# oadrian/GPUFluidSimulator

Measured on AMD Instinct MI355X. Metric: particle-steps/sec, higher is better.
Workload: dtype f32; 1 GPU; dam-break C3: 256x256x256 = 16777216 particles, grid 512^3, box 32.0, dt 5e-7, jittered lattice, FLOWING: timed after 6000 run-up steps on the device (+5 warm-up); particles=16777216, parallelism=1 GPU, whole domain, state=flow, runup_steps=6000

## Files before the change

### gpufluidsimulator_amd/capi.py

```python
from __future__ import annotations

import ctypes as C
import os

import numpy as np

HERE = os.path.dirname(os.path.abspath(__file__))
LIB_PATH = os.environ.get("SPH_HIP_LIB", os.path.join(HERE, "libsph_hip.so"))

PHASES = ("z-index", "sort", "b-grid", "dens", "force", "collision", "integrate")
HALO_RECORD_FLOATS = 8


class SphError(RuntimeError):
    pass


EXCHANGE_FN = C.CFUNCTYPE(C.c_int, C.c_void_p, C.c_int, C.c_void_p, C.c_size_t, C.c_void_p, C.c_size_t, C.c_void_p, C.c_size_t,
                          C.c_void_p, C.c_size_t, C.c_void_p)


class Transport(C.Structure):
    _fields_ = [("self", C.c_void_p), ("exchange", EXCHANGE_FN), ("host_buffers", C.c_int),
                ("abort", C.CFUNCTYPE(None, C.c_void_p))]


class Params(C.Structure):
    _fields_ = [("box_min", C.c_float * 3), ("box_max", C.c_float * 3), ("grid", C.c_uint32 * 3),
                ("h", C.c_float), ("mass", C.c_float), ("rest_density", C.c_float), ("gas_constant", C.c_float),
                ("viscosity", C.c_float), ("gravity_y", C.c_float), ("wall_eps", C.c_float),
                ("wall_damping", C.c_float), ("restitution", C.c_float), ("collision_param", C.c_float),
                ("particle_radius", C.c_float)]


MAX_COLLIDERS = 8


class Collider(C.Structure):
    _fields_ = [("center", C.c_float * 3), ("radius", C.c_float), ("velocity", C.c_float * 3), ("pad", C.c_float)]


_P = C.c_void_p
_U32 = C.c_uint32
SIGNATURES = {
    "sph_abi_version": (C.c_int, []),
    "sph_last_error": (C.c_char_p, []),
    "sph_device_count": (C.c_int, [C.POINTER(C.c_int)]),
    "sph_select_device": (C.c_int, [C.c_int]),
    "sph_selected_device": (C.c_int, []),
    "sph_default_params": (None, [C.POINTER(Params), C.POINTER(C.c_float), C.POINTER(_U32)]),
    "sph_grid_dim_for_edge": (_U32, [C.c_float, C.c_float]),
    "sph_create": (C.c_int, [C.POINTER(_P), C.c_int, _U32, C.POINTER(Params)]),
    "sph_create_slab": (C.c_int, [C.POINTER(_P), C.c_int, _U32, C.POINTER(Params), _U32, _U32, _U32]),
    "sph_create_slab_layers": (C.c_int, [C.POINTER(_P), C.c_int, _U32, C.POINTER(Params), _U32, _U32, _U32, _U32]),
    "sph_ghost_layers": (_U32, [_P]),
    "sph_slab_set_protocol": (C.c_int, [_P, C.c_int]),
    "sph_slab_protocol": (C.c_int, [_P, C.POINTER(C.c_uint64)]),
    "sph_destroy": (None, [_P]),
    "sph_set_stream": (C.c_int, [_P, _P]),
    "sph_set_params": (C.c_int, [_P, C.POINTER(Params)]),
    "sph_get_params": (C.c_int, [_P, C.POINTER(Params)]),
    "sph_sync": (C.c_int, [_P]),
    "sph_num_particles": (_U32, [_P]),
    "sph_capacity": (_U32, [_P]),
    "sph_upload": (C.c_int, [_P, _U32, _P, _P, _P]),
    "sph_set_by_index": (C.c_int, [_P, _U32, _U32, C.c_void_p, C.c_void_p]),
    "sph_reset_lattice": (C.c_int, [_P, C.POINTER(_U32), C.c_int, C.POINTER(C.c_float), C.c_uint64, _U32]),
    "sph_download": (C.c_int, [_P, _U32, _U32, _P, _P, _P, _P]),
    "sph_download_owned": (C.c_int, [_P, _P, _P, _P]),
    "sph_download_forces": (C.c_int, [_P, _U32, _U32, _P, _P, _P, _P]),
    "sph_snapshot_save": (C.c_int, [_P, C.c_char_p]),
    "sph_snapshot_load": (C.c_int, [_P, C.c_char_p]),
    "sph_snapshot_info": (C.c_int, [C.c_char_p, C.POINTER(_U32), C.POINTER(Params)]),
    "sph_set_colliders": (C.c_int, [_P, _U32, C.POINTER(Collider)]),
    "sph_get_colliders": (C.c_int, [_P, C.POINTER(_U32), C.POINTER(Collider)]),
    "sph_positions_dev": (C.c_int, [_P, C.POINTER(_P)]),
    "sph_download_positions4": (C.c_int, [_P, _P]),
    "sph_get_keys": (C.c_int, [_P, _P]),
    "sph_get_order": (C.c_int, [_P, _P]),
    "sph_get_cell_range": (C.c_int, [_P, _U32, C.POINTER(_U32), C.POINTER(_U32)]),
    "sph_get_cells": (C.c_int, [_P, _U32, _P, _P, _P]),
    "sph_cell_key": (_U32, [_P, _U32, _U32, _U32]),
    "sph_hash": (C.c_int, [_P]),
    "sph_sort": (C.c_int, [_P]),
    "sph_build_cells": (C.c_int, [_P]),
    "sph_density": (C.c_int, [_P]),
    "sph_force": (C.c_int, [_P]),
    "sph_collide": (C.c_int, [_P]),
    "sph_integrate": (C.c_int, [_P, C.c_float]),
    "sph_step": (C.c_int, [_P, C.c_float, _U32]),
    "sph_step_phased": (C.c_int, [_P, C.c_float, _U32]),
    "sph_force_collide_integrate": (C.c_int, [_P, C.c_float]),
    "sph_timing_enable": (C.c_int, [_P, C.c_int]),
    "sph_timing_get": (C.c_int, [_P, C.POINTER(C.c_float), C.POINTER(_U32)]),
    "sph_timing_reset": (C.c_int, [_P]),
    "sph_last_sort_skipped": (C.c_int, [_P]),
    "sph_sort_stats": (C.c_int, [_P, C.POINTER(C.c_uint64), C.POINTER(C.c_uint64), C.POINTER(C.c_uint64), C.POINTER(C.c_uint32),
                                 C.POINTER(C.c_uint64)]),
    "sph_set_sort_mode": (C.c_int, [_P, C.c_int]),
    "sph_set_direct_hull": (C.c_int, [_P, C.c_uint32]),
    "sph_set_pair_small_launch": (C.c_int, [_P, C.c_uint32]),
    "sph_set_block_order": (C.c_int, [_P, C.c_int, C.c_int, C.c_uint32]),
    "sph_sort_forms": (C.c_int, [_P, C.POINTER(C.c_uint64)]),
    "sph_test_trust_mover_hint": (C.c_int, [_P]),
    "sph_set_precision": (C.c_int, [_P, C.c_int]),
    "sph_get_precision": (C.c_int, [_P]),
    "sph_migrants_count": (C.c_int, [_P, C.POINTER(_U32)]),
    "sph_slab_counts": (C.c_int, [_P, C.POINTER(_U32)]),
    "sph_migrants_pack": (C.c_int, [_P, C.POINTER(_P), _U32]),
    "sph_migrants_append": (C.c_int, [_P, _P, _U32]),
    "sph_halo_count": (C.c_int, [_P, C.POINTER(_U32)]),
    "sph_halo_pack": (C.c_int, [_P, C.POINTER(_P), _U32]),
    "sph_halo_pack_counts": (C.c_int, [_P, C.POINTER(_P), _U32, C.POINTER(_U32)]),
    "sph_halo_unpack": (C.c_int, [_P, _P, _U32, _P, _U32]),
    "sph_halo_pack_density": (C.c_int, [_P, C.POINTER(_P), _U32]),
    "sph_halo_unpack_density": (C.c_int, [_P, _P, _P]),
    "sph_layer_histogram": (C.c_int, [_P, _P, _U32]),
    "sph_rccl_unique_id": (C.c_int, [C.c_void_p]),
    "sph_rccl_transport_create": (C.c_int, [C.POINTER(C.POINTER(Transport)), C.c_void_p, C.c_int, C.c_int, C.c_int]),
    "sph_rccl_transport_destroy": (None, [C.POINTER(Transport)]),
    "sph_rccl_transport_selftest": (C.c_int, [C.POINTER(Transport), C.c_size_t]),
    "sph_rccl_transport_info": (C.c_int, [C.POINTER(Transport), C.POINTER(C.c_int)]),
    "sph_slab_ping": (C.c_int, [_P, C.c_size_t, _U32, C.POINTER(C.c_double)]),
    "sph_slab_recut": (C.c_int, [_P, _U32, _U32]),
    "sph_slab_recut_stats": (C.c_int, [_P, C.POINTER(C.c_uint64)]),
    "sph_slab_set_early_force": (C.c_int, [_P, C.c_int]),
    "sph_slab_early_force_stats": (C.c_int, [_P, C.POINTER(C.c_uint64)]),
    "sph_slab_timing_enable": (C.c_int, [_P, C.c_int]),
    "sph_slab_timing_reset": (C.c_int, [_P]),
    "sph_slab_timing_get": (C.c_int, [_P, C.POINTER(C.c_double)]),
    "sph_slab_test_raise_flag": (C.c_int, [_P, C.c_int]),
    "sph_slab_in_place_merges": (C.c_uint64, [C.c_void_p]),
    "sph_slab_exchanges": (C.c_uint64, [C.c_void_p]),
    "sph_slab_failed": (C.c_int, [C.c_void_p]),
    "sph_slab_create": (C.c_int, [C.POINTER(_P), _P, C.c_int, C.c_int, C.POINTER(Transport), _U32]),
    "sph_slab_destroy": (None, [_P]),
    "sph_slab_step": (C.c_int, [_P, C.c_float, _U32]),
    "sph_slab_sync": (C.c_int, [_P]),
    "sph_slab_stats": (C.c_int, [_P, C.POINTER(C.c_uint64)]),
    "sph_slab_counters": (C.c_int, [_P, C.POINTER(C.c_uint64)]),
    "sph_slab_set_wait_timeout": (C.c_int, [_P, C.c_double]),
    "sph_local_hub_create": (C.c_int, [C.POINTER(_P), C.c_int, C.c_int]),
    "sph_local_hub_destroy": (None, [_P]),
    "sph_local_hub_set_timeout": (C.c_int, [_P, C.c_double]),
    "sph_local_transport_create": (C.c_int, [C.POINTER(C.POINTER(Transport)), _P, C.c_int]),
    "sph_local_transport_destroy": (None, [C.POINTER(Transport)]),
    "sph_loop_transport_create": (C.c_int, [C.POINTER(C.POINTER(Transport)), C.c_float, C.c_double, C.c_double]),
    "sph_loop_transport_destroy": (None, [C.POINTER(Transport)]),
    "sph_ic_dam_break": (None, [C.POINTER(_U32), C.POINTER(C.c_float), C.c_int, C.c_uint64, C.c_uint64, _P, _P]),
    "sph_ic_random_box": (None, [C.c_uint64, C.POINTER(C.c_float), C.c_float, _U32, C.c_float, _P, _P]),
}

_lib = None
_torch_first = None


def load():
    global _lib, _torch_first
    if _lib is None:
        import sys
        _torch_first = "torch" in sys.modules
        if not os.path.exists(LIB_PATH):
            from . import build as _b
            _b.build()
        lib = C.CDLL(LIB_PATH)
        lenient = bool(os.environ.get("SPH_HIP_LIB_ALLOW_MISSING"))
        for name, (res, args) in SIGNATURES.items():
            if lenient and not hasattr(lib, name):
                continue
            fn = getattr(lib, name)
            fn.restype = res
            fn.argtypes = args
        if lib.sph_abi_version() != 2:
            raise SphError("libsph_hip.so ABI version mismatch")
        _lib = lib
    return _lib


def _check(rc):
    if rc < 0:
        raise SphError(f"libsph_hip error {rc}: {load().sph_last_error().decode()}")
    return rc


def default_params(box, grid) -> Params:
    p = Params()
    load().sph_default_params(C.byref(p), (C.c_float * 3)(*[float(b) for b in box]),
                              (C.c_uint32 * 3)(*[int(g) for g in grid]))
    return p


def device_count():
    flag = C.c_int(0)
    n = load().sph_device_count(C.byref(flag))
    return n, bool(flag.value)


class LocalHub:

    def __init__(self, world, device=0, timeout_s=None):
        h = _P()
        _check(load().sph_local_hub_create(C.byref(h), int(world), int(device)))
        self.h = h
        if timeout_s:
            _check(load().sph_local_hub_set_timeout(self.h, float(timeout_s)))

    def transport(self, rank):
        t = C.POINTER(Transport)()
        _check(load().sph_local_transport_create(C.byref(t), self.h, int(rank)))
        return t

    def close(self):
        if getattr(self, "h", None):
            load().sph_local_hub_destroy(self.h)
            self.h = None


def _f32(a, cols):
    a = np.ascontiguousarray(a, dtype=np.float32)
    return a.reshape(-1, cols)


class Context:

    def __init__(self, capacity, box=None, grid=None, params: Params | None = None, device=0,
                 slab=None, ghost_capacity=0, ghost_layers=1):
        self.L = load()
        self.params = params if params is not None else default_params(box, grid)
        h = _P()
        if slab is None:
            _check(self.L.sph_create(C.byref(h), device, int(capacity), C.byref(self.params)))
        else:
            _check(self.L.sph_create_slab_layers(C.byref(h), device, int(capacity), C.byref(self.params),
                                                 int(slab[0]), int(slab[1]), int(ghost_capacity), int(ghost_layers)))
        self.h = h
        self.capacity = int(capacity)
        self.index_base = 0
        self.index_count = int(capacity)

    def close(self):
        if getattr(self, "h", None):
            self.L.sph_destroy(self.h)
            self.h = None

    def __del__(self):
        try:
            self.close()
        except Exception:
            pass

    def __enter__(self):
        return self

    def __exit__(self, *a):
        self.close()

    @property
    def n(self):
        return int(self.L.sph_num_particles(self.h))

    def set_stream(self, stream_handle):
        _check(self.L.sph_set_stream(self.h, _P(stream_handle)))

    def set_params(self, params: Params):
        _check(self.L.sph_set_params(self.h, C.byref(params)))
        self.params = params

    def upload(self, pos, vel=None, index=None):
        pos = _f32(pos, 3)
        n = pos.shape[0]
        vel = _f32(vel, 3) if vel is not None else None
        idx = np.ascontiguousarray(index, dtype=np.uint32) if index is not None else None
        _check(self.L.sph_upload(self.h, n, pos.ctypes.data, vel.ctypes.data if vel is not None else None,
                                 idx.ctypes.data if idx is not None else None))

    def set_by_index(self, first_index, pos=None, vel=None):
        pos = None if pos is None else np.ascontiguousarray(pos, dtype=np.float32)
        vel = None if vel is None else np.ascontiguousarray(vel, dtype=np.float32)
        count = (pos if pos is not None else vel).shape[0]
        assert vel is None or pos is None or vel.shape == pos.shape
        _check(self.L.sph_set_by_index(self.h, int(first_index), int(count),
                                       None if pos is None else pos.ctypes.data, None if vel is None else vel.ctypes.data))

    def reset_lattice(self, lattice, jitter=True, jitter_dims=None, start=0, count=None):
        lat = (_U32 * 3)(*[int(v) for v in lattice])
        total = int(lattice[0]) * int(lattice[1]) * int(lattice[2])
        count = total - start if count is None else count
        jd = (C.c_float * 3)(*[float(v) for v in jitter_dims]) if jitter_dims is not None else None
        _check(self.L.sph_reset_lattice(self.h, lat, 1 if jitter else 0, jd, int(start), int(count)))

    def download(self, index_base=0, count=None, want=("pos", "vel", "density", "pressure")):
        count = self.index_count if count is None else count
        out = {}
        for k in want:
            out[k] = np.full((count, 3) if k in ("pos", "vel") else (count,), np.nan, dtype=np.float32)
        ptr = lambda k: out[k].ctypes.data if k in out else None
        _check(self.L.sph_download(self.h, int(index_base), int(count), ptr("pos"), ptr("vel"), ptr("density"),
                                   ptr("pressure")))
        return out

    def download_owned(self):
        n = self.n
        pos, vel, idx = np.empty((n, 3), np.float32), np.empty((n, 3), np.float32), np.empty(n, np.uint32)
        _check(self.L.sph_download_owned(self.h, pos.ctypes.data, vel.ctypes.data, idx.ctypes.data))
        return pos, vel, idx

    def download_forces(self, index_base=0, count=None, force=True, collision=True):
        count = self.index_count if count is None else count
        out = {}
        if force:
            out["fpress"] = np.full((count, 3), np.nan, dtype=np.float32)
            out["fvisc"] = np.full((count, 3), np.nan, dtype=np.float32)
        if collision:
            out["dv"] = np.full((count, 3), np.nan, dtype=np.float32)
            out["count"] = np.full((count,), -1, dtype=np.int32)
        ptr = lambda k: out[k].ctypes.data if k in out else None
        _check(self.L.sph_download_forces(self.h, int(index_base), int(count), ptr("fpress"), ptr("fvisc"), ptr("dv"),
                                          ptr("count")))
        return out

    def save(self, path):
        _check(self.L.sph_snapshot_save(self.h, os.fsencode(path)))

    def load_snapshot(self, path):
        _check(self.L.sph_snapshot_load(self.h, os.fsencode(path)))

    @staticmethod
    def snapshot_info(path):
        n, p = _U32(0), Params()
        _check(load().sph_snapshot_info(os.fsencode(path), C.byref(n), C.byref(p)))
        return int(n.value), p

    def set_colliders(self, centers, radii, velocities=None):
        centers = _f32(centers, 3)
        n = centers.shape[0]
        radii = np.ascontiguousarray(radii, dtype=np.float32).reshape(-1)
        velocities = np.zeros((n, 3), np.float32) if velocities is None else _f32(velocities, 3)
        if radii.shape[0] != n or velocities.shape[0] != n:
            raise ValueError("centers, radii and velocities describe different numbers of spheres")
        arr = (Collider * max(n, 1))()
        for j in range(n):
            arr[j].center[:] = [float(v) for v in centers[j]]
            arr[j].radius = float(radii[j])
            arr[j].velocity[:] = [float(v) for v in velocities[j]]
        _check(self.L.sph_set_colliders(self.h, n, arr))

    def colliders(self):
        arr = (Collider * MAX_COLLIDERS)()
        n = _U32()
        _check(self.L.sph_get_colliders(self.h, C.byref(n), arr))
        rows = [arr[j] for j in range(n.value)]
        return {"centers": np.array([list(r.center) for r in rows], np.float32).reshape(-1, 3),
                "radii": np.array([r.radius for r in rows], np.float32),
                "velocities": np.array([list(r.velocity) for r in rows], np.float32).reshape(-1, 3)}

    def positions4(self):
        out = np.empty((self.capacity, 4), dtype=np.float32)
        _check(self.L.sph_download_positions4(self.h, out.ctypes.data))
        return out

    def positions_dev(self):
        p = _P()
        _check(self.L.sph_positions_dev(self.h, C.byref(p)))
        return p.value

    def keys(self):
        out = np.empty(self.n, dtype=np.uint32)
        _check(self.L.sph_get_keys(self.h, out.ctypes.data))
        return out

    def order(self):
        out = np.empty(self.n, dtype=np.uint32)
        _check(self.L.sph_get_order(self.h, out.ctypes.data))
        return out

    def cells(self, max_cells=None):
        max_cells = self.n + 16 if max_cells is None else max_cells
        k = np.empty(max_cells, dtype=np.uint32)
        s = np.empty(max_cells, dtype=np.uint32)
        c = np.empty(max_cells, dtype=np.uint32)
        m = _check(self.L.sph_get_cells(self.h, max_cells, k.ctypes.data, s.ctypes.data, c.ctypes.data))
        m = min(m, max_cells)
        return k[:m], s[:m], c[:m]

    def cell_range(self, cell):
        a, b = _U32(), _U32()
        _check(self.L.sph_get_cell_range(self.h, int(cell), C.byref(a), C.byref(b)))
        return a.value, b.value

    def cell_key(self, x, y, z):
        return int(self.L.sph_cell_key(self.h, int(x), int(y), int(z)))

    def hash(self): _check(self.L.sph_hash(self.h))
    def sort(self): _check(self.L.sph_sort(self.h))
    def build_cells(self): _check(self.L.sph_build_cells(self.h))
    def density(self): _check(self.L.sph_density(self.h))
    def force(self): _check(self.L.sph_force(self.h))
    def collide(self): _check(self.L.sph_collide(self.h))
    def integrate(self, dt): _check(self.L.sph_integrate(self.h, float(dt)))
    def step(self, dt, n=1): _check(self.L.sph_step(self.h, float(dt), int(n)))
    def step_phased(self, dt, n=1): _check(self.L.sph_step_phased(self.h, float(dt), int(n)))
    def sync(self): _check(self.L.sph_sync(self.h))

    def timing(self, on=True): _check(self.L.sph_timing_enable(self.h, 1 if on else 0))
    def timing_reset(self): _check(self.L.sph_timing_reset(self.h))

    def sort_skipped(self):
        return bool(self.L.sph_last_sort_skipped(self.h))

    def sort_stats(self):
        a, b, k, m, t = C.c_uint64(), C.c_uint64(), C.c_uint64(), C.c_uint32(), C.c_uint64()
        _check(self.L.sph_sort_stats(self.h, C.byref(a), C.byref(b), C.byref(k), C.byref(m), C.byref(t)))
        return {"sorts": a.value, "merges": b.value, "skips": k.value, "last_movers": m.value, "movers_total": t.value}

    def set_precision(self, mixed_f16=False):
        _check(self.L.sph_set_precision(self.h, 1 if mixed_f16 else 0))

    def set_sort_mode(self, merge=True):
        _check(self.L.sph_set_sort_mode(self.h, int(merge)))

    def trust_mover_hint(self):
        _check(self.L.sph_test_trust_mover_hint(self.h))

    def sort_forms(self):
        out = (C.c_uint64 * 3)()
        _check(self.L.sph_sort_forms(self.h, out))
        return tuple(int(v) for v in out)

    def set_block_order(self, xcd=True, ztile=True, strip_blocks_log2=4):
        _check(self.L.sph_set_block_order(self.h, int(bool(xcd)), int(bool(ztile)), int(strip_blocks_log2)))

    def set_direct_hull(self, slots=512):
        _check(self.L.sph_set_direct_hull(self.h, int(slots) & 0xFFFFFFFF))

    def set_pair_small_launch(self, slots):
        _check(self.L.sph_set_pair_small_launch(self.h, int(slots) & 0xFFFFFFFF))

    def timing_get(self):
        ms = (C.c_float * len(PHASES))()
        steps = _U32(0)
        _check(self.L.sph_timing_get(self.h, ms, C.byref(steps)))
        return {PHASES[k]: float(ms[k]) for k in range(len(PHASES))}, int(steps.value)

    def _pair(self, fn, *a):
        cnt = (_U32 * 2)()
        _check(fn(self.h, cnt, *a))
        return int(cnt[0]), int(cnt[1])

    def slab_counts(self):
        cnt = (_U32 * 4)()
        _check(self.L.sph_slab_counts(self.h, cnt))
        return tuple(int(v) for v in cnt)

    def force_collide_integrate(self, dt): _check(self.L.sph_force_collide_integrate(self.h, float(dt)))

    def migrants_count(self): return self._pair(self.L.sph_migrants_count)
    def halo_count(self): return self._pair(self.L.sph_halo_count)

    def migrants_pack(self, buf_lo, buf_hi, capacity):
        _check(self.L.sph_migrants_pack(self.h, (_P * 2)(buf_lo, buf_hi), int(capacity)))

    def migrants_append(self, buf, n):
        _check(self.L.sph_migrants_append(self.h, _P(buf), int(n)))

    def halo_pack(self, buf_lo, buf_hi, capacity, counts=None):
        if counts is None:
            _check(self.L.sph_halo_pack(self.h, (_P * 2)(buf_lo, buf_hi), int(capacity)))
        else:
            _check(self.L.sph_halo_pack_counts(self.h, (_P * 2)(buf_lo, buf_hi), int(capacity),
                                               (_U32 * 2)(int(counts[0]), int(counts[1]))))

    def halo_unpack(self, lo, n_lo, hi, n_hi):
        _check(self.L.sph_halo_unpack(self.h, _P(lo), int(n_lo), _P(hi), int(n_hi)))

    def halo_pack_density(self, buf_lo, buf_hi, capacity):
        _check(self.L.sph_halo_pack_density(self.h, (_P * 2)(buf_lo, buf_hi), int(capacity)))

    def halo_unpack_density(self, lo, hi):
        _check(self.L.sph_halo_unpack_density(self.h, _P(lo), _P(hi)))

    def layer_histogram(self):
        n = int(self.params.grid[2])
        out = np.zeros(n, dtype=np.uint32)
        _check(self.L.sph_layer_histogram(self.h, out.ctypes.data, n))
        return out
```

### gpufluidsimulator_amd/csrc/sph_capi.hip

```cpp
#include "sph_common.hpp"

#include <cmath>
#include <cstdarg>
#include <cstdlib>
#include <cstring>
#include <new>

namespace sph {

static thread_local std::string g_err;
static int g_device = 0;

void set_error(const char* fmt, ...) {
    char buf[512];
    va_list ap;
    va_start(ap, fmt);
    vsnprintf(buf, sizeof(buf), fmt, ap);
    va_end(ap);
    g_err = buf;
}

int hip_fail(hipError_t e, const char* what, const char* file, int line) {
    set_error("HIP error %d (%s) at %s:%d: %s", (int)e, hipGetErrorString(e), file, line, what);
    return SPH_E_DEVICE;
}

static uint32_t next_pow2(uint32_t x) {
    x--; x |= x >> 1; x |= x >> 2; x |= x >> 4; x |= x >> 8; x |= x >> 16; x++;
    return x;
}

static int derive(sph_ctx* c, const sph_params* p, uint32_t z_lo, uint32_t z_hi, bool slab) {
    for (int a = 0; a < 3; a++) {
        SPH_REQUIRE(p->grid[a] >= 1 && p->grid[a] <= 4096, SPH_E_INVALID, "grid[%d] = %u out of range", a, p->grid[a]);
        SPH_REQUIRE(p->box_max[a] > p->box_min[a], SPH_E_INVALID, "empty box on axis %d", a);
    }
    SPH_REQUIRE(p->h > 0.f && p->mass > 0.f && p->particle_radius > 0.f, SPH_E_INVALID, "h, mass, radius must be > 0");
    SPH_REQUIRE(z_lo < z_hi && z_hi <= p->grid[2], SPH_E_INVALID, "bad slab [%u, %u) of %u layers", z_lo, z_hi, p->grid[2]);
    c->params = *p;
    GridDesc& g = c->grid;
    for (int a = 0; a < 3; a++) {
        g.box_min[a] = p->box_min[a];
        g.box_dims[a] = p->box_max[a] - p->box_min[a];
        {
            int e = 0;
            const float m = frexpf(g.box_dims[a], &e);
            g.inv_dims[a] = (m == 0.5f && e > -100 && e < 100) ? 1.0f / g.box_dims[a] : 0.0f;
        }
        g.g[a] = p->grid[a];
        g.gf[a] = (float)p->grid[a];
    }
    c->z_lo = z_lo; c->z_hi = z_hi;
    const uint32_t G = c->ghost_layers;
    SPH_REQUIRE(G == 1u || G == 2u, SPH_E_INVALID, "a slab keeps 1 or 2 ghost layers per side, not %u", G);
    g.z_off = slab ? (int32_t)z_lo - (int32_t)G : 0;
    g.zl = slab ? z_hi - z_lo + 2u * G : p->grid[2];
    SPH_REQUIRE(slab || (z_lo == 0 && z_hi == p->grid[2]), SPH_E_INVALID, "a whole-domain context owns every layer");
    uint64_t nc = (uint64_t)g.g[0] * g.g[1] * g.zl;
    SPH_REQUIRE(nc < (1ull << 32), SPH_E_INVALID, "cell table too large (%llu cells)", (unsigned long long)nc);
    g.ncells = (uint32_t)nc;
    c->key_bits = 1;
    while (c->key_bits < 32 && (1ull << c->key_bits) < nc) c->key_bits++;

    const float PI_F = 3.141592654f;
    Phys& ph = c->phys;
    ph.h = p->h;
    ph.h2 = p->h * p->h;
    ph.mass = p->mass;
    ph.rest_density = p->rest_density;
    ph.gas_constant = p->gas_constant;
    const float poly6 = 315.f / (65.f * PI_F * powf(p->h, 9.f));
    const float spiky = 45.f / (PI_F * powf(p->h, 6.f));
    ph.poly6_mass = p->mass * poly6;
    ph.spiky_half_mass = p->mass * spiky * 0.5f;
    const float visc = p->viscosity != 0.f ? p->viscosity : 1.f;
    ph.visc_coef = (visc * p->mass) * spiky;
    ph.cp_scale = ph.spiky_half_mass / ph.visc_coef;
    ph.visc_on = p->viscosity != 0.f ? 1.f : 0.f;
    ph.gravity_y = p->gravity_y;
    ph.wall_eps = p->wall_eps;
    ph.wall_damping = p->wall_damping;
    const double cd = (double)p->collision_param * 2.0 * (double)p->particle_radius;
    float r2max = (float)(cd * cd);
    for (int k = 0; k < 8; k++) r2max = nextafterf(r2max, INFINITY);
    while ((double)sqrtf(r2max) > cd) r2max = nextafterf(r2max, 0.f);
    ph.coll_dist2 = r2max;
    ph.coll_mass = p->mass * (1.f + p->restitution);
    for (int a = 0; a < 3; a++) { ph.box_min[a] = p->box_min[a]; ph.box_max[a] = p->box_max[a]; }
    return SPH_OK;
}

template <class T>
static int dev_alloc(T** p, size_t count) {
    *p = nullptr;
    if (count == 0) count = 1;
    hipError_t e = hipMalloc((void**)p, count * sizeof(T));
    if (e != hipSuccess) {
        set_error("hipMalloc of %zu bytes failed: %s", count * sizeof(T), hipGetErrorString(e));
        return SPH_E_NOMEM;
    }
    return SPH_OK;
}

static void free_all(sph_ctx* c) {
    hipFree(c->posi); hipFree(c->velr); hipFree(c->posi2); hipFree(c->velr2); hipFree(c->keyS); hipFree(c->dp); hipFree(c->cw);
    hipFree(c->fpress); hipFree(c->fvisc); hipFree(c->dvel); hipFree(c->pos_out); hipFree(c->cells_base);
    hipFree(c->k0); hipFree(c->v0); hipFree(c->k1); hipFree(c->v1); hipFree(c->os_hist); hipFree(c->os_base); hipFree(c->os_tickets); hipFree(c->os_tot); hipFree(c->os_status); hipFree(c->os_status32); hipFree(c->keyS2); hipFree(c->mm_tileL); hipFree(c->mm_tileA);
    if (c->os_err_host) hipHostFree(c->os_err_host);
    hipFree(c->d_scratch);
    hipFree(c->mm_mask); hipFree(c->mm_M64); hipFree(c->mm_tile_cnt); hipFree(c->mm_tile_off);
    hipFree(c->mm_k0); hipFree(c->mm_k1); hipFree(c->mm_v1); hipFree(c->mm_count); hipFree(c->mm_total);
    if (c->mm_count_host) hipHostFree(c->mm_count_host);
    if (c->h_scratch) hipHostFree(c->h_scratch);
}

static int create_impl(sph_ctx** out, int device, uint32_t capacity, const sph_params* p, uint32_t z_lo, uint32_t z_hi,
                       uint32_t gcap, bool slab, uint32_t ghost_layers = 1) {
    SPH_REQUIRE(out && p, SPH_E_INVALID, "null argument");
    *out = nullptr;
    SPH_REQUIRE(capacity > 0 && (uint64_t)capacity + 2ull * gcap < (1ull << 31), SPH_E_INVALID, "bad capacity");
    int ndev = 0;
    hipError_t e = hipGetDeviceCount(&ndev);
    if (e != hipSuccess || ndev <= 0) {
        set_error("no HIP device available (%s): libsph_hip has no CPU fallback", hipGetErrorString(e));
        return SPH_E_DEVICE;
    }
    if (device < 0) device = g_device;
    SPH_REQUIRE(device < ndev, SPH_E_DEVICE, "device %d out of range (%d devices)", device, ndev);
    SPH_HIP(hipSetDevice(device));
    hipDeviceProp_t prop;
    SPH_HIP(hipGetDeviceProperties(&prop, device));
    if (strncmp(prop.gcnArchName, "gfx950", 6) != 0) {
        set_error("device %d is %s; libsph_hip is built for gfx950 (MI355X) only", device, prop.gcnArchName);
        return SPH_E_DEVICE;
    }
    sph_ctx* c = new (std::nothrow) sph_ctx();
    SPH_REQUIRE(c, SPH_E_NOMEM, "out of host memory");
    c->device = device;
    c->ghost_layers = slab ? ghost_layers : 1u;
    int rc = derive(c, p, z_lo, z_hi, slab);
    if (rc) { delete c; return rc; }
    c->cap = capacity; c->gcap = gcap; c->tot = capacity + 2 * gcap; c->slab = slab;
    c->own_off = gcap;
    c->sort_blocks_cap = ceil_div(capacity, SORT_TILE_KEYS) + 1;
    c->pos_out_cap = slab ? 0 : capacity;
    const size_t tot = (size_t)c->tot + 256;
    rc = dev_alloc(&c->posi, tot);
    if (!rc) rc = dev_alloc(&c->velr, tot);
    if (!rc) rc = dev_alloc(&c->posi2, tot);
    if (!rc) rc = dev_alloc(&c->velr2, tot);
    if (!rc) rc = dev_alloc(&c->keyS, tot);
    if (!rc) rc = dev_alloc(&c->keyS2, tot);
    if (!rc) rc = dev_alloc(&c->dp, tot);
    if (!rc) rc = dev_alloc(&c->cw, tot);
    if (!rc) rc = dev_alloc(&c->fpress, tot);
    if (!rc) rc = dev_alloc(&c->fvisc, tot);
    if (!rc) rc = dev_alloc(&c->dvel, tot);
    if (!rc) rc = dev_alloc(&c->pos_out, (size_t)c->pos_out_cap);
    if (!rc) rc = dev_alloc(&c->cells_base, (size_t)c->grid.ncells + 2);
    if (!rc) { c->cells = c->cells_base + 1; c->cells_alloc = c->grid.ncells; }
    if (!rc) rc = dev_alloc(&c->k0, (size_t)capacity);
    if (!rc) rc = dev_alloc(&c->v0, (size_t)capacity);
    if (!rc) rc = dev_alloc(&c->k1, (size_t)capacity);
    if (!rc) rc = dev_alloc(&c->v1, (size_t)capacity);
    const size_t os_groups = (size_t)c->sort_blocks_cap / 4 + 3;
    c->os_groups_cap = (uint32_t)os_groups;
    if (!rc) rc = dev_alloc(&c->os_hist, os_groups * 4 * 512);
    if (!rc) rc = dev_alloc(&c->os_base, os_groups * 4 * 512);
    if (!rc) rc = dev_alloc(&c->os_tickets, (size_t)4 * os_groups);
    if (!rc) rc = dev_alloc(&c->os_tot, (size_t)4 * 512);
    if (!rc) rc = dev_alloc(&c->os_status, (size_t)512 * c->sort_blocks_cap);
    if (!rc) rc = dev_alloc(&c->os_status32, (size_t)512 * c->sort_blocks_cap);
    if (!rc) rc = dev_alloc(&c->mm_tileL, (size_t)c->sort_blocks_cap + 2);
    if (!rc) rc = dev_alloc(&c->mm_tileA, (size_t)c->sort_blocks_cap + 2);
    if (!rc && (hipHostMalloc((void**)&c->os_err_host, sizeof(uint32_t), hipHostMallocMapped) != hipSuccess ||
                hipHostGetDevicePointer((void**)&c->os_err_dev, c->os_err_host, 0) != hipSuccess)) {
        set_error("hipHostMalloc(mapped) failed");
        rc = SPH_E_NOMEM;
    }
    if (!rc) {
        *c->os_err_host = 0;
        if (hipMemset(c->os_status, 0, (size_t)512 * c->sort_blocks_cap * sizeof(unsigned long long)) != hipSuccess ||
            hipMemset(c->os_status32, 0, (size_t)512 * c->sort_blocks_cap * sizeof(uint32_t)) != hipSuccess ||
            hipMemset(c->os_tickets, 0, 4 * os_groups * sizeof(uint32_t)) != hipSuccess ||
            hipMemset(c->os_hist, 0, os_groups * 4 * 512 * sizeof(uint32_t)) != hipSuccess ||
            hipMemset(c->keyS, 0, tot * sizeof(uint32_t)) != hipSuccess ||
            hipMemset(c->keyS2, 0, tot * sizeof(uint32_t)) != hipSuccess) {
            set_error("hipMemset failed");
            rc = SPH_E_DEVICE;
        }
    }
    if (!rc) rc = dev_alloc(&c->d_scratch, (size_t)64);
    if (!rc && hipHostMalloc((void**)&c->h_scratch, 64 * sizeof(uint32_t)) != hipSuccess) {
        set_error("hipHostMalloc failed");
        rc = SPH_E_NOMEM;
    }
    if (const char* env = getenv("SPH_BLOCK_ORDER")) {
        int x = 1, z = 1, sh = 4, zd = 1, xr = 1;
        if (sscanf(env, "%d,%d,%d,%d,%d", &x, &z, &sh, &zd, &xr) >= 1) {
            c->order_xcd = x != 0; c->order_ztile = z != 0; if (sh >= 1 && sh <= 10) c->order_strip_sh = (uint32_t)sh;
            c->order_ztile_dens = zd != 0; c->order_xrot = xr != 0;
        }
    }
    if (const char* env = getenv("SPH_PAIR_SMALL_SLOTS")) {
        unsigned long v = 0;
        if (sscanf(env, "%lu", &v) == 1) c->pair_small_slots = v > 0xFFFFFFFFul ? 0xFFFFFFFFu : (uint32_t)v;
    }
    {
        const char* env = getenv("SPH_SORT_MERGE");
        c->sort_merge = !(env && env[0] == '0');
        const size_t nchunks = (size_t)ceil_div(capacity, 64u) + 1, ntiles = nchunks / 256 + 2;
        if (!rc) rc = dev_alloc(&c->mm_mask, nchunks);
        if (!rc) rc = dev_alloc(&c->mm_M64, nchunks);
        if (!rc) rc = dev_alloc(&c->mm_tile_cnt, ntiles);
        if (!rc) rc = dev_alloc(&c->mm_tile_off, ntiles);
        if (!rc) rc = dev_alloc(&c->mm_k0, (size_t)capacity);
        if (!rc) rc = dev_alloc(&c->mm_k1, (size_t)capacity);
        if (!rc) rc = dev_alloc(&c->mm_v1, (size_t)capacity);
        if (!rc) rc = dev_alloc(&c->mm_count, (size_t)1);
        if (!rc) rc = dev_alloc(&c->mm_total, (size_t)1);
        if (!rc && (hipHostMalloc((void**)&c->mm_count_host, 8 * sizeof(uint32_t), hipHostMallocMapped) != hipSuccess ||
                    hipHostGetDevicePointer((void**)&c->mm_count_host_dev, c->mm_count_host, 0) != hipSuccess)) {
            set_error("hipHostMalloc(mapped) failed");
            rc = SPH_E_NOMEM;
        }
        if (!rc) {
            c->mm_count_host[0] = 0;
            c->mm_count_host[1] = 1; c->mm_count_host[2] = 0;
            for (int k = 3; k < 8; k++) c->mm_count_host[k] = 0;
            if (hipMemset(c->mm_tile_cnt, 0, ntiles * sizeof(uint32_t)) != hipSuccess ||
                hipMemset(c->mm_count, 0, sizeof(uint32_t)) != hipSuccess ||
                hipMemset(c->mm_total, 0, sizeof(unsigned long long)) != hipSuccess) {
                set_error("hipMemset failed");
                rc = SPH_E_DEVICE;
            }
        }
    }
    if (!rc && hipMemset(c->cells_base, 0, ((size_t)c->grid.ncells + 2) * sizeof(uint2)) != hipSuccess) {
        set_error("hipMemset(cells) failed");
        rc = SPH_E_DEVICE;
    }
    if (!rc && (hipMemset(c->dp, 0, tot * sizeof(float2)) != hipSuccess ||
                hipMemset(c->cw, 0, tot * sizeof(float2)) != hipSuccess ||
                hipMemset(c->posi, 0, tot * sizeof(float4)) != hipSuccess ||
                hipMemset(c->velr, 0, tot * sizeof(float4)) != hipSuccess ||
                hipMemset(c->posi2, 0, tot * sizeof(float4)) != hipSuccess ||
                hipMemset(c->velr2, 0, tot * sizeof(float4)) != hipSuccess)) {
        set_error("hipMemset failed");
        rc = SPH_E_DEVICE;
    }
    if (rc) { free_all(c); delete c; return rc; }
    *out = c;
    return SPH_OK;
}

void timing_collect(sph_ctx* c) {
    for (size_t k = 0; k + 3 <= c->events.size(); k += 3) {
        hipEvent_t a = c->events[k], b = c->events[k + 1];
        int phase = (int)(intptr_t)c->events[k + 2];
        hipEventSynchronize(b);
        float ms = 0.f;
        if (hipEventElapsedTime(&ms, a, b) == hipSuccess) c->ph_ms[phase] += ms;
        hipEventDestroy(a);
        hipEventDestroy(b);
    }
    c->events.clear();
}

static int do_hash(sph_ctx* c) {
    PhaseTimer t(c, SPH_PH_ZINDEX);
    const uint32_t lo = c->own_off - c->n_glo, hi = c->own_off + c->n + c->n_ghi;
    c->cells_clear_deferred = c->sort_merge && c->order_valid && c->cells_valid && c->cells_lo == lo && c->cells_hi == hi;
    int rc;
    c->ghost_clear_pending = false;
    if (c->cells_clear_deferred && c->defer_ghost_clear && (c->n_glo | c->n_ghi)) {
        c->ghost_clear[0] = lo; c->ghost_clear[1] = c->own_off; c->ghost_clear[2] = c->own_off + c->n; c->ghost_clear[3] = hi;
        c->ghost_clear_pending = true;
        rc = SPH_OK;
    } else if (c->cells_clear_deferred) {
        rc = launch_cells_clear_2ranges(c, lo, c->own_off, c->own_off + c->n, hi);
        c->cells_lo = c->own_off; c->cells_hi = c->own_off + c->n;
    } else {
        rc = launch_cells_clear(c);
    }
    if (rc) return rc;
    rc = launch_hash(c);
    if (rc) return rc;
    c->keys_fresh = false;
    c->stage = sph_ctx::ST_HASHED;
    return SPH_OK;
}

static int do_sort(sph_ctx* c) {
    PhaseTimer t(c, SPH_PH_SORT);
    int rc = launch_sort(c);
    if (rc) return rc;
    c->n_glo = c->n_ghi = 0;
    c->halo_n_valid = false;
    c->stage = sph_ctx::ST_SORTED;
    c->have_dens = c->have_force = c->have_coll = false;
    return SPH_OK;
}

static int do_cells(sph_ctx* c) {
    PhaseTimer t(c, SPH_PH_BGRID);
    const uint32_t lo = c->own_off - c->n_glo, hi = c->own_off + c->n + c->n_ghi;
    if (!(c->cells_valid && c->cells_lo == lo && c->cells_hi == hi)) {
        int rc = launch_cells_build(c);
        if (rc) return rc;
    }
    c->stage = sph_ctx::ST_CELLS;
    return SPH_OK;
}

int step_hash(sph_ctx* c) { return do_hash(c); }
int step_sort(sph_ctx* c) { return do_sort(c); }
int step_cells(sph_ctx* c) { return do_cells(c); }

static int do_density(sph_ctx* c) {
    PhaseTimer t(c, SPH_PH_DENS);
    int rc = launch_density(c);
    if (rc) return rc;
    c->have_dens = true;
    return SPH_OK;
}

}

namespace sph {
int set_slab_range(sph_ctx* c, uint32_t z_lo, uint32_t z_hi) {
    SPH_REQUIRE(c && c->slab, SPH_E_INVALID, "set_slab_range needs a slab context");
    sph_ctx tmp;
    tmp.params = c->params;
    tmp.ghost_layers = c->ghost_layers;
    int rc = derive(&tmp, &c->params, z_lo, z_hi, true);
    if (rc) return rc;
    if (tmp.grid.ncells > c->cells_alloc) {
        SPH_HIP(hipStreamSynchronize(c->stream));
        uint2* base = nullptr;
        rc = dev_alloc(&base, (size_t)tmp.grid.ncells + 2);
        if (rc) return rc;
        if (hipMemset(base, 0, ((size_t)tmp.grid.ncells + 2) * sizeof(uint2)) != hipSuccess) {
            hipFree(base);
            set_error("set_slab_range: clearing the new cell table failed");
            return SPH_E_DEVICE;
        }
        hipFree(c->cells_base);
        c->cells_base = base; c->cells = base + 1; c->cells_alloc = tmp.grid.ncells;
    }
    c->grid = tmp.grid; c->z_lo = z_lo; c->z_hi = z_hi; c->key_bits = tmp.key_bits;
    c->cells_valid = false; c->cells_clear_deferred = false;
    c->keys_fresh = false; c->order_valid = false;
    c->stage = sph_ctx::ST_LOADED;
    c->have_dens = c->have_force = c->have_coll = false;
    c->n_glo = c->n_ghi = 0;
    c->halo_n_valid = false;
    return SPH_OK;
}
}

using namespace sph;

__global__ __launch_bounds__(256) void k_set_by_index(float4* __restrict__ posi, float4* __restrict__ velr, uint32_t n,
                                                      uint32_t first, uint32_t count, const float* __restrict__ pos,
                                                      const float* __restrict__ vel, float4* __restrict__ pos_by_index) {
    const uint32_t i = blockIdx.x * 256u + threadIdx.x;
    if (i >= n) return;
    float4 p = posi[i];
    const uint32_t k = __float_as_uint(p.w) - first;
    if (k >= count) return;
    if (pos) {
        p.x = pos[3 * k]; p.y = pos[3 * k + 1]; p.z = pos[3 * k + 2];
        posi[i] = p;
        if (pos_by_index) pos_by_index[first + k] = make_float4(p.x, p.y, p.z, 1.0f);
    }
    if (vel) velr[i] = make_float4(vel[3 * k], vel[3 * k + 1], vel[3 * k + 2], 0.f);
}


__global__ __launch_bounds__(256) void k_gather_cells(const uint32_t* __restrict__ keys, uint32_t m,
                                                      const uint2* __restrict__ cells, uint2* __restrict__ out) {
    const uint32_t k = blockIdx.x * 256u + threadIdx.x;
    if (k < m) out[k] = cells[keys[k]];
}

extern "C" {

int sph_abi_version(void) { return SPH_ABI_VERSION; }

const char* sph_last_error(void) { return g_err.c_str(); }

int sph_device_count(int* is_gfx950) {
    int n = 0;
    if (is_gfx950) *is_gfx950 = 0;
    hipError_t e = hipGetDeviceCount(&n);
    if (e != hipSuccess) { set_error("hipGetDeviceCount: %s", hipGetErrorString(e)); return SPH_E_DEVICE; }
    if (n > 0 && is_gfx950) {
        hipDeviceProp_t prop;
        if (hipGetDeviceProperties(&prop, 0) == hipSuccess) *is_gfx950 = strncmp(prop.gcnArchName, "gfx950", 6) == 0;
    }
    return n;
}

int sph_select_device(int device) {
    int n = 0;
    hipError_t e = hipGetDeviceCount(&n);
    if (e != hipSuccess || n <= 0) {
        set_error("no HIP device available (%s): libsph_hip has no CPU fallback", hipGetErrorString(e));
        return SPH_E_DEVICE;
    }
    SPH_REQUIRE(device >= 0 && device < n, SPH_E_DEVICE, "device %d out of range (%d devices)", device, n);
    hipDeviceProp_t prop;
    SPH_HIP(hipGetDeviceProperties(&prop, device));
    SPH_REQUIRE(strncmp(prop.gcnArchName, "gfx950", 6) == 0, SPH_E_DEVICE,
                "device %d is %s; libsph_hip is built for gfx950 (MI355X) only", device, prop.gcnArchName);
    SPH_HIP(hipSetDevice(device));
    g_device = device;
    return SPH_OK;
}

int sph_selected_device(void) { return g_device; }

void sph_default_params(sph_params* p, const float box_dims[3], const uint32_t grid[3]) {
    memset(p, 0, sizeof(*p));
    for (int a = 0; a < 3; a++) {
        p->box_min[a] = -box_dims[a] / 2;
        p->box_max[a] = box_dims[a] / 2;
        p->grid[a] = grid[a];
    }
    p->h = 0.1f;
    p->mass = 65.f;
    p->rest_density = 1000.f;
    p->gas_constant = 2000.f;
    p->viscosity = 250.f;
    p->gravity_y = -9.81f * 11000;
    p->wall_eps = 0.00001f;
    p->wall_damping = -.75f;
    p->restitution = 0.f;
    p->collision_param = 1.0f;
    p->particle_radius = 1.0f / 64.0f;
}

uint32_t sph_grid_dim_for_edge(float edge, float h) { return next_pow2((uint32_t)(edge / (0.66666f * h))); }

int sph_create(sph_ctx** out, int device, uint32_t capacity, const sph_params* p) {
    if (!p) { set_error("null params"); return SPH_E_INVALID; }
    return create_impl(out, device, capacity, p, 0, p->grid[2], 0, false);
}

int sph_create_slab(sph_ctx** out, int device, uint32_t capacity, const sph_params* p, uint32_t z_lo, uint32_t z_hi,
                    uint32_t ghost_capacity) {
    if (!p) { set_error("null params"); return SPH_E_INVALID; }
    return create_impl(out, device, capacity, p, z_lo, z_hi, ghost_capacity, true);
}

int sph_create_slab_layers(sph_ctx** out, int device, uint32_t capacity, const sph_params* p, uint32_t z_lo, uint32_t z_hi,
                           uint32_t ghost_capacity, uint32_t ghost_layers) {
    if (!p) { set_error("null params"); return SPH_E_INVALID; }
    if (ghost_layers != 1u && ghost_layers != 2u) { set_error("a slab keeps 1 or 2 ghost layers per side, not %u", ghost_layers); return SPH_E_INVALID; }
    return create_impl(out, device, capacity, p, z_lo, z_hi, ghost_capacity, true, ghost_layers);
}

uint32_t sph_ghost_layers(const sph_ctx* c) { return c ? (c->slab ? c->ghost_layers : 0u) : 0u; }

void sph_destroy(sph_ctx* c) {
    if (!c) return;
    hipSetDevice(c->device);
    hipStreamSynchronize(c->stream);
    timing_collect(c);
    free_all(c);
    delete c;
}

int sph_set_stream(sph_ctx* c, void* s) {
    SPH_REQUIRE(c, SPH_E_INVALID, "null context");
    c->stream = (hipStream_t)s;
    return SPH_OK;
}

int sph_set_params(sph_ctx* c, const sph_params* p) {
    SPH_REQUIRE(c && p, SPH_E_INVALID, "null argument");
    for (int a = 0; a < 3; a++)
        SPH_REQUIRE(p->grid[a] == c->params.grid[a], SPH_E_INVALID, "the grid cannot change after sph_create");
    sph_ctx tmp;
    tmp.params = c->params;
    tmp.ghost_layers = c->ghost_layers;
    int rc = derive(&tmp, p, c->z_lo, c->z_hi, c->slab);
    if (rc) return rc;
    c->params = tmp.params; c->grid = tmp.grid; c->phys = tmp.phys;
    c->keys_fresh = false;
    c->order_valid = false;
    c->sort_form_both_until = c->sort_calls + 5;
    return SPH_OK;
}

int sph_get_params(const sph_ctx* c, sph_params* p) {
    SPH_REQUIRE(c && p, SPH_E_INVALID, "null argument");
    *p = c->params;
    return SPH_OK;
}

int sph_sync(sph_ctx* c) {
    SPH_REQUIRE(c, SPH_E_INVALID, "null context");
    SPH_HIP(hipStreamSynchronize(c->stream));
    SPH_REQUIRE(*c->os_err_host == 0u, SPH_E_DEVICE,
                "radix sort: a look-back on another tile's digit counts timed out (results of the last sort are invalid)");
    return SPH_OK;
}

uint32_t sph_num_particles(const sph_ctx* c) { return c ? c->n : 0; }
uint32_t sph_capacity(const sph_ctx* c) { return c ? c->cap : 0; }

int sph_upload(sph_ctx* c, uint32_t n, const float* pos, const float* vel, const uint32_t* index) {
    SPH_REQUIRE(c, SPH_E_INVALID, "null context");
    SPH_REQUIRE(n <= c->cap, SPH_E_CAPACITY, "%u particles > capacity %u", n, c->cap);
    SPH_REQUIRE(n == 0 || pos, SPH_E_INVALID, "null positions");
    SPH_HIP(hipSetDevice(c->device));
    std::vector<float4> hp(n), hv(n);
    for (uint32_t i = 0; i < n; i++) {
        uint32_t idx = index ? index[i] : i;
        if (!c->slab) SPH_REQUIRE(idx < c->pos_out_cap, SPH_E_INVALID, "creation index %u >= capacity %u", idx, c->pos_out_cap);
        float w;
        memcpy(&w, &idx, 4);
        hp[i] = make_float4(pos[3 * i], pos[3 * i + 1], pos[3 * i + 2], w);
        hv[i] = vel ? make_float4(vel[3 * i], vel[3 * i + 1], vel[3 * i + 2], 0.f) : make_float4(0.f, 0.f, 0.f, 0.f);
    }
    SPH_HIP(hipStreamSynchronize(c->stream));
    int rc = launch_cells_clear(c);
    if (rc) return rc;
    c->own_off = c->gcap;
    c->n = n; c->n_glo = c->n_ghi = 0;
    if (n) {
        SPH_HIP(hipMemcpyAsync(c->posi + c->own_off, hp.data(), n * sizeof(float4), hipMemcpyHostToDevice, c->stream));
        SPH_HIP(hipMemcpyAsync(c->velr + c->own_off, hv.data(), n * sizeof(float4), hipMemcpyHostToDevice, c->stream));
        SPH_HIP(hipMemsetAsync(c->dp + c->own_off, 0, n * sizeof(float2), c->stream));
        SPH_HIP(hipMemsetAsync(c->cw + c->own_off, 0, n * sizeof(float2), c->stream));
        if (!c->slab) {
            std::vector<float4> ho(c->pos_out_cap, make_float4(0.f, 0.f, 0.f, 0.f));
            for (uint32_t i = 0; i < n; i++) {
                uint32_t idx = index ? index[i] : i;
                ho[idx] = make_float4(pos[3 * i], pos[3 * i + 1], pos[3 * i + 2], 1.0f);
            }
            SPH_HIP(hipMemcpyAsync(c->pos_out, ho.data(), ho.size() * sizeof(float4), hipMemcpyHostToDevice, c->stream));
            SPH_HIP(hipStreamSynchronize(c->stream));
        }
    }
    SPH_HIP(hipStreamSynchronize(c->stream));
    c->stage = sph_ctx::ST_LOADED;
    c->keys_fresh = false;
    c->order_valid = false;
    c->sort_form_both_until = c->sort_calls + 5;
    c->have_dens = c->have_force = c->have_coll = false;
    return SPH_OK;
}

int sph_set_by_index(sph_ctx* c, uint32_t first_index, uint32_t count, const float* pos_xyz, const float* vel_xyz) {
    SPH_REQUIRE(c, SPH_E_INVALID, "null context");
    SPH_REQUIRE(c->slab || (uint64_t)first_index + count <= c->pos_out_cap, SPH_E_INVALID,
                "creation indices [%u, +%u) exceed the capacity %u", first_index, count, c->pos_out_cap);
    if (count == 0 || (!pos_xyz && !vel_xyz)) return SPH_OK;
    SPH_HIP(hipSetDevice(c->device));
    float* d_pos = nullptr; float* d_vel = nullptr;
    const size_t bytes = (size_t)count * 3 * sizeof(float);
    int rc = SPH_OK;
    if (pos_xyz) rc = dev_alloc(&d_pos, (size_t)count * 3);
    if (!rc && vel_xyz) rc = dev_alloc(&d_vel, (size_t)count * 3);
    if (!rc) {
        hipError_t e = hipSuccess;
        if (pos_xyz) e = hipMemcpyAsync(d_pos, pos_xyz, bytes, hipMemcpyHostToDevice, c->stream);
        if (e == hipSuccess && vel_xyz) e = hipMemcpyAsync(d_vel, vel_xyz, bytes, hipMemcpyHostToDevice, c->stream);
        if (e == hipSuccess && c->n) {
            hipLaunchKernelGGL(k_set_by_index, dim3(ceil_div(c->n, 256)), dim3(256), 0, c->stream, c->posi + c->own_off,
                               c->velr + c->own_off, c->n, first_index, count, d_pos, d_vel,
                               c->slab ? nullptr : c->pos_out);
            e = hipGetLastError();
        }
        if (e == hipSuccess) e = hipStreamSynchronize(c->stream);
        if (e != hipSuccess) { set_error("sph_set_by_index: %s", hipGetErrorString(e)); rc = SPH_E_DEVICE; }
    }
    hipFree(d_pos); hipFree(d_vel);
    if (rc) return rc;
    mm_drop_marks(c);
    c->keys_fresh = false;
    c->sort_form_both_until = c->sort_calls + 5;
    c->stage = sph_ctx::ST_LOADED;
    c->have_dens = c->have_force = c->have_coll = false;
    return SPH_OK;
}

int sph_reset_lattice(sph_ctx* c, const uint32_t lattice[3], int jitter, const float jitter_dims[3], uint64_t start,
                      uint32_t count) {
    SPH_REQUIRE(c && lattice, SPH_E_INVALID, "null argument");
    SPH_REQUIRE(count <= c->cap, SPH_E_CAPACITY, "%u particles > capacity %u", count, c->cap);
    const uint64_t total = (uint64_t)lattice[0] * lattice[1] * lattice[2];
    SPH_REQUIRE(lattice[0] && lattice[1] && lattice[2] && start + count <= total, SPH_E_INVALID,
                "index range [%llu, +%u) outside the %llu-particle lattice", (unsigned long long)start, count,
                (unsigned long long)total);
    SPH_REQUIRE(c->slab || start + count <= c->pos_out_cap, SPH_E_INVALID, "creation indices exceed the capacity %u",
                c->pos_out_cap);
    SPH_REQUIRE(total <= 0xFFFFFFFFull, SPH_E_INVALID, "creation indices are 32-bit");
    SPH_HIP(hipSetDevice(c->device));
    int rc = launch_cells_clear(c);
    if (rc) return rc;
    c->own_off = c->gcap;
    c->n = count; c->n_glo = c->n_ghi = 0;
    rc = launch_reset_lattice(c, lattice, jitter, jitter_dims, start, count);
    if (rc) return rc;
    c->stage = sph_ctx::ST_LOADED;
    c->keys_fresh = false;
    c->order_valid = false;
    c->sort_form_both_until = c->sort_calls + 5;
    c->have_dens = c->have_force = c->have_coll = false;
    return SPH_OK;
}

static int fetch_sorted(sph_ctx* c, std::vector<float4>* hp, std::vector<float4>* hv, std::vector<float2>* hd) {
    SPH_HIP(hipSetDevice(c->device));
    const uint32_t n = c->n;
    if (hp) { hp->resize(n); if (n) SPH_HIP(hipMemcpyAsync(hp->data(), c->posi + c->own_off, n * sizeof(float4), hipMemcpyDeviceToHost, c->stream)); }
    if (hv) { hv->resize(n); if (n) SPH_HIP(hipMemcpyAsync(hv->data(), c->velr + c->own_off, n * sizeof(float4), hipMemcpyDeviceToHost, c->stream)); }
    if (hd) { hd->resize(n); if (n) SPH_HIP(hipMemcpyAsync(hd->data(), c->dp + c->own_off, n * sizeof(float2), hipMemcpyDeviceToHost, c->stream)); }
    SPH_HIP(hipStreamSynchronize(c->stream));
    return SPH_OK;
}

static inline uint32_t idx_of(const float4& p) { uint32_t u; memcpy(&u, &p.w, 4); return u; }

int sph_download(sph_ctx* c, uint32_t base, uint32_t count, float* pos, float* vel, float* density, float* pressure) {
    SPH_REQUIRE(c, SPH_E_INVALID, "null context");
    std::vector<float4> hp, hv;
    std::vector<float2> hd;
    int rc = fetch_sorted(c, &hp, vel ? &hv : nullptr, (density || pressure) ? &hd : nullptr);
    if (rc) return rc;
    for (uint32_t s = 0; s < c->n; s++) {
        const uint32_t rel = idx_of(hp[s]) - base;
        if (rel >= count) continue;
        const size_t i = rel;
        if (pos) { pos[3 * i] = hp[s].x; pos[3 * i + 1] = hp[s].y; pos[3 * i + 2] = hp[s].z; }
        if (vel) { vel[3 * i] = hv[s].x; vel[3 * i + 1] = hv[s].y; vel[3 * i + 2] = hv[s].z; }
        if (density) density[i] = hd[s].x;
        if (pressure) pressure[i] = hd[s].y;
    }
    return SPH_OK;
}

int sph_download_owned(sph_ctx* c, float* pos, float* vel, uint32_t* index) {
    SPH_REQUIRE(c, SPH_E_INVALID, "null context");
    std::vector<float4> hp, hv;
    int rc = fetch_sorted(c, &hp, vel ? &hv : nullptr, nullptr);
    if (rc) return rc;
    for (uint32_t s = 0; s < c->n; s++) {
        if (pos) { pos[3 * s] = hp[s].x; pos[3 * s + 1] = hp[s].y; pos[3 * s + 2] = hp[s].z; }
        if (vel) { vel[3 * s] = hv[s].x; vel[3 * s + 1] = hv[s].y; vel[3 * s + 2] = hv[s].z; }
        if (index) index[s] = idx_of(hp[s]);
    }
    return SPH_OK;
}

int sph_download_forces(sph_ctx* c, uint32_t base, uint32_t n_out, float* fp, float* fv, float* dv, int32_t* count) {
    SPH_REQUIRE(c, SPH_E_INVALID, "null context");
    SPH_REQUIRE((!fp && !fv) || c->have_force, SPH_E_STATE, "sph_force has not run for this particle order");
    SPH_REQUIRE((!dv && !count) || c->have_coll, SPH_E_STATE, "sph_collide has not run for this particle order");
    std::vector<float4> hp;
    int rc = fetch_sorted(c, &hp, nullptr, nullptr);
    if (rc) return rc;
    const uint32_t n = c->n;
    std::vector<float4> a(n), b(n), d(n);
    if (n && (fp || fv)) {
        SPH_HIP(hipMemcpy(a.data(), c->fpress + c->own_off, n * sizeof(float4), hipMemcpyDeviceToHost));
        SPH_HIP(hipMemcpy(b.data(), c->fvisc + c->own_off, n * sizeof(float4), hipMemcpyDeviceToHost));
    }
    if (n && (dv || count)) SPH_HIP(hipMemcpy(d.data(), c->dvel + c->own_off, n * sizeof(float4), hipMemcpyDeviceToHost));
    for (uint32_t s = 0; s < n; s++) {
        const uint32_t rel = idx_of(hp[s]) - base;
        if (rel >= n_out) continue;
        const size_t i = rel;
        if (fp) { fp[3 * i] = a[s].x; fp[3 * i + 1] = a[s].y; fp[3 * i + 2] = a[s].z; }
        if (fv) { fv[3 * i] = b[s].x; fv[3 * i + 1] = b[s].y; fv[3 * i + 2] = b[s].z; }
        if (dv) { dv[3 * i] = d[s].x; dv[3 * i + 1] = d[s].y; dv[3 * i + 2] = d[s].z; }
        if (count) { uint32_t u; memcpy(&u, &d[s].w, 4); count[i] = (int32_t)u; }
    }
    return SPH_OK;
}

static const uint32_t kSnapMagic = 0x53485053u, kSnapVersion = 1u;

int sph_snapshot_save(sph_ctx* c, const char* path) {
    SPH_REQUIRE(c && path, SPH_E_INVALID, "null argument");
    std::vector<float4> hp, hv;
    int rc = fetch_sorted(c, &hp, &hv, nullptr);
    if (rc) return rc;
    FILE* f = fopen(path, "wb");
    SPH_REQUIRE(f, SPH_E_INVALID, "cannot open %s for writing", path);
    const uint32_t hdr[4] = {kSnapMagic, kSnapVersion, c->n, (uint32_t)sizeof(sph_params)};
    bool ok = fwrite(hdr, sizeof(hdr), 1, f) == 1 && fwrite(&c->params, sizeof(sph_params), 1, f) == 1;
    if (c->n) ok = ok && fwrite(hp.data(), sizeof(float4), c->n, f) == c->n && fwrite(hv.data(), sizeof(float4), c->n, f) == c->n;
    ok = (fclose(f) == 0) && ok;
    SPH_REQUIRE(ok, SPH_E_INVALID, "short write to %s", path);
    return SPH_OK;
}

static int snap_header(FILE* f, const char* path, uint32_t* n, sph_params* p) {
    uint32_t hdr[4];
    SPH_REQUIRE(fread(hdr, sizeof(hdr), 1, f) == 1 && hdr[0] == kSnapMagic, SPH_E_INVALID, "%s is not an SPH snapshot", path);
    SPH_REQUIRE(hdr[1] == kSnapVersion && hdr[3] == sizeof(sph_params), SPH_E_INVALID, "%s: unsupported snapshot version", path);
    SPH_REQUIRE(fread(p, sizeof(sph_params), 1, f) == 1, SPH_E_INVALID, "%s: truncated", path);
    *n = hdr[2];
    return SPH_OK;
}

int sph_snapshot_info(const char* path, uint32_t* n, sph_params* p) {
    SPH_REQUIRE(path && n && p, SPH_E_INVALID, "null argument");
    FILE* f = fopen(path, "rb");
    SPH_REQUIRE(f, SPH_E_INVALID, "cannot open %s", path);
    int rc = snap_header(f, path, n, p);
    fclose(f);
    return rc;
}

int sph_snapshot_load(sph_ctx* c, const char* path) {
    SPH_REQUIRE(c && path, SPH_E_INVALID, "null argument");
    FILE* f = fopen(path, "rb");
    SPH_REQUIRE(f, SPH_E_INVALID, "cannot open %s", path);
    uint32_t n = 0;
    sph_params p;
    int rc = snap_header(f, path, &n, &p);
    if (rc) { fclose(f); return rc; }
    if (n > c->cap) { fclose(f); set_error("snapshot holds %u particles, context capacity is %u", n, c->cap); return SPH_E_CAPACITY; }
    std::vector<float4> hp(n), hv(n);
    bool ok = n == 0 || (fread(hp.data(), sizeof(float4), n, f) == n && fread(hv.data(), sizeof(float4), n, f) == n);
    fclose(f);
    SPH_REQUIRE(ok, SPH_E_INVALID, "%s: truncated", path);
    rc = sph_set_params(c, &p);
    if (rc) return rc;
    std::vector<float> pos((size_t)n * 3), vel((size_t)n * 3);
    std::vector<uint32_t> idx(n);
    if (!c->slab) {
        std::vector<bool> seen(n, false);
        for (uint32_t i = 0; i < n; i++) {
            const uint32_t k = idx_of(hp[i]);
            SPH_REQUIRE(k < n && !seen[k], SPH_E_INVALID, "%s: creation index %u of record %u is out of range or repeated", path, k, i);
            seen[k] = true;
        }
    }
    for (uint32_t i = 0; i < n; i++) {
        pos[3 * i] = hp[i].x; pos[3 * i + 1] = hp[i].y; pos[3 * i + 2] = hp[i].z;
        vel[3 * i] = hv[i].x; vel[3 * i + 1] = hv[i].y; vel[3 * i + 2] = hv[i].z;
        idx[i] = idx_of(hp[i]);
    }
    return sph_upload(c, n, pos.data(), vel.data(), idx.data());
}

int sph_set_colliders(sph_ctx* c, uint32_t n, const sph_collider* colliders) {
    SPH_REQUIRE(c, SPH_E_INVALID, "null context");
    SPH_REQUIRE(n <= SPH_MAX_COLLIDERS, SPH_E_INVALID, "%u colliders > SPH_MAX_COLLIDERS (%d)", n, SPH_MAX_COLLIDERS);
    SPH_REQUIRE(n == 0 || colliders, SPH_E_INVALID, "null colliders");
    for (uint32_t j = 0; j < n; j++) {
        const sph_collider& s = colliders[j];
        SPH_REQUIRE(std::isfinite(s.radius) && s.radius > 0.f, SPH_E_INVALID, "collider %u: radius %g is not a positive finite number", j,
                    (double)s.radius);
        for (int a = 0; a < 3; a++)
            SPH_REQUIRE(std::isfinite(s.center[a]) && std::isfinite(s.velocity[a]), SPH_E_INVALID,
                        "collider %u: centre or velocity is not finite", j);
    }
    for (uint32_t j = 0; j < n; j++) {
        c->colliders[j] = colliders[j];
        c->colliders[j].pad = 0.f;
    }
    c->n_colliders = n;
    return SPH_OK;
}

int sph_get_colliders(const sph_ctx* c, uint32_t* n, sph_collider* out) {
    SPH_REQUIRE(c && n, SPH_E_INVALID, "null argument");
    *n = c->n_colliders;
    if (out)
        for (uint32_t j = 0; j < c->n_colliders; j++) out[j] = c->colliders[j];
    return SPH_OK;
}

int sph_positions_dev(sph_ctx* c, void** out) {
    SPH_REQUIRE(c && out, SPH_E_INVALID, "null argument");
    SPH_REQUIRE(!c->slab, SPH_E_STATE, "slab contexts keep no by-index position buffer");
    *out = c->pos_out;
    return SPH_OK;
}

int sph_download_positions4(sph_ctx* c, float* out) {
    SPH_REQUIRE(c && out, SPH_E_INVALID, "null argument");
    SPH_REQUIRE(!c->slab, SPH_E_STATE, "slab contexts keep no by-index position buffer");
    SPH_HIP(hipSetDevice(c->device));
    SPH_HIP(hipMemcpyAsync(out, c->pos_out, (size_t)c->pos_out_cap * sizeof(float4), hipMemcpyDeviceToHost, c->stream));
    SPH_HIP(hipStreamSynchronize(c->stream));
    return SPH_OK;
}

int sph_get_keys(sph_ctx* c, uint32_t* keys) {
    SPH_REQUIRE(c && keys, SPH_E_INVALID, "null argument");
    SPH_REQUIRE(c->stage >= sph_ctx::ST_HASHED, SPH_E_STATE, "sph_hash has not run");
    SPH_HIP(hipSetDevice(c->device));
    const uint32_t* src = c->stage == sph_ctx::ST_HASHED ? c->k0 : c->keyS + c->own_off;
    if (c->n) SPH_HIP(hipMemcpyAsync(keys, src, c->n * sizeof(uint32_t), hipMemcpyDeviceToHost, c->stream));
    SPH_HIP(hipStreamSynchronize(c->stream));
    return SPH_OK;
}

int sph_get_order(sph_ctx* c, uint32_t* index) {
    SPH_REQUIRE(c && index, SPH_E_INVALID, "null argument");
    std::vector<float4> hp;
    int rc = fetch_sorted(c, &hp, nullptr, nullptr);
    if (rc) return rc;
    for (uint32_t s = 0; s < c->n; s++) index[s] = idx_of(hp[s]);
    return SPH_OK;
}

int sph_get_cell_range(sph_ctx* c, uint32_t cell, uint32_t* start, uint32_t* end) {
    SPH_REQUIRE(c && start && end, SPH_E_INVALID, "null argument");
    SPH_REQUIRE(c->cells_valid, SPH_E_STATE, "sph_build_cells has not run");
    SPH_REQUIRE(cell < c->grid.ncells, SPH_E_INVALID, "cell %u out of range", cell);
    uint2 v;
    SPH_HIP(hipSetDevice(c->device));
    SPH_HIP(hipStreamSynchronize(c->stream));
    SPH_HIP(hipMemcpy(&v, c->cells + cell, sizeof(v), hipMemcpyDeviceToHost));
    *start = v.x - (v.y > v.x ? c->own_off - c->n_glo : 0);
    *end = v.y - (v.y > v.x ? c->own_off - c->n_glo : 0);
    return SPH_OK;
}

int sph_get_cells(sph_ctx* c, uint32_t max_cells, uint32_t* key, uint32_t* start, uint32_t* count) {
    SPH_REQUIRE(c, SPH_E_INVALID, "null context");
    SPH_REQUIRE(c->cells_valid, SPH_E_STATE, "sph_build_cells has not run");
    SPH_HIP(hipSetDevice(c->device));
    SPH_HIP(hipStreamSynchronize(c->stream));
    const uint32_t lo = c->cells_lo, hi = c->cells_hi;
    std::vector<uint32_t> ks(hi - lo);
    if (hi > lo) SPH_HIP(hipMemcpy(ks.data(), c->keyS + lo, (hi - lo) * sizeof(uint32_t), hipMemcpyDeviceToHost));
    std::vector<uint32_t> uniq;
    for (uint32_t s = 0; s < hi - lo; s++)
        if (s == 0 || ks[s] != ks[s - 1]) uniq.push_back(ks[s]);
    const uint32_t m = (uint32_t)uniq.size(), take = m < max_cells ? m : max_cells;
    if (take) {
        uint32_t* d_keys = nullptr; uint2* d_out = nullptr;
        int rc = dev_alloc(&d_keys, (size_t)take);
        if (!rc) rc = dev_alloc(&d_out, (size_t)take);
        std::vector<uint2> got(take);
        if (!rc) {
            hipError_t e = hipMemcpy(d_keys, uniq.data(), take * sizeof(uint32_t), hipMemcpyHostToDevice);
            if (e == hipSuccess) {
                hipLaunchKernelGGL(k_gather_cells, dim3(ceil_div(take, 256)), dim3(256), 0, c->stream, d_keys, take, c->cells,
                                   d_out);
                e = hipGetLastError();
            }
            if (e == hipSuccess) e = hipStreamSynchronize(c->stream);
            if (e == hipSuccess) e = hipMemcpy(got.data(), d_out, take * sizeof(uint2), hipMemcpyDeviceToHost);
            if (e != hipSuccess) { set_error("sph_get_cells: %s", hipGetErrorString(e)); rc = SPH_E_DEVICE; }
        }
        hipFree(d_keys); hipFree(d_out);
        if (rc) return rc;
        for (uint32_t k = 0; k < take; k++) {
            if (key) key[k] = uniq[k];
            if (start) start[k] = got[k].x - lo;
            if (count) count[k] = got[k].y - got[k].x;
        }
    }
    return (int)m;
}

uint32_t sph_cell_key(const sph_ctx* c, uint32_t x, uint32_t y, uint32_t z) {
    if (!c) return 0;
    return ((uint32_t)((int32_t)z - c->grid.z_off) * c->grid.g[1] + y) * c->grid.g[0] + x;
}

int sph_hash(sph_ctx* c) {
    SPH_REQUIRE(c, SPH_E_INVALID, "null context");
    SPH_HIP(hipSetDevice(c->device));
    return do_hash(c);
}

int sph_sort(sph_ctx* c) {
    SPH_REQUIRE(c, SPH_E_INVALID, "null context");
    SPH_REQUIRE(c->stage == sph_ctx::ST_HASHED, SPH_E_STATE, "sph_sort needs sph_hash first");
    SPH_HIP(hipSetDevice(c->device));
    return do_sort(c);
}

int sph_build_cells(sph_ctx* c) {
    SPH_REQUIRE(c, SPH_E_INVALID, "null context");
    SPH_REQUIRE(c->stage >= sph_ctx::ST_SORTED, SPH_E_STATE, "sph_build_cells needs sph_sort first");
    SPH_HIP(hipSetDevice(c->device));
    return do_cells(c);
}

int sph_density(sph_ctx* c) {
    SPH_REQUIRE(c, SPH_E_INVALID, "null context");
    SPH_REQUIRE(c->stage >= sph_ctx::ST_CELLS && c->cells_valid, SPH_E_STATE, "sph_density needs sph_build_cells first");
    SPH_HIP(hipSetDevice(c->device));
    return do_density(c);
}

int sph_force(sph_ctx* c) {
    SPH_REQUIRE(c, SPH_E_INVALID, "null context");
    SPH_REQUIRE(c->stage >= sph_ctx::ST_CELLS && c->have_dens, SPH_E_STATE, "sph_force needs sph_density first");
    SPH_HIP(hipSetDevice(c->device));
    PhaseTimer t(c, SPH_PH_FORCE);
    int rc = launch_force(c, true, false, false, 0.f);
    if (rc) return rc;
    c->have_force = true;
    return SPH_OK;
}

int sph_collide(sph_ctx* c) {
    SPH_REQUIRE(c, SPH_E_INVALID, "null context");
    SPH_REQUIRE(c->stage >= sph_ctx::ST_CELLS && c->cells_valid, SPH_E_STATE, "sph_collide needs sph_build_cells first");
    SPH_HIP(hipSetDevice(c->device));
    PhaseTimer t(c, SPH_PH_COLLISION);
    int rc = launch_force(c, false, true, false, 0.f);
    if (rc) return rc;
    c->have_coll = true;
    return SPH_OK;
}

int sph_integrate(sph_ctx* c, float dt) {
    SPH_REQUIRE(c, SPH_E_INVALID, "null context");
    SPH_REQUIRE(c->have_dens && c->have_force && c->have_coll, SPH_E_STATE,
                "sph_integrate needs sph_density, sph_force and sph_collide first");
    SPH_HIP(hipSetDevice(c->device));
    PhaseTimer t(c, SPH_PH_INTEGRATE);
    int rc = launch_integrate(c, dt);
    if (rc) return rc;
    c->have_force = c->have_coll = false;
    return SPH_OK;
}

int sph_step(sph_ctx* c, float dt, uint32_t n_steps) {
    SPH_REQUIRE(c, SPH_E_INVALID, "null context");
    SPH_HIP(hipSetDevice(c->device));
    for (uint32_t s = 0; s < n_steps; s++) {
        int rc = do_hash(c);
        if (!rc) rc = do_sort(c);
        if (!rc) rc = do_cells(c);
        if (!rc) rc = do_density(c);
        if (rc) return rc;
        {
            PhaseTimer t(c, SPH_PH_FORCE);
            rc = launch_force(c, true, true, true, dt);
            if (rc) return rc;
        }
        c->have_force = c->have_coll = false;
        if (c->timing) { c->timed_steps++; if (c->events.size() > 3 * 4096) timing_collect(c); }
    }
    return SPH_OK;
}

int sph_force_collide_integrate(sph_ctx* c, float dt) {
    SPH_REQUIRE(c, SPH_E_INVALID, "null context");
    SPH_REQUIRE(c->stage >= sph_ctx::ST_CELLS && c->have_dens, SPH_E_STATE,
                "sph_force_collide_integrate needs sph_density first");
    SPH_HIP(hipSetDevice(c->device));
    PhaseTimer t(c, SPH_PH_FORCE);
    int rc = launch_force(c, true, true, true, dt);
    if (rc) return rc;
    c->have_force = c->have_coll = false;
    return SPH_OK;
}

int sph_step_phased(sph_ctx* c, float dt, uint32_t n_steps) {
    for (uint32_t s = 0; s < n_steps; s++) {
        int rc = sph_hash(c);
        if (!rc) rc = sph_sort(c);
        if (!rc) rc = sph_build_cells(c);
        if (!rc) rc = sph_density(c);
        if (!rc) rc = sph_force(c);
        if (!rc) rc = sph_collide(c);
        if (!rc) rc = sph_integrate(c, dt);
        if (rc) return rc;
        if (c->timing) { c->timed_steps++; if (c->events.size() > 3 * 4096) timing_collect(c); }
    }
    return SPH_OK;
}

int sph_timing_enable(sph_ctx* c, int on) {
    SPH_REQUIRE(c, SPH_E_INVALID, "null context");
    c->timing = on != 0;
    return SPH_OK;
}

int sph_timing_get(sph_ctx* c, float ms[SPH_PH_COUNT], uint32_t* n_steps) {
    SPH_REQUIRE(c && ms, SPH_E_INVALID, "null argument");
    SPH_HIP(hipSetDevice(c->device));
    timing_collect(c);
    for (int k = 0; k < SPH_PH_COUNT; k++) ms[k] = (float)c->ph_ms[k];
    if (n_steps) *n_steps = c->timed_steps;
    return SPH_OK;
}

int sph_timing_reset(sph_ctx* c) {
    SPH_REQUIRE(c, SPH_E_INVALID, "null context");
    SPH_HIP(hipSetDevice(c->device));
    timing_collect(c);
    for (int k = 0; k < SPH_PH_COUNT; k++) c->ph_ms[k] = 0;
    c->timed_steps = 0;
    return SPH_OK;
}

int sph_last_sort_skipped(const sph_ctx* c) { return c && c->last_sort_skipped ? 1 : 0; }

int sph_set_precision(sph_ctx* c, int precision) {
    SPH_REQUIRE(c, SPH_E_INVALID, "null context");
    SPH_REQUIRE(precision == SPH_PRECISION_F32 || precision == SPH_PRECISION_MIXED_F16, SPH_E_INVALID,
                "unknown precision %d", precision);
    c->precision = precision;
    return SPH_OK;
}

int sph_get_precision(const sph_ctx* c) { return c ? c->precision : SPH_PRECISION_F32; }

int sph_set_sort_mode(sph_ctx* c, int merge) {
    SPH_REQUIRE(c, SPH_E_INVALID, "null context");
    c->sort_merge = merge != 0;
    c->sort_merge_always = merge == 2;
    return SPH_OK;
}

int sph_test_trust_mover_hint(sph_ctx* c) {
    SPH_REQUIRE(c, SPH_E_INVALID, "null context");
    c->sort_form_both_until = 0;
    return SPH_OK;
}

int sph_sort_forms(const sph_ctx* c, uint64_t out[3]) {
    SPH_REQUIRE(c && out, SPH_E_INVALID, "null argument");
    for (int k = 0; k < 3; k++) out[k] = c->sort_forms[k];
    return SPH_OK;
}

int sph_set_block_order(sph_ctx* c, int xcd, int ztile, uint32_t strip_blocks_log2) {
    SPH_REQUIRE(c, SPH_E_INVALID, "null context");
    SPH_REQUIRE(strip_blocks_log2 >= 1u && strip_blocks_log2 <= 10u, SPH_E_INVALID, "strip of 2^%u blocks", strip_blocks_log2);
    c->order_xcd = xcd != 0;
    c->order_ztile = c->order_ztile_dens = ztile != 0;
    c->order_strip_sh = strip_blocks_log2;
    return SPH_OK;
}

int sph_set_direct_hull(sph_ctx* c, uint32_t slots) {
    SPH_REQUIRE(c, SPH_E_INVALID, "null context");
    c->direct_hull = slots;
    return SPH_OK;
}

int sph_set_pair_small_launch(sph_ctx* c, uint32_t slots) {
    SPH_REQUIRE(c, SPH_E_INVALID, "null context");
    c->pair_small_slots = slots;
    return SPH_OK;
}

int sph_sort_stats(sph_ctx* c, uint64_t* sorts, uint64_t* merges, uint64_t* skips, uint32_t* last_movers,
                   uint64_t* movers_total) {
    SPH_REQUIRE(c, SPH_E_INVALID, "null context");
    SPH_HIP(hipSetDevice(c->device));
    SPH_HIP(hipStreamSynchronize(c->stream));
    if (movers_total) {
        unsigned long long t = 0;
        SPH_HIP(hipMemcpy(&t, c->mm_total, sizeof(t), hipMemcpyDeviceToHost));
        *movers_total = t;
    }
    if (sorts) *sorts = c->sort_calls;
    if (merges) *merges = c->sort_merges;
    if (skips) *skips = c->sort_skips;
    if (last_movers) *last_movers = *c->mm_count_host;
    return SPH_OK;
}

}
```

### gpufluidsimulator_amd/csrc/sph_common.hpp

```cpp
#pragma once

#include <hip/hip_runtime.h>

#include <cstdint>
#include <cstdio>
#include <string>
#include <vector>

#include "../../include/sph_hip.h"

namespace sph {

constexpr int WAVE = 64;
#ifndef SPH_SORT_KPT
#define SPH_SORT_KPT 16
#endif
constexpr uint32_t SORT_TILE_KEYS = 256 * SPH_SORT_KPT;
#ifndef SPH_PAIR_SMALL_SLOTS_DEFAULT
#define SPH_PAIR_SMALL_SLOTS_DEFAULT 524288u
#endif
constexpr uint32_t MM_TILE_CHUNKS = 256;

struct GridDesc {
    float box_min[3];
    float box_dims[3];
    float inv_dims[3];
    uint32_t g[3];
    float gf[3];
    int32_t z_off;
    uint32_t zl;
    uint32_t ncells;
};

struct Phys {
    float h, h2;
    float mass;
    float rest_density, gas_constant;
    float poly6_mass;
    float spiky_half_mass;
    float visc_coef;
    float cp_scale;
    float gravity_y;
    float wall_eps, wall_damping;
    float coll_dist2;
    float coll_mass;
    float box_min[3], box_max[3];
    float visc_on;
};

struct Spheres {
    float4 c[SPH_MAX_COLLIDERS];
    float4 u[SPH_MAX_COLLIDERS];
    uint32_t n;
};

}

struct sph_ctx {
    int device = 0;
    hipStream_t stream = nullptr;
    sph_params params{};
    int precision = SPH_PRECISION_F32;
    sph::GridDesc grid{};
    sph::Phys phys{};

    uint32_t cap = 0;
    uint32_t gcap = 0;
    uint32_t tot = 0;
    bool slab = false;
    uint32_t z_lo = 0, z_hi = 0;
    uint32_t ghost_layers = 1;

    uint32_t n = 0;
    uint32_t own_off = 0;
    uint32_t n_glo = 0, n_ghi = 0;
    uint32_t halo_n[2] = {0, 0};
    bool halo_n_valid = false;

    float4* posi = nullptr;
    float4* velr = nullptr;
    float4* posi2 = nullptr;
    float4* velr2 = nullptr;
    uint32_t* keyS = nullptr;
    uint32_t* keyS2 = nullptr;
    float2* dp = nullptr;
    float2* cw = nullptr;
    float4* fpress = nullptr;
    float4* fvisc = nullptr;
    float4* dvel = nullptr;
    float4* pos_out = nullptr;
    uint32_t pos_out_cap = 0;

    uint32_t n_colliders = 0;
    sph_collider colliders[SPH_MAX_COLLIDERS] = {};

    uint32_t direct_hull = 512;
    uint32_t pair_small_slots = SPH_PAIR_SMALL_SLOTS_DEFAULT;
    bool order_xcd = true, order_ztile = true;
    bool order_ztile_dens = true, order_xrot = true;
    uint32_t order_strip_sh = 4;

    uint2* cells = nullptr;
    uint2* cells_base = nullptr;
    uint32_t cells_alloc = 0;
    uint32_t cells_lo = 0, cells_hi = 0;
    bool cells_valid = false;
    bool cells_clear_deferred = false;
    bool owned_cells_in_bounds = false, owned_cells_pending = false;
    bool defer_ghost_clear = false, ghost_clear_pending = false;
    uint32_t ghost_clear[4] = {0, 0, 0, 0};
    bool keys_fresh = false;

    uint32_t* k0 = nullptr; uint32_t* v0 = nullptr;
    uint32_t* k1 = nullptr; uint32_t* v1 = nullptr;
    uint32_t* os_hist = nullptr;
    uint32_t* os_base = nullptr;
    uint32_t* os_tickets = nullptr;
    uint32_t* os_tot = nullptr;
    uint32_t os_groups_cap = 0;
    unsigned long long* os_status = nullptr;
    uint32_t* os_status32 = nullptr;
    uint32_t os_epoch = 0;
    uint32_t* os_err_host = nullptr;
    uint32_t* os_err_dev = nullptr;
    uint32_t sort_blocks_cap = 0;
    uint32_t key_bits = 0;
    const uint32_t* last_perm = nullptr;
    bool keep_perm = false;
    bool sort_merge = true;
    bool sort_merge_always = false;
    bool order_valid = false;
    bool last_sort_skipped = false;
    bool host_paced = false;
    uint32_t sort_seq_issued = 0;
    uint32_t scan_seq_issued = 0;
    uint32_t cells_seq_next = 0;
    bool mm_counted_valid = false;
    uint64_t sort_merges = 0, sort_calls = 0, sort_skips = 0;
    uint64_t sort_form_both_until = 0;
    uint64_t sort_forms[3] = {0, 0, 0};
    uint64_t* mm_mask = nullptr;
    uint32_t* mm_M64 = nullptr;
    uint32_t* mm_tile_cnt = nullptr; uint32_t* mm_tile_off = nullptr;
    uint32_t* mm_k0 = nullptr; uint32_t* mm_k1 = nullptr; uint32_t* mm_v1 = nullptr;
    uint32_t* mm_count = nullptr;
    uint32_t* mm_count_host = nullptr;
    uint32_t* mm_count_host_dev = nullptr;
    unsigned long long* mm_total = nullptr;
    bool mm_marked = false;
    bool mm_scanned = false;
    uint32_t* mm_tileL = nullptr;
    uint32_t* mm_tileA = nullptr;
    uint32_t mm_marked_off = 0, mm_marked_n = 0;
    uint32_t* d_scratch = nullptr;
    uint32_t* h_scratch = nullptr;

    enum Stage { ST_LOADED = 0, ST_HASHED, ST_SORTED, ST_CELLS } stage = ST_LOADED;
    bool have_force = false, have_coll = false, have_dens = false;

    bool timing = false;
    std::vector<hipEvent_t> events;
    double ph_ms[SPH_PH_COUNT] = {0};
    uint32_t timed_steps = 0;
};

namespace sph {

void set_error(const char* fmt, ...);
void mm_drop_marks(sph_ctx* c);
void mm_scan_marks(sph_ctx* c);
int hip_fail(hipError_t e, const char* what, const char* file, int line);

#define SPH_HIP(call)                                                        \
    do {                                                                     \
        hipError_t e__ = (call);                                             \
        if (e__ != hipSuccess) return sph::hip_fail(e__, #call, __FILE__, __LINE__); \
    } while (0)

#define SPH_REQUIRE(cond, code, ...)          \
    do {                                      \
        if (!(cond)) {                        \
            sph::set_error(__VA_ARGS__);      \
            return (code);                    \
        }                                     \
    } while (0)

int launch_hash(sph_ctx* c);
int launch_reset_lattice(sph_ctx* c, const uint32_t lattice[3], int jitter, const float jitter_dims[3], uint64_t start,
                         uint32_t count);
int launch_sort(sph_ctx* c);
int launch_merge_arrivals(sph_ctx* c, uint32_t n_in, uint32_t n_front = 0);
int launch_cells_clear(sph_ctx* c);
int launch_cells_clear_range(sph_ctx* c, uint32_t lo, uint32_t hi);
int launch_cells_build_range(sph_ctx* c, uint32_t lo, uint32_t hi);
int launch_cells_clear_2ranges(sph_ctx* c, uint32_t lo0, uint32_t hi0, uint32_t lo1, uint32_t hi1);
int launch_cells_build_2ranges(sph_ctx* c, uint32_t lo0, uint32_t hi0, uint32_t lo1, uint32_t hi1);
int launch_cells_build(sph_ctx* c);
constexpr uint32_t CELLS_SPT = 4;
inline uint32_t cells_build_blocks(uint32_t count) { return (count + 256u * CELLS_SPT - 1u) / (256u * CELLS_SPT); }
int launch_density(sph_ctx* c);
int launch_force(sph_ctx* c, bool force, bool collide, bool integrate, float dt);
int launch_density_range(sph_ctx* c, uint32_t lo, uint32_t hi);
int launch_density_hole(sph_ctx* c, uint32_t lo, uint32_t hi, uint32_t hole_lo, uint32_t hole_hi);
int launch_density_dev_range(sph_ctx* c, const uint32_t* range_dev, uint32_t max_count);
int launch_force_dev_range(sph_ctx* c, const uint32_t* range_dev, uint32_t max_count, float dt);
int launch_force_hole(sph_ctx* c, uint32_t lo, uint32_t hi, uint32_t hole_lo, uint32_t hole_hi, bool force, bool collide,
                      bool integrate, float dt, bool mark);
bool force_begin(sph_ctx* c, bool integrate);
int launch_force_range(sph_ctx* c, uint32_t lo, uint32_t hi, bool force, bool collide, bool integrate, float dt, bool mark);
void force_finish(sph_ctx* c, bool integrate, bool mark, float dt);
int set_slab_range(sph_ctx* c, uint32_t z_lo, uint32_t z_hi);
int step_hash(sph_ctx* c);
int step_sort(sph_ctx* c);
int step_cells(sph_ctx* c);
int launch_integrate(sph_ctx* c, float dt);

inline uint32_t ceil_div(uint32_t a, uint32_t b) { return (a + b - 1) / b; }

struct PhaseTimer {
    sph_ctx* c; int phase; hipEvent_t a = nullptr, b = nullptr;
    PhaseTimer(sph_ctx* c_, int ph) : c(c_), phase(ph) {
        if (!c->timing) return;
        if (hipEventCreate(&a) != hipSuccess || hipEventCreate(&b) != hipSuccess) { a = b = nullptr; return; }
        hipEventRecord(a, c->stream);
    }
    ~PhaseTimer() {
        if (!a || !b) return;
        hipEventRecord(b, c->stream);
        c->events.push_back(a);
        c->events.push_back(b);
        c->events.push_back((hipEvent_t)(intptr_t)phase);
    }
};
void timing_collect(sph_ctx* c);

}
```

### gpufluidsimulator_amd/csrc/sph_pairs.hip

```cpp
#include "sph_device.hpp"

namespace sph {

#ifndef SPH_PAIR_THREADS
#define SPH_PAIR_THREADS 256
#endif
constexpr int PAIR_THREADS = SPH_PAIR_THREADS;
constexpr int PAIR_WAVES = PAIR_THREADS / WAVE;
#ifndef SPH_DENS_THREADS
#define SPH_DENS_THREADS SPH_PAIR_THREADS
#endif
constexpr int DENS_THREADS = SPH_DENS_THREADS;
constexpr int SMALL_THREADS_PAIR = 128;
static inline bool small_blocks(const sph_ctx* c) { return c->n < c->pair_small_slots; }
constexpr int PIECE = 128;

typedef float v2f __attribute__((ext_vector_type(2)));
typedef const volatile __attribute__((address_space(3))) v2f* lds_v2f_ptr;
typedef const volatile __attribute__((address_space(3))) float* lds_f32_ptr;

__global__ __launch_bounds__(256) void k_cells_clear(const uint32_t* __restrict__ key, uint32_t lo, uint32_t hi,
                                                     uint2* __restrict__ cells) {
    uint32_t s = lo + blockIdx.x * 256u + threadIdx.x;
    if (s >= hi) return;
    uint32_t k = key[s];
    if (s == lo || key[s - 1] != k) cells[k] = make_uint2(0u, 0u);
}

__global__ __launch_bounds__(256) void k_cells_build(const uint32_t* __restrict__ key, uint32_t lo, uint32_t hi,
                                                     uint2* __restrict__ cells, volatile uint32_t* __restrict__ ends_host, uint32_t seq) {
    cells_build_thread(key, lo, hi, cells, ends_host, seq, blockIdx.x * 256u + threadIdx.x);
}

__global__ __launch_bounds__(256) void k_cells_clear2(const uint32_t* __restrict__ key, uint32_t lo0, uint32_t hi0,
                                                      uint32_t lo1, uint32_t hi1, uint2* __restrict__ cells) {
    const uint32_t t = blockIdx.x * 256u + threadIdx.x, n0 = hi0 - lo0;
    const uint32_t lo = t < n0 ? lo0 : lo1, hi = t < n0 ? hi0 : hi1;
    const uint32_t s = t < n0 ? lo0 + t : lo1 + (t - n0);
    if (s >= hi) return;
    const uint32_t k = key[s];
    if (s == lo || key[s - 1] != k) cells[k] = make_uint2(0u, 0u);
}

__global__ __launch_bounds__(256) void k_cells_build2(const uint32_t* __restrict__ key, uint32_t lo0, uint32_t hi0,
                                                      uint32_t lo1, uint32_t hi1, uint2* __restrict__ cells) {
    const uint32_t t = blockIdx.x * 256u + threadIdx.x, n0 = hi0 - lo0;
    const uint32_t lo = t < n0 ? lo0 : lo1, hi = t < n0 ? hi0 : hi1;
    const uint32_t s = t < n0 ? lo0 + t : lo1 + (t - n0);
    if (s >= hi) return;
    const uint32_t k = key[s];
    if (s == lo || key[s - 1] != k) cells[k].x = s;
    if (s + 1 == hi || key[s + 1] != k) cells[k].y = s + 1;
}

int launch_cells_clear_2ranges(sph_ctx* c, uint32_t lo0, uint32_t hi0, uint32_t lo1, uint32_t hi1) {
    if (hi0 < lo0) hi0 = lo0;
    if (hi1 < lo1) hi1 = lo1;
    const uint32_t tot = (hi0 - lo0) + (hi1 - lo1);
    if (!tot) return SPH_OK;
    hipLaunchKernelGGL(k_cells_clear2, dim3(ceil_div(tot, 256)), dim3(256), 0, c->stream, c->keyS, lo0, hi0, lo1, hi1, c->cells);
    SPH_HIP(hipGetLastError());
    return SPH_OK;
}

int launch_cells_build_2ranges(sph_ctx* c, uint32_t lo0, uint32_t hi0, uint32_t lo1, uint32_t hi1) {
    if (hi0 < lo0) hi0 = lo0;
    if (hi1 < lo1) hi1 = lo1;
    const uint32_t tot = (hi0 - lo0) + (hi1 - lo1);
    if (!tot) return SPH_OK;
    hipLaunchKernelGGL(k_cells_build2, dim3(ceil_div(tot, 256)), dim3(256), 0, c->stream, c->keyS, lo0, hi0, lo1, hi1, c->cells);
    SPH_HIP(hipGetLastError());
    return SPH_OK;
}

int launch_cells_clear(sph_ctx* c) {
    if (!c->cells_valid || c->cells_hi <= c->cells_lo) { c->cells_valid = false; return SPH_OK; }
    hipLaunchKernelGGL(k_cells_clear, dim3(ceil_div(c->cells_hi - c->cells_lo, 256)), dim3(256), 0, c->stream, c->keyS,
                       c->cells_lo, c->cells_hi, c->cells);
    SPH_HIP(hipGetLastError());
    c->cells_valid = false;
    return SPH_OK;
}

int launch_cells_clear_range(sph_ctx* c, uint32_t lo, uint32_t hi) {
    if (hi <= lo) return SPH_OK;
    hipLaunchKernelGGL(k_cells_clear, dim3(ceil_div(hi - lo, 256)), dim3(256), 0, c->stream, c->keyS, lo, hi, c->cells);
    SPH_HIP(hipGetLastError());
    return SPH_OK;
}

int launch_cells_build_range(sph_ctx* c, uint32_t lo, uint32_t hi) {
    if (hi <= lo) return SPH_OK;
    uint32_t* ends = (lo == c->own_off && hi == c->own_off + c->n) ? c->mm_count_host_dev + 1 : (uint32_t*)nullptr;
    const uint32_t seq = ends ? c->cells_seq_next : 0u;
    if (ends) c->cells_seq_next = 0u;
    hipLaunchKernelGGL(k_cells_build, dim3(cells_build_blocks(hi - lo)), dim3(256), 0, c->stream, c->keyS, lo, hi, c->cells, ends, seq);
    SPH_HIP(hipGetLastError());
    return SPH_OK;
}

int launch_cells_build(sph_ctx* c) {
    const uint32_t lo = c->own_off - c->n_glo, hi = c->own_off + c->n + c->n_ghi;
    int rc;
    if (c->cells_valid && c->cells_lo == c->own_off && c->cells_hi == c->own_off + c->n) {
        rc = launch_cells_build_2ranges(c, lo, c->own_off, c->own_off + c->n, hi);
    } else {
        rc = launch_cells_clear(c);
        if (!rc) rc = launch_cells_build_range(c, lo, hi);
    }
    if (rc) return rc;
    c->cells_lo = lo; c->cells_hi = hi; c->cells_valid = true;
    return SPH_OK;
}

struct Rows {
    uint32_t lo[9], hi[9];
};

__device__ __forceinline__ void lane_rows(const uint2* __restrict__ cells, const GridDesc& g, uint32_t key, bool active,
                                          Rows& R) {
    const uint32_t gx = g.g[0], gy = g.g[1];
    uint32_t cx, cy, lz;
    if (((gx & (gx - 1u)) | (gy & (gy - 1u))) == 0u) {
        const uint32_t sx = 31u - (uint32_t)__clz((int)gx), sy = 31u - (uint32_t)__clz((int)gy);
        cx = key & (gx - 1u);
        cy = (key >> sx) & (gy - 1u);
        lz = key >> (sx + sy);
    } else {
        cx = key % gx;
        const uint32_t t = key / gx;
        cy = t % gy;
        lz = t / gy;
    }
    const bool has_l = cx > 0u, has_r = cx + 1u < gx;
    const bool y_ok[3] = {cy > 0u, true, cy + 1u < gy};
    const bool z_ok[3] = {lz > 0u, true, lz + 1u < g.zl};
    const int sy_ = (int)gx, sz_ = (int)(gx * gy);
    uint2 a[9], b[9], d[9];
    bool ok[9];
#pragma unroll
    for (int dz = -1; dz <= 1; dz++) {
#pragma unroll
        for (int dy = -1; dy <= 1; dy++) {
            const int r = (dz + 1) * 3 + (dy + 1);
            ok[r] = active && y_ok[dy + 1] && z_ok[dz + 1];
            const uint2* p = cells + (ok[r] ? (int)key + dz * sz_ + dy * sy_ : (int)key);
            a[r] = p[-1]; b[r] = p[0]; d[r] = p[1];
        }
    }
#pragma unroll
    for (int r = 0; r < 9; r++) {
        const bool na = ok[r] && has_l && a[r].y > a[r].x, nb = ok[r] && b[r].y > b[r].x,
                   nd = ok[r] && has_r && d[r].y > d[r].x;
        R.lo[r] = na ? a[r].x : (nb ? b[r].x : (nd ? d[r].x : 0u));
        R.hi[r] = nd ? d[r].y : (nb ? b[r].y : (na ? a[r].y : 0u));
    }
}

__device__ __forceinline__ void lane_row_one(const uint2* __restrict__ cells, const GridDesc& g, uint32_t key, bool active,
                                             int dz, int dy, uint32_t& lo, uint32_t& hi) {
    const uint32_t gx = g.g[0], gy = g.g[1];
    uint32_t cx, cy, lz;
    if (((gx & (gx - 1u)) | (gy & (gy - 1u))) == 0u) {
        const uint32_t sx = 31u - (uint32_t)__clz((int)gx), sy = 31u - (uint32_t)__clz((int)gy);
        cx = key & (gx - 1u); cy = (key >> sx) & (gy - 1u); lz = key >> (sx + sy);
    } else {
        cx = key % gx;
        const uint32_t t = key / gx;
        cy = t % gy; lz = t / gy;
    }
    const bool ok = active && (int)cy + dy >= 0 && (int)cy + dy < (int)gy && (int)lz + dz >= 0 && (int)lz + dz < (int)g.zl;
    const uint2* p = cells + (ok ? (int)key + dz * (int)(gx * gy) + dy * (int)gx : (int)key);
    const uint2 a = p[-1], b = p[0], d = p[1];
    const bool na = ok && cx > 0u && a.y > a.x, nb = ok && b.y > b.x, nd = ok && cx + 1u < gx && d.y > d.x;
    lo = na ? a.x : (nb ? b.x : (nd ? d.x : 0u));
    hi = nd ? d.y : (nb ? b.y : (na ? a.y : 0u));
}

#ifndef SPH_DENS_OCC
#define SPH_DENS_OCC 6
#endif
#ifndef SPH_FORCE_OCC
#define SPH_FORCE_OCC 5
#endif

__device__ __forceinline__ float in_vgpr(float x) {
    asm volatile("" : "+v"(x));
    return x;
}

__device__ __forceinline__ float inv_sqrt(float x) { return __builtin_amdgcn_rsqf(x); }

__device__ __forceinline__ void wave_lds_sync() {
    __builtin_amdgcn_fence(__ATOMIC_RELEASE, "wavefront");
    __builtin_amdgcn_wave_barrier();
    __builtin_amdgcn_fence(__ATOMIC_ACQUIRE, "wavefront");
}

constexpr int lds_ent(int threads) { return (threads / WAVE + 1) * PIECE + 8; }
#ifndef SPH_DENS_UNROLL
#define SPH_DENS_UNROLL 4
#endif
constexpr int UNROLL = SPH_DENS_UNROLL;
#ifndef SPH_FORCE_UNROLL
#define SPH_FORCE_UNROLL 2
#endif
#ifndef SPH_EXACT_DIV
#define SPH_EXACT_DIV 0
#endif

struct Hulls {
    uint32_t A[9], B[9];
};

__device__ __forceinline__ void wave_hulls(const Rows& R, Hulls& H) {
#pragma unroll
    for (int r = 0; r < 9; r++) {
        const uint64_t m = __ballot(R.hi[r] > R.lo[r]);
        if (m == 0ull) { H.A[r] = 0u; H.B[r] = 0u; continue; }
        const int first = __builtin_ctzll(m), last = 63 - __builtin_clzll(m);
        H.A[r] = (uint32_t)__builtin_amdgcn_readlane((int)R.lo[r], first);
        H.B[r] = (uint32_t)__builtin_amdgcn_readlane((int)R.hi[r], last);
    }
}

template <class Load, class Store, class Work>
__device__ __forceinline__ void traverse(const Hulls& H, Load&& load, Store&& store, Work&& work) {
    bool ready = false;
#pragma unroll
    for (int r = 0; r < 9; r++) {
        if (H.A[r] >= H.B[r]) continue;
        if (!ready) load(H.A[r]);
        ready = false;
        for (uint32_t a = H.A[r]; a < H.B[r]; a += PIECE) {
            const uint32_t b = min(a + PIECE, H.B[r]);
            if (a != H.A[r]) load(a);
            store();
            if (b >= H.B[r] && r + 1 < 9 && H.A[r + 1] < H.B[r + 1]) {
                load(H.A[r + 1]);
                ready = true;
            }
            wave_lds_sync();
            work(r, a, b);
            wave_lds_sync();
        }
    }
}

__device__ __forceinline__ bool wave_has_long_hull(const Hulls& H, uint32_t key, uint32_t direct_hull) {
    const uint32_t k0 = (uint32_t)__builtin_amdgcn_readlane((int)key, 0), k1 = (uint32_t)__builtin_amdgcn_readlane((int)key, 63);
    if (k1 - k0 <= 64u && direct_hull >= 128u) return false;
    bool any = false;
#pragma unroll
    for (int r = 0; r < 9; r++) any = any || (H.B[r] > H.A[r] && H.B[r] - H.A[r] > direct_hull);
    return any;
}

template <class Row>
__device__ __forceinline__ void direct_rows(const uint2* __restrict__ cells, const GridDesc& g, uint32_t key, bool active,
                                            Row&& row) {
#pragma clang loop unroll(disable)
    for (int r = 0; r < 9; r++) {
        uint32_t l0, l1;
        lane_row_one(cells, g, key, active, r / 3 - 1, r % 3 - 1, l0, l1);
        const uint32_t len = l1 > l0 ? l1 - l0 : 0u;
        const uint32_t T = wave_max_u32(len);
        if (T) row(l0, len, T);
    }
}

struct Targets {
    uint32_t lo, hi, gap_lo, gap_len;
    const uint32_t* dev;
    uint32_t direct_hull;
    BlockOrder order;
};

__device__ __forceinline__ uint32_t pair_block() {
    const uint32_t rot = max(gridDim.x >> 6, 1u);
    return blockIdx.x < rot ? gridDim.x - rot + blockIdx.x : blockIdx.x - rot;
}

__device__ __forceinline__ bool wave_targets(const Targets& T, uint32_t wave, uint32_t lane, uint32_t& i, uint32_t& hi,
                                             uint32_t& first) {
    uint32_t lo = T.lo;
    hi = T.hi;
    if (T.dev) { lo = T.dev[0]; hi = T.dev[1]; }
    first = lo + (ordered_block(pair_block(), gridDim.x, T.order) * (blockDim.x >> 6) + wave) * WAVE;
    if (first >= T.gap_lo) first += T.gap_len;
    i = first + lane;
    return first < hi;
}

template <int THREADS>
__global__ __launch_bounds__(THREADS, SPH_DENS_OCC) void k_density(const float4* __restrict__ posi,
                                                                   const uint32_t* __restrict__ keyS,
                                                                   const uint2* __restrict__ cells,
                                                                   float2* __restrict__ dp, float2* __restrict__ cw,
                                                                   Targets tg, GridDesc g, Phys ph) {
    static_assert(UNROLL % 2 == 0, "the z-pair walk reads candidates two at a time");
    constexpr int DENS_ENT = lds_ent(THREADS);
    __shared__ float2 s_xy[DENS_ENT];
    __shared__ __attribute__((aligned(8))) float s_z[DENS_ENT];
    __shared__ __attribute__((aligned(8))) float s_zo_[DENS_ENT + 2];
    float* const s_zo = s_zo_ + 2;
    if (tg.dev && tg.dev[0] + ordered_block(pair_block(), gridDim.x, tg.order) * (uint32_t)THREADS >= tg.dev[1]) return;
    for (uint32_t k = threadIdx.x; k < DENS_ENT; k += THREADS) {
        s_xy[k] = make_float2(0.f, 0.f);
        s_z[k] = 0.f;
        s_zo_[k] = 0.f;
        if (k < 2u) s_zo_[DENS_ENT + k] = 0.f;
    }
    __syncthreads();
    const uint32_t wave = threadIdx.x >> 6, lane = threadIdx.x & 63u;
    const uint32_t slice = wave * PIECE;
    uint32_t i, tgt_hi, wave_first;
    if (!wave_targets(tg, wave, lane, i, tgt_hi, wave_first)) return;
    const bool active = i < tgt_hi;
    const uint32_t ii = active ? i : tgt_hi - 1;
    const float4 pi = posi[ii];
    Rows R;
    const uint32_t my_key = keyS[ii];
    lane_rows(cells, g, my_key, active, R);
    Hulls H;
    wave_hulls(R, H);
    float4 q0, q1;
    float acc = 0.f;
    const float h2_v = in_vgpr(ph.h2);
    auto pair_math = [&](float x, float y, float z, bool valid) {
        const float dx = pi.x - x, dy = pi.y - y, dz = pi.z - z;
        float d = fmaxf(fmaf(-dz, dz, fmaf(-dy, dy, fmaf(-dx, dx, h2_v))), 0.f);
        d = valid ? d : 0.f;
        acc = fmaf(d * d, d, acc);
    };
    auto finish = [&]() {
        if (active) {
            float rho = acc * ph.poly6_mass;
            float p = fmaxf(0.f, ph.gas_constant * (rho - ph.rest_density));
            dp[i] = make_float2(rho, p);
            cw[i] = neighbour_terms(ph, rho, p);
        }
    };
    if (wave_has_long_hull(H, my_key, tg.direct_hull)) {
        const uint32_t me = active ? i : tgt_hi - 1u;
        direct_rows(cells, g, keyS[me], active, [&](uint32_t l0, uint32_t len, uint32_t T) {
            for (uint32_t t = 0; t < T; t += 2u) {
                float4 q[2];
#pragma unroll
                for (uint32_t u = 0; u < 2u; u++) q[u] = posi[t + u < len ? l0 + t + u : me];
#pragma unroll
                for (uint32_t u = 0; u < 2u; u++) pair_math(q[u].x, q[u].y, q[u].z, t + u < len);
            }
        });
        finish();
        return;
    }
    traverse(
        H,
        [&](uint32_t a) {
            q0 = posi[a + lane];
            q1 = posi[a + WAVE + lane];
        },
        [&]() {
            s_xy[slice + lane] = make_float2(q0.x, q0.y);
            s_z[slice + lane] = q0.z;
            s_xy[slice + WAVE + lane] = make_float2(q1.x, q1.y);
            s_z[slice + WAVE + lane] = q1.z;
            s_zo[(int)(slice + lane) - 1] = q0.z;
            s_zo[slice + WAVE + lane - 1u] = q1.z;
        },
        [&](int r, uint32_t a, uint32_t b) {
            const uint32_t l0 = max(R.lo[r], a), l1 = min(R.hi[r], b);
            const uint32_t len = l1 > l0 ? l1 - l0 : 0u;
            const uint32_t rel = len ? l0 - a : 0u;
            uint32_t idx = slice + rel;
            const uint32_t tmin = wave_min_u32_uniform_first(len) & ~(uint32_t)(UNROLL - 1);
            lds_v2f_ptr zp = (lds_v2f_ptr)((rel & 1u) ? (const float*)s_zo : (const float*)s_z) + ((slice + rel) >> 1);
            auto group = [&](uint32_t t, bool check) {
#pragma unroll
                for (int u = 0; u < UNROLL; u += 2) {
                    const v2f xy0 = ((lds_v2f_ptr)s_xy)[idx + u], xy1 = ((lds_v2f_ptr)s_xy)[idx + u + 1];
                    const v2f zz = zp[u >> 1];
                    pair_math(xy0.x, xy0.y, zz.x, !check || t + u < len);
                    pair_math(xy1.x, xy1.y, zz.y, !check || t + u + 1 < len);
                }
                idx += UNROLL;
                zp += UNROLL / 2;
            };
            uint32_t t = 0;
            for (; t < tmin; t += UNROLL) group(t, false);
            for (; __ballot(t < len) != 0ull; t += UNROLL) group(t, true);
        });
    finish();
}

typedef _Float16 h2 __attribute__((ext_vector_type(2)));
typedef const volatile __attribute__((address_space(3))) h2* lds_h2_ptr;
typedef _Float16 h4 __attribute__((ext_vector_type(4)));
typedef const volatile __attribute__((address_space(3))) h4* lds_h4_ptr;

__device__ __forceinline__ h2 h2_splat(float x) { const _Float16 v = (_Float16)x; return h2{v, v}; }
__device__ __forceinline__ h2 h2_mask(bool lo, bool hi) {
    const uint32_t bits = (lo ? 0x3C00u : 0u) | (hi ? 0x3C000000u : 0u);
    return __builtin_bit_cast(h2, bits);
}

constexpr int HPAIRS = PIECE / 2;
constexpr int LDS_PAIRS = (PAIR_WAVES + 1) * HPAIRS + 8;
constexpr int HUNROLL = 4;

struct PairWalk {
    uint32_t idx;
    uint32_t whole;
    bool odd;
    uint32_t kmin, T;
};

__device__ __forceinline__ PairWalk pair_walk(uint32_t slice_pairs, uint32_t l0, uint32_t l1) {
    PairWalk w;
    const uint32_t len = l1 > l0 ? l1 - l0 : 0u;
    w.idx = (len && (l0 & 1u) ? (uint32_t)LDS_PAIRS : 0u) + slice_pairs + (len ? l0 >> 1 : 0u);
    w.whole = len >> 1;
    w.odd = (len & 1u) != 0u;
    uint32_t tmin;
    wave_min_max_u32(w.whole + (w.odd ? 1u : 0u), tmin, w.T);
    w.kmin = wave_min_u32_uniform_first(w.whole) & ~(uint32_t)(HUNROLL - 1);
    return w;
}

#ifndef SPH_DENSH_OCC
#define SPH_DENSH_OCC 5
#endif
#ifndef SPH_MIXED_SPAN
#define SPH_MIXED_SPAN 6.0f
#endif
#ifndef SPH_MIXED_XSPAN
#define SPH_MIXED_XSPAN 1000.0f
#endif
#ifndef SPH_MIXED_PASSES
#define SPH_MIXED_PASSES 3
#endif

__global__ __launch_bounds__(PAIR_THREADS, SPH_DENSH_OCC) void k_density_h(const float4* __restrict__ posi,
                                                                           const uint32_t* __restrict__ keyS,
                                                                           const uint2* __restrict__ cells,
                                                                           float2* __restrict__ dp, float2* __restrict__ cw,
                                                                           Targets tg, GridDesc g, Phys ph) {
    struct XY { h2 x, y; };
    struct ZL { h2 z, xl; };
    __shared__ XY s_xy[2 * LDS_PAIRS];
    __shared__ ZL s_zl[2 * LDS_PAIRS];
    const h2 zero = h2{(_Float16)0, (_Float16)0}, one = h2{(_Float16)1, (_Float16)1};
    for (uint32_t k = threadIdx.x; k < 2 * LDS_PAIRS; k += PAIR_THREADS) {
        s_xy[k].x = zero; s_xy[k].y = zero; s_zl[k].z = zero; s_zl[k].xl = zero;
    }
    __syncthreads();
    const uint32_t wave = threadIdx.x >> 6, lane = threadIdx.x & 63u;
    const uint32_t slice = wave * HPAIRS;
    uint32_t i, tgt_hi, wave_first;
    if (!wave_targets(tg, wave, lane, i, tgt_hi, wave_first)) return;
    const bool active = i < tgt_hi;
    const uint32_t ii = active ? i : tgt_hi - 1;
    const float4 pi = posi[ii];
    const uint32_t my_key = keyS[ii];
    const float inv_h = 1.0f / ph.h;
    float4 q0, q1, q2;
    float acc = 0.f;
    float acc32 = 0.f;

    auto serve = [&](bool in, float rx, float ry, float rz) {
        const float X = (pi.x - rx) * inv_h;
        const float Xc = rintf(X + X) * 0.5f;
        const h2 tx = h2_splat(Xc), txl = h2_splat(X - Xc);
        const h2 ty = h2_splat((pi.y - ry) * inv_h), tz = h2_splat((pi.z - rz) * inv_h);
        auto pair_math = [&](h2& row, h2 x, h2 xl, h2 y, h2 z, h2 m, bool masked) {
            const h2 dx = (tx - x) + (txl - xl), dy = ty - y, dz = tz - z;
            h2 t = one - dx * dx;
            t = t - dy * dy;
            t = t - dz * dz;
            t = __builtin_elementwise_max(t, zero);
            if (masked) t = t * m;
            row = row + (t * t) * t;
        };
        auto x_parts = [&](float qx, _Float16& hi, _Float16& lo) {
            const float v = (qx - rx) * inv_h;
            const float c = rintf(v + v) * 0.5f;
            hi = (_Float16)c;
            lo = (_Float16)(v - c);
        };
        Rows R;
        lane_rows(cells, g, my_key, in, R);
        Hulls H;
        wave_hulls(R, H);
        if (wave_has_long_hull(H, my_key, tg.direct_hull)) {
            direct_rows(cells, g, keyS[ii], in, [&](uint32_t l0, uint32_t len, uint32_t) {
                const uint32_t T = wave_max_u32((len + 1u) >> 1);
                h2 row = zero;
                for (uint32_t k = 0; k < T; k++) {
                    const bool v0 = 2u * k < len, v1 = 2u * k + 1u < len;
                    const float4 a = posi[v0 ? l0 + 2u * k : ii], b = posi[v1 ? l0 + 2u * k + 1u : ii];
                    _Float16 xa, xb, la, lb;
                    x_parts(a.x, xa, la);
                    x_parts(b.x, xb, lb);
                    const h2 x = h2{xa, xb}, xl = h2{la, lb};
                    const h2 y = h2{(_Float16)((a.y - ry) * inv_h), (_Float16)((b.y - ry) * inv_h)};
                    const h2 z = h2{(_Float16)((a.z - rz) * inv_h), (_Float16)((b.z - rz) * inv_h)};
                    pair_math(row, x, xl, y, z, h2_mask(v0, v1), true);
                }
                acc += (float)row.x + (float)row.y;
            });
            return;
        }
        traverse(
            H,
            [&](uint32_t a) {
                q0 = posi[a + 2u * lane];
                q1 = posi[a + 2u * lane + 1u];
                q2 = posi[a + 2u * lane + 2u];
            },
            [&]() {
                _Float16 x0, x1, x2, l0, l1, l2;
                x_parts(q0.x, x0, l0);
                x_parts(q1.x, x1, l1);
                x_parts(q2.x, x2, l2);
                const _Float16 y0 = (_Float16)((q0.y - ry) * inv_h), y1 = (_Float16)((q1.y - ry) * inv_h),
                               y2 = (_Float16)((q2.y - ry) * inv_h);
                const _Float16 z0 = (_Float16)((q0.z - rz) * inv_h), z1 = (_Float16)((q1.z - rz) * inv_h),
                               z2 = (_Float16)((q2.z - rz) * inv_h);
                s_xy[slice + lane].x = h2{x0, x1}; s_xy[slice + lane].y = h2{y0, y1};
                s_zl[slice + lane].z = h2{z0, z1}; s_zl[slice + lane].xl = h2{l0, l1};
                s_xy[LDS_PAIRS + slice + lane].x = h2{x1, x2}; s_xy[LDS_PAIRS + slice + lane].y = h2{y1, y2};
                s_zl[LDS_PAIRS + slice + lane].z = h2{z1, z2}; s_zl[LDS_PAIRS + slice + lane].xl = h2{l1, l2};
            },
            [&](int r, uint32_t a, uint32_t b) {
                const uint32_t l0 = max(R.lo[r], a), l1 = min(R.hi[r], b);
                const PairWalk w = pair_walk(slice, l1 > l0 ? l0 - a : 0u, l1 > l0 ? l1 - a : 0u);
                uint32_t idx = w.idx;
                h2 row = zero;
                auto pair = [&](int u, h2 m, bool masked) {
                    const h4 xy = ((lds_h4_ptr)s_xy)[idx + u], zl = ((lds_h4_ptr)s_zl)[idx + u];
                    pair_math(row, __builtin_shufflevector(xy, xy, 0, 1), __builtin_shufflevector(zl, zl, 2, 3),
                              __builtin_shufflevector(xy, xy, 2, 3), __builtin_shufflevector(zl, zl, 0, 1), m, masked);
                };
                uint32_t k = 0;
                for (; k < w.kmin; k += HUNROLL) {
#pragma unroll
                    for (int u = 0; u < HUNROLL; u++) pair(u, one, false);
                    idx += HUNROLL;
                }
                for (; k < w.T; k++) {
                    pair(0, h2_mask(k < w.whole + (w.odd ? 1u : 0u), k < w.whole), true);
                    idx++;
                }
                acc += (float)row.x + (float)row.y;
            });
    };

    constexpr float MIXED_SPAN = SPH_MIXED_SPAN;
    uint64_t todo = __ballot(active);
    for (int pass = 0; todo != 0ull; pass++) {
        if (pass == SPH_MIXED_PASSES) {
            const bool in = ((todo >> lane) & 1ull) != 0ull;
            const float h2_v = in_vgpr(ph.h2);
            direct_rows(cells, g, keyS[ii], in, [&](uint32_t l0, uint32_t len, uint32_t T) {
                for (uint32_t t = 0; t < T; t += 2u) {
                    float4 q[2];
#pragma unroll
                    for (uint32_t u = 0; u < 2u; u++) q[u] = posi[t + u < len ? l0 + t + u : ii];
#pragma unroll
                    for (uint32_t u = 0; u < 2u; u++) {
                        const float dx = pi.x - q[u].x, dy = pi.y - q[u].y, dz = pi.z - q[u].z;
                        float d = fmaxf(fmaf(-dz, dz, fmaf(-dy, dy, fmaf(-dx, dx, h2_v))), 0.f);
                        d = t + u < len ? d : 0.f;
                        acc32 = fmaf(d * d, d, acc32);
                    }
                }
            });
            break;
        }
        const int lead = __builtin_ctzll(todo);
        const float rx = __builtin_bit_cast(float, __builtin_amdgcn_readlane(__builtin_bit_cast(int, pi.x), lead)),
                    ry = __builtin_bit_cast(float, __builtin_amdgcn_readlane(__builtin_bit_cast(int, pi.y), lead)),
                    rz = __builtin_bit_cast(float, __builtin_amdgcn_readlane(__builtin_bit_cast(int, pi.z), lead));
        const float far = fmaxf(fabsf(pi.y - ry), fabsf(pi.z - rz)) * inv_h;
        const bool in = ((todo >> lane) & 1ull) != 0ull && far <= MIXED_SPAN &&
                        fabsf(pi.x - rx) * inv_h <= SPH_MIXED_XSPAN;
        todo &= ~__ballot(in);
        serve(in, rx, ry, rz);
    }
    if (active) {
        const float h2f = ph.h2;
        const float rho = fmaf(acc, ph.poly6_mass * (h2f * h2f * h2f), acc32 * ph.poly6_mass);
        const float p = fmaxf(0.f, ph.gas_constant * (rho - ph.rest_density));
        dp[i] = make_float2(rho, p);
        cw[i] = neighbour_terms(ph, rho, p);
    }
}

int launch_density_range(sph_ctx* c, uint32_t lo, uint32_t hi);
int launch_density(sph_ctx* c) {
    if (c->n == 0) return SPH_OK;
    return launch_density_range(c, c->own_off, c->own_off + c->n);
}

__device__ __forceinline__ void wall(float& x, float& v, float lo, float hi, float eps, float damp) {
    if (x - eps < lo) { x = lo + eps; v *= damp; }
    if (x + eps > hi) { x = hi - eps; v *= damp; }
}

__device__ __forceinline__ void push_out_of_spheres(const Phys& ph, float4& pi, float4& vi, const Spheres& sp) {
#pragma clang fp contract(off)
    bool inside = false;
    for (uint32_t j = 0; j < sp.n; j++) {
        const float dx = pi.x - sp.c[j].x, dy = pi.y - sp.c[j].y, dz = pi.z - sp.c[j].z;
        inside |= dx * dx + dy * dy + dz * dz < sp.u[j].w;
    }
    if (__ballot(inside) == 0ull) return;
    bool hit = false;
    for (uint32_t j = 0; j < sp.n; j++) {
        const float dx = pi.x - sp.c[j].x, dy = pi.y - sp.c[j].y, dz = pi.z - sp.c[j].z;
        const float r2 = dx * dx + dy * dy + dz * dz;
        if (r2 < sp.u[j].w) {
            float nx = 0.f, ny = 1.f, nz = 0.f;
            if (r2 > 0.f) {
                const float r = sqrtf(r2);
                nx = dx / r; ny = dy / r; nz = dz / r;
            }
            const float rp = sp.c[j].w;
            pi.x = sp.c[j].x + rp * nx;
            pi.y = sp.c[j].y + rp * ny;
            pi.z = sp.c[j].z + rp * nz;
            const float wn = (vi.x - sp.u[j].x) * nx + (vi.y - sp.u[j].y) * ny + (vi.z - sp.u[j].z) * nz;
            if (wn < 0.f) {
                const float k = (ph.wall_damping - 1.f) * wn;
                vi.x += k * nx; vi.y += k * ny; vi.z += k * nz;
            }
            hit = true;
        }
    }
    if (hit) {
        wall(pi.x, vi.x, ph.box_min[0], ph.box_max[0], ph.wall_eps, ph.wall_damping);
        wall(pi.y, vi.y, ph.box_min[1], ph.box_max[1], ph.wall_eps, ph.wall_damping);
        wall(pi.z, vi.z, ph.box_min[2], ph.box_max[2], ph.wall_eps, ph.wall_damping);
    }
}

template <class... Sph>
__device__ __forceinline__ void integrate_one(const Phys& ph, float dt, float4& pi, float4& vi, float rho, float fx,
                                              float fy, float fz, float dvx, float dvy, float dvz, const Sph&... sp) {
    fy += ph.gravity_y * rho;
#if SPH_EXACT_DIV
    float ax = fx / rho, ay = fy / rho, az = fz / rho;
#else
    const float ir = __builtin_amdgcn_rcpf(rho);
    float ax = fx * ir, ay = fy * ir, az = fz * ir;
#endif
    vi.x += dt * ax + dvx;
    vi.y += dt * ay + dvy;
    vi.z += dt * az + dvz;
    pi.x += dt * vi.x;
    pi.y += dt * vi.y;
    pi.z += dt * vi.z;
    const float e = ph.wall_eps;
    const bool near_wall = pi.x - e < ph.box_min[0] || pi.x + e > ph.box_max[0] || pi.y - e < ph.box_min[1] || pi.y + e > ph.box_max[1] ||
                           pi.z - e < ph.box_min[2] || pi.z + e > ph.box_max[2];
    if (__ballot(near_wall) != 0ull) {
        wall(pi.x, vi.x, ph.box_min[0], ph.box_max[0], ph.wall_eps, ph.wall_damping);
        wall(pi.y, vi.y, ph.box_min[1], ph.box_max[1], ph.wall_eps, ph.wall_damping);
        wall(pi.z, vi.z, ph.box_min[2], ph.box_max[2], ph.wall_eps, ph.wall_damping);
    }
    if constexpr (sizeof...(Sph) > 0) push_out_of_spheres(ph, pi, vi, sp...);
}

#ifdef SPH_PAIR_STATS
__device__ unsigned long long g_pair_stats[12];
__device__ int g_pair_stats_on;
#define PAIR_STAT(k, v) do { if (lane == 0 && g_pair_stats_on) atomicAdd(&g_pair_stats[k], (unsigned long long)(v)); } while (0)
extern "C" void sph_debug_pair_stats(unsigned long long* out, int on) {
    (void)hipDeviceSynchronize();
    (void)hipMemcpyFromSymbol(out, HIP_SYMBOL(g_pair_stats), sizeof(g_pair_stats));
    unsigned long long z[12] = {};
    (void)hipMemcpyToSymbol(HIP_SYMBOL(g_pair_stats), z, sizeof(z));
    (void)hipMemcpyToSymbol(HIP_SYMBOL(g_pair_stats_on), &on, sizeof(on));
}
#else
#define PAIR_STAT(k, v) do { } while (0)
#endif
template <bool FORCE, bool COLL, bool INTEG, int THREADS, class... Sph>
__global__ __launch_bounds__(THREADS, SPH_FORCE_OCC) void k_force(
    const float4* __restrict__ posi, const float4* __restrict__ velr, const float2* __restrict__ dp,
    const float2* __restrict__ cw, const uint32_t* __restrict__ keyS, const uint2* __restrict__ cells, float4* __restrict__ fpress,
    float4* __restrict__ fvisc, float4* __restrict__ dvel, float4* __restrict__ posi_out,
    float4* __restrict__ velr_out, float4* __restrict__ pos_by_index, uint32_t* __restrict__ keys_out,
    uint64_t* __restrict__ mm_mask, uint32_t* __restrict__ mm_tile_cnt, Targets tg,
    uint32_t slot0, float dt, GridDesc g, Phys ph, Sph... sp) {
    constexpr int E2 = 5;
    constexpr int ENT = lds_ent(THREADS);
    __shared__ float2 s_e[ENT * 5];
    if (tg.dev && tg.dev[0] + ordered_block(pair_block(), gridDim.x, tg.order) * (uint32_t)THREADS >= tg.dev[1]) return;
    for (uint32_t k = threadIdx.x; k < ENT * E2; k += THREADS)
        s_e[k] = make_float2(0.f, 0.f);
    __syncthreads();
    const uint32_t wave = threadIdx.x >> 6, lane = threadIdx.x & 63u;
    const uint32_t slice = wave * PIECE;
    uint32_t i, tgt_hi, wave_first;
    if (!wave_targets(tg, wave, lane, i, tgt_hi, wave_first)) return;
    const bool active = i < tgt_hi;
    const uint32_t ii = active ? i : tgt_hi - 1;
    float4 pi = posi[ii];
    float4 vi = velr[ii];
    const float2 dpi = dp[ii];
    Rows R;
    const uint32_t my_key = keyS[ii];
    lane_rows(cells, g, my_key, active, R);
    Hulls H;
    wave_hulls(R, H);
    PAIR_STAT(0, 1);
#ifdef SPH_PAIR_STATS
    {
        uint32_t hmax = 0;
        for (int r = 0; r < 9; r++) hmax = max(hmax, H.B[r] > H.A[r] ? H.B[r] - H.A[r] : 0u);
        PAIR_STAT(5, hmax > 256u ? 1 : 0); PAIR_STAT(6, hmax > 512u ? 1 : 0); PAIR_STAT(7, hmax > 2048u ? 1 : 0);
    }
#endif
    float4 q0, q1, w0, w1;
    float2 e0, e1;
    const float cpi = ph.cp_scale * dpi.y;
    const float h_v = in_vgpr(ph.h);
    const float coll_next_v = in_vgpr(__uint_as_float(__float_as_uint(ph.coll_dist2) + 8u));
    float fpx = 0.f, fpy = 0.f, fpz = 0.f, fvx = 0.f, fvy = 0.f, fvz = 0.f, sw = 0.f;
    float cvx = 0.f, cvy = 0.f, cvz = 0.f;
    uint32_t ccount = 0;
#ifdef SPH_PAIR_STATS
    uint32_t stat_near = 0;
#endif
    auto pair_math = [&](float qx, float qy, float qz, float ux, float uy, float uz, float cpj, float wj, bool valid) -> float {
        const float dx = pi.x - qx, dy = pi.y - qy, dz = pi.z - qz;
        float r2 = fmaf(dz, dz, fmaf(dx, dx, fmaf(dy, dy, 1e-30f)));
        r2 = valid ? r2 : 1e30f;
        if (FORCE) {
            const float rinv = inv_sqrt(r2);
            const float hr = fmaxf(fmaf(-r2, rinv, h_v), 0.f);
            const float w = wj * hr;
            const float s = (cpi + cpj) * w * (hr * rinv);
            fpx += s * dx; fpy += s * dy; fpz += s * dz;
            fvx += w * ux; fvy += w * uy; fvz += w * uz;
            sw += w;
        }
        return r2 - coll_next_v;
    };
    auto collide_math = [&](float qx, float qy, float qz, float wx, float wy, float wz) {
        const float dx = pi.x - qx, dy = pi.y - qy, dz = pi.z - qz;
        const float ux = wx - vi.x, uy = wy - vi.y, uz = wz - vi.z;
        float r2c, dot;
        {
#pragma clang fp contract(off)
            r2c = dx * dx + (dy * dy + dz * dz);
            dot = -(dx * ux + (dy * uy + dz * uz));
        }
        const bool hit = r2c <= ph.coll_dist2 && dot < 0.f;
        const float cfac = hit ? ph.coll_mass * dot * __builtin_amdgcn_rcpf(r2c) : 0.f;
        cvx += cfac * dx; cvy += cfac * dy; cvz += cfac * dz;
        ccount += hit ? 1u : 0u;
    };
    auto finish = [&]() {
#ifdef SPH_PAIR_STATS
        if (COLL) {
            const uint32_t busiest = wave_max_u32(stat_near);
            PAIR_STAT(8, busiest);
            uint32_t sum = stat_near;
            for (int off = 32; off; off >>= 1) sum += (uint32_t)__shfl_xor((int)sum, off);
            PAIR_STAT(9, sum);
        }
#endif
        if (FORCE) {
            fvx = fmaf(-vi.x, sw, fvx) * ph.visc_on; fvy = fmaf(-vi.y, sw, fvy) * ph.visc_on; fvz = fmaf(-vi.z, sw, fvz) * ph.visc_on;
        }
        bool moved = false;
        if (active) {
            float dvx = 0.f, dvy = 0.f, dvz = 0.f;
            if (COLL) {
#if SPH_EXACT_DIV
                const float den = ph.mass * (float)(1u + ccount);
                dvx = -cvx / den; dvy = -cvy / den; dvz = -cvz / den;
#else
                const float nid = -__builtin_amdgcn_rcpf(ph.mass * (float)(1u + ccount));
                dvx = cvx * nid; dvy = cvy * nid; dvz = cvz * nid;
#endif
            }
            if (INTEG) {
                integrate_one(ph, dt, pi, vi, dpi.x, fpx + fvx, fpy + fvy, fpz + fvz, dvx, dvy, dvz, sp...);
                posi_out[i] = pi;
                velr_out[i] = vi;
                if (pos_by_index) pos_by_index[__float_as_uint(pi.w)] = make_float4(pi.x, pi.y, pi.z, 1.0f);
                const uint32_t key = cell_key(g, pi.x, pi.y, pi.z);
                keys_out[i - slot0] = key;
                if (mm_mask) moved = key != keyS[i];
            } else {
                if (FORCE) {
                    fpress[i] = make_float4(fpx, fpy, fpz, 0.f);
                    fvisc[i] = make_float4(fvx, fvy, fvz, 0.f);
                }
                if (COLL) dvel[i] = make_float4(dvx, dvy, dvz, __uint_as_float(ccount));
            }
        }
        if (INTEG && mm_mask) {
            const uint64_t m = __ballot(moved);
            const uint32_t chunk = (wave_first - slot0) >> 6;
            if (lane == 0) {
                mm_mask[chunk] = m;
                if (m) atomicAdd(&mm_tile_cnt[chunk / MM_TILE_CHUNKS], (uint32_t)__popcll(m));
            }
        }
    };
    if (wave_has_long_hull(H, my_key, tg.direct_hull)) {
        const uint32_t me = active ? i : tgt_hi - 1u;
        direct_rows(cells, g, keyS[me], active, [&](uint32_t l0, uint32_t len, uint32_t T) {
            for (uint32_t t = 0; t < T; t++) {
                const bool valid = t < len;
                const uint32_t j = valid ? l0 + t : me;
                const float4 q = posi[j], w = velr[j];
                float2 e = make_float2(0.f, 0.f);
                if (FORCE) e = cw[j];
                const float tt = pair_math(q.x, q.y, q.z, w.x, w.y, w.z, e.x, e.y, valid);
                if (COLL && __ballot(tt < 0.f) != 0ull) {
                    if (tt < 0.f) collide_math(q.x, q.y, q.z, w.x, w.y, w.z);
                }
            }
        });
        finish();
        return;
    }
    traverse(
        H,
        [&](uint32_t a) {
            q0 = posi[a + lane]; q1 = posi[a + WAVE + lane];
            w0 = velr[a + lane]; w1 = velr[a + WAVE + lane];
            if (FORCE) { e0 = cw[a + lane]; e1 = cw[a + WAVE + lane]; }
        },
        [&]() {
            float2* e0p = &s_e[(slice + lane) * 5];
            float2* e1p = &s_e[(slice + WAVE + lane) * 5];
            e0p[0] = make_float2(q0.x, q0.y);
            e0p[1] = make_float2(q0.z, w0.x);
            e0p[2] = make_float2(w0.y, w0.z);
            e1p[0] = make_float2(q1.x, q1.y);
            e1p[1] = make_float2(q1.z, w1.x);
            e1p[2] = make_float2(w1.y, w1.z);
            if (FORCE) {
                e0p[3] = e0;
                e1p[3] = e1;
            }
        },
        [&](int r, uint32_t a, uint32_t b) {
            const uint32_t l0 = max(R.lo[r], a), l1 = min(R.hi[r], b);
            const uint32_t len = l1 > l0 ? l1 - l0 : 0u;
            uint32_t T, tmin_raw;
            wave_min_max_u32(len, tmin_raw, T);
            uint32_t idx = slice + (len ? l0 - a : 0u);
            const uint32_t tmin = tmin_raw & ~(uint32_t)(SPH_FORCE_UNROLL - 1);
            uint32_t near = 0u;
            PAIR_STAT(1, 1); PAIR_STAT(2, T);
            auto pair = [&](int u, bool valid) {
                const lds_v2f_ptr e = (lds_v2f_ptr)s_e + (idx + u) * 5;
                const v2f qa = e[0], qb = e[1];
                v2f qc = {0.f, 0.f}, qd = {0.f, 0.f};
                if (FORCE) { qc = e[2]; qd = e[3]; }
                const float t = pair_math(qa.x, qa.y, qb.x, qb.y, qc.x, qc.y, qd.x, qd.y, valid);
                if (COLL) near = __builtin_amdgcn_alignbit(near, __float_as_uint(t), 31);
            };
            for (uint32_t t0 = 0; t0 < T; t0 += 32u) {
                const uint32_t tend = min(T, t0 + 32u);
                const uint32_t tsafe = min(tend, max(tmin, t0));
                const uint32_t idx0 = idx;
                uint32_t done = 0u;
                near = 0u;
                PAIR_STAT(3, 1);
                uint32_t t = t0;
                for (; t < tsafe; t += SPH_FORCE_UNROLL) {
#pragma unroll
                    for (int u = 0; u < SPH_FORCE_UNROLL; u++) pair(u, true);
                    idx += SPH_FORCE_UNROLL;
                    done += SPH_FORCE_UNROLL;
                }
                for (; t < tend; t += SPH_FORCE_UNROLL) {
#pragma unroll
                    for (int u = 0; u < SPH_FORCE_UNROLL; u++) pair(u, t + u < len);
                    idx += SPH_FORCE_UNROLL;
                    done += SPH_FORCE_UNROLL;
                }
#ifdef SPH_PAIR_STATS
                if (COLL) stat_near += (uint32_t)__popc(near);
#endif
                if (COLL) {
                    while (__ballot(near != 0u) != 0ull) {
                        PAIR_STAT(4, 1);
                        if (near != 0u) {
                            const uint32_t hb = 31u - (uint32_t)__clz((int)near);
                            near &= ~(1u << hb);
                            const uint32_t ci = idx0 + (done - 1u - hb);
                            const float2* e = &s_e[(ci << 2) + ci];
                            const float2 qa = e[0], qb = e[1], qc = e[2];
                            collide_math(qa.x, qa.y, qb.x, qb.y, qc.x, qc.y);
                        }
                    }
                }
            }
        });
    finish();
}

static BlockOrder block_order(const sph_ctx* c, uint32_t nblocks, bool ztile) {
    BlockOrder o{c->order_xcd ? 1u : 0u, 0u, 0u, 0u, c->order_xrot ? 1u : 0u};
    if (!o.xcd || !ztile || !c->order_ztile || nblocks < 1024u) return o;
    const uint32_t k0 = c->mm_count_host[1], k1 = c->mm_count_host[2], layer = c->grid.g[0] * c->grid.g[1];
    if (k1 < k0 || layer == 0u) return o;
    const uint32_t nz = k1 / layer - k0 / layer + 1u;
    const uint32_t per_layer = nblocks / nz;
    if (per_layer < 32u) return o;
    uint32_t lb_sh = 31u - (uint32_t)__builtin_clz(per_layer);
    if ((per_layer >> lb_sh) && (per_layer - (1u << lb_sh)) > (1u << lb_sh) / 2u) lb_sh++;
    const uint32_t q = nblocks >> 3, nl = q >> lb_sh;
    if (nl < 2u) return o;
    o.lb_sh = lb_sh; o.s_sh = c->order_strip_sh; o.nl_sh = 31u - (uint32_t)__builtin_clz(nl);
    if (o.s_sh >= o.lb_sh) o.nl_sh = 0u;
    return o;
}

static Targets targets_with_hole(uint32_t lo, uint32_t hi, uint32_t hole_lo, uint32_t hole_hi, uint32_t& threads) {
    Targets t{lo, hi, hi, 0u, nullptr, 0u, BlockOrder{0u, 0u, 0u, 0u, 0u}};
    threads = hi - lo;
    if (hole_lo < lo) hole_lo = lo;
    if (hole_hi > hi) hole_hi = hi;
    if (hole_lo < hole_hi) {
        const uint32_t g0 = lo + ((hole_lo - lo + 63u) & ~63u);
        if (g0 < hole_hi) { t.gap_lo = g0; t.gap_len = hole_hi - g0; threads -= t.gap_len; }
    }
    return t;
}

static Spheres sphere_table(const sph_ctx* c) {
    Spheres t{};
    const float eps = c->params.wall_eps;
    for (uint32_t j = 0; j < c->n_colliders; j++) {
        const sph_collider& s = c->colliders[j];
        const float rp = s.radius + eps;
        t.c[j] = make_float4(s.center[0], s.center[1], s.center[2], rp);
        t.u[j] = make_float4(s.velocity[0], s.velocity[1], s.velocity[2], rp * rp);
    }
    t.n = c->n_colliders;
    return t;
}

template <bool F, bool C, bool I, class... Sph>
static void force_kernel(sph_ctx* c, bool small, const Targets& tg, uint32_t threads, float dt, bool mark, Sph... sp) {
#define SPH_LAUNCH_FORCE_T(T)                                                                                                   \
    hipLaunchKernelGGL((k_force<F, C, I, T, Sph...>), dim3(ceil_div(threads, (uint32_t)T)), dim3(T), 0, c->stream, c->posi,       \
                       c->velr, c->dp, c->cw, c->keyS, c->cells, c->fpress, c->fvisc, c->dvel, c->posi2, c->velr2,                \
                       c->slab ? nullptr : c->pos_out, c->k0, mark ? c->mm_mask : nullptr, c->mm_tile_cnt, tg, c->own_off, dt, \
                       c->grid, c->phys, sp...)
    if (small) SPH_LAUNCH_FORCE_T(SMALL_THREADS_PAIR); else SPH_LAUNCH_FORCE_T(PAIR_THREADS);
#undef SPH_LAUNCH_FORCE_T
}

static void advance_colliders(sph_ctx* c, float dt) {
#pragma clang fp contract(off)
    for (uint32_t j = 0; j < c->n_colliders; j++)
        for (int a = 0; a < 3; a++) c->colliders[j].center[a] = c->colliders[j].center[a] + dt * c->colliders[j].velocity[a];
}

int launch_force_hole(sph_ctx* c, uint32_t lo, uint32_t hi, uint32_t hole_lo, uint32_t hole_hi, bool force, bool collide,
                      bool integrate, float dt, bool mark) {
    if (hi <= lo) return SPH_OK;
    SPH_REQUIRE(((lo - c->own_off) & 63u) == 0u, SPH_E_INVALID, "force sub-range does not start on a 64-slot chunk");
    uint32_t threads;
    Targets tg = targets_with_hole(lo, hi, hole_lo, hole_hi, threads);
    tg.direct_hull = c->direct_hull;
    const bool small = small_blocks(c);
    const uint32_t bt = small ? (uint32_t)SMALL_THREADS_PAIR : (uint32_t)PAIR_THREADS;
    tg.order = block_order(c, ceil_div(threads, bt), integrate && force);
    SPH_REQUIRE(tg.gap_len == 0u || (((tg.gap_lo - lo) | tg.gap_len) & 63u) == 0u || tg.gap_lo + tg.gap_len == hi, SPH_E_INVALID,
                "force hole is not made of whole 64-slot chunks");
    if (threads == 0) return SPH_OK;
    if (force && collide && integrate) {
        if (c->n_colliders) force_kernel<true, true, true>(c, small, tg, threads, dt, mark, sphere_table(c));
        else force_kernel<true, true, true>(c, small, tg, threads, dt, mark);
    } else if (force && !collide && !integrate) force_kernel<true, false, false>(c, small, tg, threads, dt, mark);
    else if (!force && collide && !integrate) force_kernel<false, true, false>(c, small, tg, threads, dt, mark);
    else {
        set_error("launch_force: unsupported combination");
        return SPH_E_INVALID;
    }
    SPH_HIP(hipGetLastError());
    return SPH_OK;
}

int launch_force_dev_range(sph_ctx* c, const uint32_t* range_dev, uint32_t max_count, float dt) {
    if (max_count == 0) return SPH_OK;
    const Targets tg{0u, 0u, 0xFFFFFFFFu, 0u, range_dev, c->direct_hull, BlockOrder{0u, 0u, 0u, 0u, 0u}};
#define SPH_LAUNCH_EARLY(T, ...)                                                                                                    \
    hipLaunchKernelGGL((k_force<true, true, true, T __VA_OPT__(, ) __VA_ARGS__>), dim3(ceil_div(max_count, (uint32_t)T)), dim3(T), 0,   \
                       c->stream, c->posi, c->velr, c->dp, c->cw, c->keyS, c->cells, c->fpress, c->fvisc, c->dvel, c->posi2, c->velr2,  \
                       c->slab ? nullptr : c->pos_out, c->keyS2, (uint64_t*)nullptr, c->mm_tile_cnt, tg, 0u, dt, c->grid, c->phys      \
                       __VA_OPT__(, sphere_table(c)))
    if (c->n_colliders) {
        if (small_blocks(c)) SPH_LAUNCH_EARLY(SMALL_THREADS_PAIR, Spheres); else SPH_LAUNCH_EARLY(PAIR_THREADS, Spheres);
    } else {
        if (small_blocks(c)) SPH_LAUNCH_EARLY(SMALL_THREADS_PAIR); else SPH_LAUNCH_EARLY(PAIR_THREADS);
    }
#undef SPH_LAUNCH_EARLY
    SPH_HIP(hipGetLastError());
    return SPH_OK;
}

int launch_force_range(sph_ctx* c, uint32_t lo, uint32_t hi, bool force, bool collide, bool integrate, float dt, bool mark) {
    return launch_force_hole(c, lo, hi, hi, hi, force, collide, integrate, dt, mark);
}

bool force_begin(sph_ctx* c, bool integrate) {
    if (integrate) mm_drop_marks(c);
    return integrate && c->sort_merge && c->order_valid;
}

void force_finish(sph_ctx* c, bool integrate, bool mark, float dt) {
    if (!integrate) return;
    advance_colliders(c, dt);
    float4* t;
    t = c->posi; c->posi = c->posi2; c->posi2 = t;
    t = c->velr; c->velr = c->velr2; c->velr2 = t;
    c->keys_fresh = true;
    if (mark) {
        c->mm_marked = true; c->mm_scanned = false; c->mm_marked_off = c->own_off; c->mm_marked_n = c->n;
        mm_scan_marks(c);
    }
}

int launch_force(sph_ctx* c, bool force, bool collide, bool integrate, float dt) {
    if (c->n == 0) {
        if (integrate) advance_colliders(c, dt);
        return SPH_OK;
    }
    const bool mark = force_begin(c, integrate);
    int rc = launch_force_range(c, c->own_off, c->own_off + c->n, force, collide, integrate, dt, mark);
    if (rc) return rc;
    force_finish(c, integrate, mark, dt);
    return SPH_OK;
}

static int launch_density_targets(sph_ctx* c, const Targets& tg, uint32_t threads) {
    if (threads == 0) return SPH_OK;
    if (c->precision == SPH_PRECISION_MIXED_F16)
        hipLaunchKernelGGL(k_density_h, dim3(ceil_div(threads, PAIR_THREADS)), dim3(PAIR_THREADS), 0, c->stream, c->posi,
                           c->keyS, c->cells, c->dp, c->cw, tg, c->grid, c->phys);
    else if (small_blocks(c))
        hipLaunchKernelGGL(k_density<SMALL_THREADS_PAIR>, dim3(ceil_div(threads, (uint32_t)SMALL_THREADS_PAIR)), dim3(SMALL_THREADS_PAIR), 0, c->stream,
                           c->posi, c->keyS, c->cells, c->dp, c->cw, tg, c->grid, c->phys);
    else
        hipLaunchKernelGGL(k_density<DENS_THREADS>, dim3(ceil_div(threads, (uint32_t)DENS_THREADS)), dim3(DENS_THREADS), 0, c->stream, c->posi,
                           c->keyS, c->cells, c->dp, c->cw, tg, c->grid, c->phys);
    SPH_HIP(hipGetLastError());
    return SPH_OK;
}

int launch_density_hole(sph_ctx* c, uint32_t lo, uint32_t hi, uint32_t hole_lo, uint32_t hole_hi) {
    if (hi <= lo) return SPH_OK;
    uint32_t threads;
    Targets tg = targets_with_hole(lo, hi, hole_lo, hole_hi, threads);
    tg.direct_hull = c->direct_hull;
    const uint32_t bt = c->precision == SPH_PRECISION_MIXED_F16 ? (uint32_t)PAIR_THREADS : (small_blocks(c) ? (uint32_t)SMALL_THREADS_PAIR : (uint32_t)DENS_THREADS);
    tg.order = block_order(c, ceil_div(threads, bt), c->order_ztile_dens);
    return launch_density_targets(c, tg, threads);
}

int launch_density_range(sph_ctx* c, uint32_t lo, uint32_t hi) { return launch_density_hole(c, lo, hi, hi, hi); }

int launch_density_dev_range(sph_ctx* c, const uint32_t* range_dev, uint32_t max_count) {
    const Targets tg{0u, 0u, 0xFFFFFFFFu, 0u, range_dev, c->direct_hull, BlockOrder{0u, 0u, 0u, 0u, 0u}};
    return launch_density_targets(c, tg, max_count);
}

template <class... Sph>
__global__ __launch_bounds__(256) void k_integrate(float4* __restrict__ posi, float4* __restrict__ velr,
                                                   const float2* __restrict__ dp, const float4* __restrict__ fpress,
                                                   const float4* __restrict__ fvisc, const float4* __restrict__ dvel,
                                                   float4* __restrict__ pos_by_index, uint32_t lo, uint32_t hi, float dt,
                                                   Phys ph, Sph... sp) {
    uint32_t i = lo + blockIdx.x * 256u + threadIdx.x;
    if (i >= hi) return;
    float4 pi = posi[i], vi = velr[i];
    const float4 fp = fpress[i], fv = fvisc[i], dv = dvel[i];
    integrate_one(ph, dt, pi, vi, dp[i].x, fp.x + fv.x, fp.y + fv.y, fp.z + fv.z, dv.x, dv.y, dv.z, sp...);
    posi[i] = pi;
    velr[i] = vi;
    if (pos_by_index) pos_by_index[__float_as_uint(pi.w)] = make_float4(pi.x, pi.y, pi.z, 1.0f);
}

int launch_integrate(sph_ctx* c, float dt) {
    if (c->n == 0) {
        advance_colliders(c, dt);
        return SPH_OK;
    }
    float4* const pos_out = c->slab ? nullptr : c->pos_out;
    if (c->n_colliders)
        hipLaunchKernelGGL(k_integrate<Spheres>, dim3(ceil_div(c->n, 256)), dim3(256), 0, c->stream, c->posi, c->velr, c->dp,
                           c->fpress, c->fvisc, c->dvel, pos_out, c->own_off, c->own_off + c->n, dt, c->phys, sphere_table(c));
    else
        hipLaunchKernelGGL(k_integrate<>, dim3(ceil_div(c->n, 256)), dim3(256), 0, c->stream, c->posi, c->velr, c->dp,
                           c->fpress, c->fvisc, c->dvel, pos_out, c->own_off, c->own_off + c->n, dt, c->phys);
    SPH_HIP(hipGetLastError());
    advance_colliders(c, dt);
    return SPH_OK;
}

}
```

### gpufluidsimulator_amd/csrc/sph_sort.hip

```cpp
#include "sph_device.hpp"

#include <atomic>
#include <chrono>

namespace sph {

constexpr int SORT_THREADS = 256;
#ifndef SPH_SORT_KPT
#define SPH_SORT_KPT 16
#endif
constexpr int SORT_KPT = SPH_SORT_KPT;
constexpr int SORT_TILE = SORT_THREADS * SORT_KPT;

__global__ __launch_bounds__(256) void k_hash(const float4* __restrict__ posi, uint32_t n, GridDesc g,
                                              uint32_t* __restrict__ keys) {
    uint32_t i = blockIdx.x * 256u + threadIdx.x;
    if (i >= n) return;
    float4 p = posi[i];
    keys[i] = cell_key(g, p.x, p.y, p.z);
}

constexpr int OS_TILE = SORT_TILE;
#ifndef SPH_OS_GROUP
#define SPH_OS_GROUP 16
// ... 821 lines not shown
    }
}

constexpr uint32_t MM_FUSED_SCAN_TILES = 2048;
__global__ __launch_bounds__(256) void k_mm_compact(const uint64_t* __restrict__ mask, uint32_t nchunks, uint32_t n_old,
                                                    const uint32_t* __restrict__ tile_off, const uint32_t* __restrict__ tile_cnt,
                                                    uint32_t nt, uint32_t* __restrict__ m_dev, volatile uint32_t* __restrict__ m_host,
                                                    unsigned long long* __restrict__ m_total,
                                                    const uint32_t* __restrict__ A, const uint32_t* __restrict__ B,
                                                    uint32_t* __restrict__ M64, uint32_t* __restrict__ mk,
                                                    uint32_t* __restrict__ mi, uint2* __restrict__ cells,
                                                    const uint32_t* __restrict__ keys_abs, uint32_t g0lo, uint32_t g0hi,
                                                    uint32_t g1lo, uint32_t g1hi) {
    if (blockIdx.x >= nt) {
        const uint32_t t = (blockIdx.x - nt) * 256u + threadIdx.x, n0 = g0hi - g0lo;
        const uint32_t lo = t < n0 ? g0lo : g1lo, hi = t < n0 ? g0hi : g1hi;
        const uint32_t s = t < n0 ? g0lo + t : g1lo + (t - n0);
        if (s >= hi) return;
        const uint32_t k = keys_abs[s];
        if (s == lo || keys_abs[s - 1] != k) cells[k] = make_uint2(0u, 0u);
        return;
    }
    __shared__ uint32_t part[256];
    uint32_t tile_start;
    if (tile_cnt) {
        uint32_t below = 0, all = 0;
        for (uint32_t t = threadIdx.x; t < nt; t += 256u) { const uint32_t v = tile_cnt[t]; all += v; below += t < blockIdx.x ? v : 0u; }
#pragma unroll
        for (int off = 32; off; off >>= 1) { below += (uint32_t)__shfl_xor((int)below, off); all += (uint32_t)__shfl_xor((int)all, off); }
        if ((threadIdx.x & 63u) == 0u) { part[threadIdx.x >> 6] = below; part[4 + (threadIdx.x >> 6)] = all; }
        __syncthreads();
        tile_start = part[0] + part[1] + part[2] + part[3];
        if (blockIdx.x == 0 && threadIdx.x == 0) {
            const uint32_t m = part[4] + part[5] + part[6] + part[7];
            *m_dev = m; *m_host = m;
            if (m_total) *m_total += m;
        }
        __syncthreads();
    } else {
        tile_start = tile_off[blockIdx.x];
    }
    const uint32_t chunk = blockIdx.x * MM_TILE_CHUNKS + threadIdx.x;
    uint64_t m = chunk < nchunks ? mask[chunk] : 0ull;
    const uint32_t cnt = (uint32_t)__popcll(m);
    part[threadIdx.x] = cnt;
    __syncthreads();
    for (int off = 1; off < 256; off <<= 1) {
        uint32_t v = threadIdx.x >= (uint32_t)off ? part[threadIdx.x - off] : 0u;
        __syncthreads();
        part[threadIdx.x] += v;
        __syncthreads();
    }
    if (chunk >= nchunks) return;
    uint32_t at = tile_start + part[threadIdx.x] - cnt;
    M64[chunk] = at;
    while (m) {
        const uint32_t i = chunk * 64u + (uint32_t)__builtin_ctzll(m);
        m &= m - 1ull;
        mk[at] = B[i];
        mi[at] = i;
        at++;
        if (cells && i < n_old) cells[A[i]] = make_uint2(0u, 0u);
    }
}

__device__ __forceinline__ uint32_t mm_lower_bound(const uint32_t* __restrict__ mk, const uint32_t* __restrict__ mi,
                                                   uint32_t lo, uint32_t hi, uint32_t key, uint32_t slot, Front f) {
    while (lo < hi) {
        const uint32_t mid = lo + ((hi - lo) >> 1);
        const uint32_t k = mk[mid];
        const bool less = k < key || (k == key && mover_slot_less(mi[mid], slot, f));
        if (less) lo = mid + 1; else hi = mid;
    }
    return lo;
}

constexpr uint32_t MM_RANK_TILE = 4096;
__global__ __launch_bounds__(256) void k_mm_tile_rank(const uint32_t* __restrict__ A, uint32_t n,
                                                      const uint32_t* __restrict__ mk, const uint32_t* __restrict__ mi,
                                                      const uint32_t* __restrict__ m_dev, uint32_t* __restrict__ tileL,
                                                      uint32_t* __restrict__ tileA, bool small_too, uint32_t small_max,
                                                      Front front) {
    const uint32_t t = blockIdx.x * 256u + threadIdx.x;
    const uint32_t ntiles = (n + MM_RANK_TILE - 1) / MM_RANK_TILE;
    if (t > ntiles) return;
    const uint32_t m = *m_dev;
    if (small_too && m <= small_max) return;
    const uint32_t slot = t * MM_RANK_TILE;
    const uint32_t a = t == ntiles ? 0xFFFFFFFFu : A[slot];
    tileA[t] = a;
    tileL[t] = t == ntiles ? m : mm_lower_bound(mk, mi, 0u, m, a, slot, front);
}

__device__ __forceinline__ void mm_scatter_body(uint32_t bid, const uint32_t* __restrict__ A, uint32_t n,
                                                const uint64_t* __restrict__ mask, const uint32_t* __restrict__ M64,
                                                const uint32_t* __restrict__ mk, const uint32_t* __restrict__ mi,
                                                const uint32_t* __restrict__ tileL, const float4* __restrict__ posi,
                                                const float4* __restrict__ velr, float4* __restrict__ posi_out,
                                                float4* __restrict__ velr_out, uint32_t* __restrict__ key_out,
                                                uint32_t* __restrict__ perm_out, Front front) {
    const uint32_t i = bid * 256u + threadIdx.x;
    const uint32_t first = __builtin_amdgcn_readfirstlane(i);
    if (first >= n) return;
    const uint32_t lane = threadIdx.x & 63u;
    const uint32_t chunk = first >> 6;
    const uint32_t last = min(first + 63u, n - 1u);
    const uint32_t tile = first / MM_RANK_TILE;
    const uint32_t b0 = tileL[tile], b1 = tileL[tile + 1];
    uint32_t L0 = b0, L1 = b0;
    if (b0 != b1) {
        L0 = mm_lower_bound(mk, mi, b0, b1, A[first], first, front);
        L1 = mm_lower_bound(mk, mi, L0, b1, A[last], last, front);
    }
    if (i >= n) return;
    const uint64_t bits = mask[chunk];
    if ((bits >> lane) & 1ull) return;
    const uint32_t key = A[i];
    const uint32_t before = M64[chunk] + (uint32_t)__popcll(bits & ((1ull << lane) - 1ull));
    const uint32_t L = L0 == L1 ? L0 : mm_lower_bound(mk, mi, L0, L1, key, i, front);
    const uint32_t dst = i - before + L;
    posi_out[dst] = posi[i];
    velr_out[dst] = velr[i];
    key_out[dst] = key;
    if (perm_out) perm_out[dst] = i;
}

__device__ __forceinline__ void mm_place_body(uint32_t bid, uint32_t nblocks, const uint32_t* __restrict__ A, uint32_t n,
                                              uint32_t nchunks, const uint64_t* __restrict__ mask,
                                              const uint32_t* __restrict__ M64, const uint32_t* __restrict__ mk,
                                              const uint32_t* __restrict__ mi, const uint32_t* __restrict__ m_dev,
                                              const uint32_t* __restrict__ tileA, const uint2* __restrict__ cells,
                                              uint32_t slot_base, const float4* __restrict__ posi,
                                              const float4* __restrict__ velr, float4* __restrict__ posi_out,
                                              float4* __restrict__ velr_out, uint32_t* __restrict__ key_out,
                                              uint32_t* __restrict__ perm_out, Front front) {
    const uint32_t m = *m_dev;
    const uint32_t ntiles = (n + MM_RANK_TILE - 1) / MM_RANK_TILE;
    for (uint32_t r = bid * 256u + threadIdx.x; r < m; r += nblocks * 256u) {
        const uint32_t key = mk[r], slot = mi[r];
        uint32_t s, e;
        uint2 ce = make_uint2(0u, 0u);
        if (cells) ce = cells[key];
        if (ce.y > ce.x) {
            s = ce.x - slot_base; e = ce.y - slot_base;
        } else {
            uint32_t lo = 0, hi = ntiles;
            while (lo < hi) { const uint32_t mid = lo + ((hi - lo) >> 1); if (tileA[mid] < key) lo = mid + 1; else hi = mid; }
            uint32_t a = lo ? (lo - 1u) * MM_RANK_TILE : 0u, b = min(lo * MM_RANK_TILE, n);
            while (a < b) { const uint32_t mid = a + ((b - a) >> 1); if (A[mid] < key) a = mid + 1; else b = mid; }
            s = a;
            uint32_t step = 1u, p = s;
            while (p < n && A[p] == key) { p = min(p + step, n); step <<= 1; }
            uint32_t q = p > s ? max(s, p - (step >> 1)) : s;
            a = q; b = p;
            while (a < b) { const uint32_t mid = a + ((b - a) >> 1); if (A[mid] <= key) a = mid + 1; else b = mid; }
            e = a;
        }
        const uint32_t j = slot - front.lo < front.cnt ? s : min(max(slot, s), e);
        uint32_t before = m;
        if ((j >> 6) < nchunks) before = M64[j >> 6] + (uint32_t)__popcll(mask[j >> 6] & ((1ull << (j & 63u)) - 1ull));
        const uint32_t dst = r + (j - before);
        posi_out[dst] = posi[slot];
        velr_out[dst] = velr[slot];
        key_out[dst] = key;
        if (perm_out) perm_out[dst] = slot;
    }
}

__global__ __launch_bounds__(256) void k_mm_move(uint32_t place_blocks, uint32_t* __restrict__ zero_cnt, uint32_t zero_n,
                                                 const uint32_t* __restrict__ A, uint32_t n,
                                                 uint32_t nchunks, const uint64_t* __restrict__ mask,
                                                 const uint32_t* __restrict__ M64, const uint32_t* __restrict__ mk,
                                                 const uint32_t* __restrict__ mi, const uint32_t* __restrict__ m_dev,
                                                 const uint32_t* __restrict__ tileL, const uint32_t* __restrict__ tileA,
                                                 const uint2* __restrict__ cells, uint32_t slot_base,
                                                 const float4* __restrict__ posi, const float4* __restrict__ velr,
                                                 float4* __restrict__ posi_out, float4* __restrict__ velr_out,
                                                 uint32_t* __restrict__ key_out, uint32_t* __restrict__ perm_out, Front front) {
    if (zero_cnt && blockIdx.x * 256u + threadIdx.x < zero_n) zero_cnt[blockIdx.x * 256u + threadIdx.x] = 0u;
    if (blockIdx.x < place_blocks)
        mm_place_body(blockIdx.x, place_blocks, A, n, nchunks, mask, M64, mk, mi, m_dev, tileA, cells, slot_base, posi, velr,
                      posi_out, velr_out, key_out, perm_out, front);
    else
        mm_scatter_body(blockIdx.x - place_blocks, A, n, mask, M64, mk, mi, tileL, posi, velr, posi_out, velr_out, key_out,
                        perm_out, front);
}

static uint32_t merge_grid_for(uint32_t movers_hint, uint32_t n) {
    const uint32_t want = max(ceil_div(2u * movers_hint + 1u, SORT_TILE) + 15u, OS_ONE_GROUP_TILES);
    return min(want, max(ceil_div(n, SORT_TILE), 1u));
}

static void mm_tilescan(sph_ctx* c, uint32_t n, bool counted) {
    const uint32_t nt = ceil_div(ceil_div(n, 64u), MM_TILE_CHUNKS);
    uint32_t seq = 0u;
    if (counted) { if (++c->scan_seq_issued == 0u) c->scan_seq_issued = 1u; seq = c->scan_seq_issued; }
    hipLaunchKernelGGL(k_mm_tilescan, dim3(1), dim3(1024), 0, c->stream, c->mm_tile_cnt, nt, c->mm_tile_off, c->mm_count,
                       c->mm_count_host_dev, counted ? c->mm_total : (unsigned long long*)nullptr, seq);
    c->mm_counted_valid = counted;
}

static uint32_t mm_tiles(uint32_t n) { return ceil_div(ceil_div(n, 64u), MM_TILE_CHUNKS); }

void mm_scan_marks(sph_ctx* c) {
    if (!c->mm_marked || c->mm_scanned) return;
    if (*c->mm_count_host != 0u && mm_tiles(c->mm_marked_n) <= MM_FUSED_SCAN_TILES) return;
    mm_tilescan(c, c->mm_marked_n, true);
    c->mm_scanned = true;
}

void mm_drop_marks(sph_ctx* c) {
    if (!c->mm_marked) return;
    if (!c->mm_scanned) mm_tilescan(c, c->mm_marked_n, false);
    c->mm_marked = false;
    c->mm_scanned = false;
}

static bool launch_merge_count(sph_ctx* c, uint32_t n) {
    if (c->mm_marked && !(c->mm_marked_off == c->own_off && c->mm_marked_n == n)) mm_drop_marks(c);
    if (!c->mm_marked) {
        hipLaunchKernelGGL(k_mm_mark, dim3(ceil_div(n, 256)), dim3(256), 0, c->stream, c->keyS + c->own_off, c->k0, n,
                           c->mm_mask, c->mm_tile_cnt);
        c->mm_scanned = false;
    }
    bool in_compact = false;
    if (!c->mm_scanned) {
        if (mm_tiles(n) <= MM_FUSED_SCAN_TILES) { in_compact = true; c->mm_counted_valid = false; }
        else mm_tilescan(c, n, true);
    }
    c->mm_marked = false;
    c->mm_scanned = false;
    return in_compact;
}

__global__ __launch_bounds__(256) void k_mm_mark_tail(uint32_t n_old, uint32_t n_tot, uint64_t* __restrict__ mask,
                                                      uint32_t* __restrict__ tile_cnt) {
    const uint32_t chunk = blockIdx.x * 256u + threadIdx.x;
    if (chunk * 64u >= n_tot) return;
    const uint32_t lo = chunk * 64u, hi = min(lo + 64u, n_tot);
    uint64_t m = 0ull;
    if (hi > n_old) {
        const uint32_t first = max(lo, n_old) - lo, cnt = hi - lo;
        m = (cnt == 64u ? ~0ull : ((1ull << cnt) - 1ull)) & ~((1ull << first) - 1ull);
        atomicAdd(&tile_cnt[chunk / MM_TILE_CHUNKS], (uint32_t)__popcll(m));
    }
    mask[chunk] = m;
}

static int launch_sort_merge(sph_ctx* c, uint32_t n, uint32_t n_tot, bool table_live, uint32_t hint, Front front = Front{0u, 0u},
                             bool count_in_compact = false, const uint32_t* ghost_clear = nullptr) {
    const uint32_t* A = c->keyS + c->own_off;
    const uint32_t* B = c->k0;
    const uint32_t nchunks = ceil_div(n_tot, 64u), nt = ceil_div(nchunks, MM_TILE_CHUNKS);
    uint32_t* mk = c->mm_k0; uint32_t* mi = c->v0; uint32_t* mk2 = c->mm_k1; uint32_t* mi2 = c->mm_v1;
    const uint32_t gc[4] = {ghost_clear ? ghost_clear[0] : 0u, ghost_clear ? ghost_clear[1] : 0u, ghost_clear ? ghost_clear[2] : 0u,
                            ghost_clear ? ghost_clear[3] : 0u};
    const uint32_t gc_blocks = ceil_div((gc[1] - gc[0]) + (gc[3] - gc[2]), 256u);
    hipLaunchKernelGGL(k_mm_compact, dim3(nt + gc_blocks), dim3(256), 0, c->stream, c->mm_mask, nchunks, n, c->mm_tile_off,
                       count_in_compact ? c->mm_tile_cnt : (const uint32_t*)nullptr, nt, c->mm_count, c->mm_count_host_dev, c->mm_total, A, B,
                       c->mm_M64, mk, mi, table_live ? c->cells : (uint2*)nullptr, c->keyS, gc[0], gc[1], gc[2], gc[3]);
    SPH_HIP(hipGetLastError());
    SmallTail tail;
    int form = SORT_FORM_BOTH;
    tail.A = A; tail.n_slots = n; tail.front = front; tail.hint = hint; tail.form = &form;
    int rc = radix_sort_pairs(c, n_tot, c->mm_count, merge_grid_for(hint, n_tot), false, mk, mi, mk2, mi2, tail);
    if (rc) return rc;
    if (form != SORT_FORM_SMALL) {
        const uint32_t rank_tiles = ceil_div(n, MM_RANK_TILE) + 1u;
        hipLaunchKernelGGL(k_mm_tile_rank, dim3(ceil_div(rank_tiles, 256u)), dim3(256), 0, c->stream, A, n, mk, mi, c->mm_count,
                           c->mm_tileL, c->mm_tileA, form == SORT_FORM_BOTH, OS_SMALL_MAX, front);
        SPH_HIP(hipGetLastError());
    }
    uint32_t* perm = c->keep_perm ? c->v1 : (uint32_t*)nullptr;
    const float4* ps = c->posi + c->own_off; const float4* vs = c->velr + c->own_off;
    float4* po = c->posi2 + c->gcap; float4* vo = c->velr2 + c->gcap; uint32_t* ko = c->keyS2 + c->gcap;
    const uint32_t place_blocks = min(max(ceil_div(2u * hint + 1u, 256u) + 15u, 512u), 65535u);
    hipLaunchKernelGGL(k_mm_move, dim3(place_blocks + ceil_div(n, 256)), dim3(256), 0, c->stream, place_blocks,
                       count_in_compact ? c->mm_tile_cnt : (uint32_t*)nullptr, nt, A, n, nchunks,
                       c->mm_mask, c->mm_M64, mk, mi, c->mm_count, c->mm_tileL, c->mm_tileA,
                       table_live ? c->cells : (const uint2*)nullptr, c->own_off, ps, vs, po, vo, ko, perm, front);
    SPH_HIP(hipGetLastError());
    c->last_perm = perm;
    return SPH_OK;
}

static int sort_throttle(sph_ctx* c) {
    volatile const uint32_t* hw = c->mm_count_host;
    if ((int32_t)(c->sort_seq_issued - hw[3]) < 4) return SPH_OK;
    const auto t0 = std::chrono::steady_clock::now();
    for (uint32_t spins = 1; (int32_t)(c->sort_seq_issued - hw[3]) >= 4; spins++) {
        __builtin_ia32_pause();
        if ((spins & 0xFFFu) == 0u) {
            const hipError_t q = hipStreamQuery(c->stream);
            if (q == hipSuccess) break;
            if (q != hipErrorNotReady) SPH_HIP(q);
            SPH_REQUIRE(std::chrono::duration<double>(std::chrono::steady_clock::now() - t0).count() < 300.0, SPH_E_DEVICE,
                        "sort: the device has not reached the table build of sort %u after 300 s", c->sort_seq_issued - 3u);
        }
    }
    return SPH_OK;
}

int launch_sort(sph_ctx* c) {
    const uint32_t n = c->n;
    if (n == 0) return SPH_OK;
    const uint32_t nblocks = ceil_div(n, SORT_TILE);
    SPH_REQUIRE(nblocks <= c->sort_blocks_cap, SPH_E_CAPACITY, "sort: %u blocks > capacity %u", nblocks,
                c->sort_blocks_cap);
    if (c->sort_merge && !c->host_paced) { const int rc = sort_throttle(c); if (rc) return rc; }
    c->sort_calls++;
    c->last_sort_skipped = false;
    const bool can_merge = c->sort_merge && c->order_valid;
    const bool table_live = c->cells_clear_deferred && c->cells_valid;
    c->cells_clear_deferred = false;
    const bool ghosts_left = c->ghost_clear_pending && table_live;
    c->ghost_clear_pending = false;
    if (can_merge && (*c->mm_count_host <= n / 8u || c->sort_merge_always)) {
        const bool was_still = *c->mm_count_host == 0u;
        const bool count_in_compact = launch_merge_count(c, n);
        if (was_still && table_live && c->own_off == c->gcap && !count_in_compact) {
            volatile const uint32_t* hw = c->mm_count_host;
            if (c->mm_counted_valid && hw[4] == c->scan_seq_issued && (std::atomic_thread_fence(std::memory_order_acquire), hw[0] == 0u)) {
                c->sort_merges++;
                c->sort_skips++;
                c->last_sort_skipped = true;
                c->last_perm = nullptr;
                c->order_valid = true;
                if (ghosts_left) {
                    const int rc2 = launch_cells_clear_2ranges(c, c->ghost_clear[0], c->ghost_clear[1], c->ghost_clear[2], c->ghost_clear[3]);
                    if (rc2) return rc2;
                    c->cells_lo = c->own_off; c->cells_hi = c->own_off + n;
                }
                return SPH_OK;
            }
        }
        int rc = launch_sort_merge(c, n, n, table_live, *c->mm_count_host, Front{0u, 0u}, count_in_compact,
                                   ghosts_left ? c->ghost_clear : (const uint32_t*)nullptr);
        if (rc) return rc;
        c->sort_merges++;
        if (c->cells_valid && !table_live) {
            rc = launch_cells_clear(c);
            if (rc) return rc;
        }
    } else {
        if (c->cells_valid) {
            int rc = launch_cells_clear(c);
            if (rc) return rc;
        }
        if (c->mm_marked) {
            if (!c->mm_scanned) mm_tilescan(c, c->mm_marked_n, true);
            c->mm_marked = false;
            c->mm_scanned = false;
        } else if (can_merge && (c->sort_calls & 7u) == 0) {
            hipLaunchKernelGGL(k_mm_mark, dim3(ceil_div(n, 256)), dim3(256), 0, c->stream, c->keyS + c->own_off, c->k0, n,
                               c->mm_mask, c->mm_tile_cnt);
            mm_tilescan(c, n, true);
            SPH_HIP(hipGetLastError());
        }
        uint32_t* kin = c->k0; uint32_t* vin = c->v0;
        uint32_t* kout = c->k1; uint32_t* vout = c->v1;
        int rc = radix_sort_pairs(c, n, nullptr, nblocks, true, kin, vin, kout, vout);
        if (rc) return rc;
        hipLaunchKernelGGL(k_reorder, dim3(ceil_div(n, 256)), dim3(256), 0, c->stream, kin, vin, n, c->posi + c->own_off,
                           c->velr + c->own_off, c->posi2 + c->gcap, c->velr2 + c->gcap, c->keyS2 + c->gcap);
        SPH_HIP(hipGetLastError());
        c->last_perm = vin;
    }
    float4* t4;
    t4 = c->posi; c->posi = c->posi2; c->posi2 = t4;
    t4 = c->velr; c->velr = c->velr2; c->velr2 = t4;
    uint32_t* tk = c->keyS; c->keyS = c->keyS2; c->keyS2 = tk;
    c->own_off = c->gcap;
    c->cells_valid = false;
    if (++c->sort_seq_issued == 0u) c->sort_seq_issued = 1u;
    c->cells_seq_next = c->sort_seq_issued;
    if (c->owned_cells_in_bounds) {
        c->owned_cells_pending = true;
        c->cells_seq_next = 0u;
    } else {
        int rc = launch_cells_build_range(c, c->gcap, c->gcap + n);
        if (rc) return rc;
    }
    c->order_valid = true;
    c->cells_lo = c->gcap; c->cells_hi = c->gcap + n; c->cells_valid = true;
    return SPH_OK;
}

int launch_merge_arrivals(sph_ctx* c, uint32_t n_in, uint32_t n_front) {
    const uint32_t n = c->n, n_tot = n + n_in;
    SPH_REQUIRE(c->order_valid && c->cells_valid && c->cells_lo == c->own_off && c->cells_hi == c->own_off + n, SPH_E_STATE,
                "launch_merge_arrivals needs the sorted owned range and its cell table");
    SPH_REQUIRE(ceil_div(n_tot, SORT_TILE) <= c->sort_blocks_cap, SPH_E_CAPACITY, "sort: capacity exceeded");
    mm_drop_marks(c);
    const uint32_t nchunks = ceil_div(n_tot, 64u);
    hipLaunchKernelGGL(k_mm_mark_tail, dim3(ceil_div(nchunks, 256u)), dim3(256), 0, c->stream, n, n_tot, c->mm_mask,
                       c->mm_tile_cnt);
    const uint32_t nt = ceil_div(nchunks, MM_TILE_CHUNKS);
    hipLaunchKernelGGL(k_mm_tilescan, dim3(1), dim3(1024), 0, c->stream, c->mm_tile_cnt, nt, c->mm_tile_off, c->mm_count,
                       c->mm_count_host_dev, (unsigned long long*)nullptr, 0u);
    c->mm_counted_valid = false;
    SPH_HIP(hipGetLastError());
    int rc = launch_sort_merge(c, n, n_tot, true, n_in, Front{n, n_front < n_in ? n_front : n_in});
    if (rc) return rc;
    float4* t4;
    t4 = c->posi; c->posi = c->posi2; c->posi2 = t4;
    t4 = c->velr; c->velr = c->velr2; c->velr2 = t4;
    uint32_t* tk = c->keyS; c->keyS = c->keyS2; c->keyS2 = tk;
    c->own_off = c->gcap;
    c->n = n_tot;
    c->cells_valid = false;
    rc = launch_cells_build_range(c, c->gcap, c->gcap + n_tot);
    if (rc) return rc;
    c->cells_lo = c->gcap; c->cells_hi = c->gcap + n_tot; c->cells_valid = true;
    c->order_valid = true;
    c->keys_fresh = false;
    c->n_glo = c->n_ghi = 0;
    c->stage = sph_ctx::ST_SORTED;
    c->have_dens = c->have_force = c->have_coll = false;
    return SPH_OK;
}

const uint32_t* last_sort_permutation(sph_ctx* c) { return c->last_perm; }

int sort_indices_by_key(sph_ctx* c, const uint32_t* keys_dev, uint32_t n, uint32_t bits, const uint32_t** perm_out) {
    *perm_out = nullptr;
    if (n == 0) return SPH_OK;
    const uint32_t nblocks = ceil_div(n, SORT_TILE);
    SPH_REQUIRE(nblocks <= c->sort_blocks_cap && n <= c->cap, SPH_E_CAPACITY, "sort: %u keys > capacity %u", n, c->cap);
    SPH_HIP(hipMemcpyAsync(c->k0, keys_dev, (size_t)n * sizeof(uint32_t), hipMemcpyDeviceToDevice, c->stream));
    uint32_t* kin = c->k0; uint32_t* vin = c->v0;
    uint32_t* kout = c->k1; uint32_t* vout = c->v1;
    const uint32_t saved = c->key_bits;
    c->key_bits = bits;
    const int rc = radix_sort_pairs(c, n, nullptr, nblocks, true, kin, vin, kout, vout);
    c->key_bits = saved;
    if (rc) return rc;
    c->keys_fresh = false;
    c->last_perm = nullptr;
    *perm_out = vin;
    return SPH_OK;
}

}
```

### include/sph_hip.h

```cpp
#ifndef SPH_HIP_H
#define SPH_HIP_H

#include <stddef.h>
#include <stdint.h>

#ifdef __cplusplus
extern "C" {
#endif

#define SPH_ABI_VERSION 2

enum {
    SPH_OK = 0,
    SPH_E_INVALID = -1,
    SPH_E_DEVICE = -2,
    SPH_E_NOMEM = -3,
    SPH_E_CAPACITY = -4,
    SPH_E_STATE = -5,
    SPH_E_PEER = -6
};

typedef struct sph_ctx sph_ctx;

typedef struct sph_params {
    float box_min[3];
    float box_max[3];
    uint32_t grid[3];
    float h;
    float mass;
    float rest_density;
    float gas_constant;
    float viscosity;
    float gravity_y;
    float wall_eps;
    float wall_damping;
    float restitution;
    float collision_param;
    float particle_radius;
} sph_params;

enum {
    SPH_PH_ZINDEX = 0,
    SPH_PH_SORT,
    SPH_PH_BGRID,
    SPH_PH_DENS,
    SPH_PH_FORCE,
    SPH_PH_COLLISION,
    SPH_PH_INTEGRATE,
    SPH_PH_COUNT
};

int sph_abi_version(void);
const char* sph_last_error(void);
int sph_device_count(int* is_gfx950);

int sph_select_device(int device);
int sph_selected_device(void);

void sph_default_params(sph_params* p, const float box_dims[3], const uint32_t grid[3]);
uint32_t sph_grid_dim_for_edge(float edge, float h);

int sph_create(sph_ctx** out, int device, uint32_t capacity, const sph_params* p);
int sph_create_slab(sph_ctx** out, int device, uint32_t capacity, const sph_params* p,
                    uint32_t z_lo, uint32_t z_hi, uint32_t ghost_capacity);
int sph_create_slab_layers(sph_ctx** out, int device, uint32_t capacity, const sph_params* p,
                           uint32_t z_lo, uint32_t z_hi, uint32_t ghost_capacity, uint32_t ghost_layers);
uint32_t sph_ghost_layers(const sph_ctx* c);
void sph_destroy(sph_ctx* c);
int sph_set_stream(sph_ctx* c, void* hip_stream);
int sph_set_params(sph_ctx* c, const sph_params* p);
int sph_get_params(const sph_ctx* c, sph_params* p);
int sph_sync(sph_ctx* c);
uint32_t sph_num_particles(const sph_ctx* c);
uint32_t sph_capacity(const sph_ctx* c);

enum { SPH_PRECISION_F32 = 0, SPH_PRECISION_MIXED_F16 = 1 };
int sph_set_precision(sph_ctx* c, int precision);
int sph_get_precision(const sph_ctx* c);

int sph_upload(sph_ctx* c, uint32_t n, const float* pos_xyz, const float* vel_xyz, const uint32_t* index);
int sph_set_by_index(sph_ctx* c, uint32_t first_index, uint32_t count, const float* pos_xyz, const float* vel_xyz);
int sph_reset_lattice(sph_ctx* c, const uint32_t lattice[3], int jitter, const float jitter_dims[3],
                      uint64_t index_start, uint32_t count);
int sph_download(sph_ctx* c, uint32_t index_base, uint32_t index_count, float* pos_xyz, float* vel_xyz, float* density,
                 float* pressure);
int sph_download_owned(sph_ctx* c, float* pos_xyz, float* vel_xyz, uint32_t* index);
 int sph_download_forces(sph_ctx* c, uint32_t index_base, uint32_t index_count, float* fpress_xyz, float* fvisc_xyz,
                        float* dv_xyz, int32_t* collision_count);
int sph_positions_dev(sph_ctx* c, void** out_dev);
int sph_download_positions4(sph_ctx* c, float* pos_xyzw);

#define SPH_MAX_COLLIDERS 8
typedef struct sph_collider {
    float center[3];
    float radius;
    float velocity[3];
    float pad;
} sph_collider;
int sph_set_colliders(sph_ctx* c, uint32_t n, const sph_collider* colliders);
int sph_get_colliders(const sph_ctx* c, uint32_t* n, sph_collider* out);

int sph_snapshot_save(sph_ctx* c, const char* path);
int sph_snapshot_load(sph_ctx* c, const char* path);
int sph_snapshot_info(const char* path, uint32_t* n, sph_params* p);

 int sph_get_keys(sph_ctx* c, uint32_t* keys);
 int sph_get_order(sph_ctx* c, uint32_t* index);
 int sph_get_cell_range(sph_ctx* c, uint32_t cell, uint32_t* start, uint32_t* end);
 int sph_get_cells(sph_ctx* c, uint32_t max_cells, uint32_t* key, uint32_t* start, uint32_t* count);
 uint32_t sph_cell_key(const sph_ctx* c, uint32_t x, uint32_t y, uint32_t z);

int sph_hash(sph_ctx* c);
int sph_sort(sph_ctx* c);
int sph_build_cells(sph_ctx* c);
int sph_density(sph_ctx* c);
int sph_force(sph_ctx* c);
int sph_collide(sph_ctx* c);
int sph_integrate(sph_ctx* c, float dt);
int sph_step(sph_ctx* c, float dt, uint32_t n_steps);
int sph_step_phased(sph_ctx* c, float dt, uint32_t n_steps);
int sph_force_collide_integrate(sph_ctx* c, float dt);

int sph_timing_enable(sph_ctx* c, int on);
int sph_timing_get(sph_ctx* c, float ms[SPH_PH_COUNT], uint32_t* n_steps);
int sph_timing_reset(sph_ctx* c);
 int sph_sort_stats(sph_ctx* c, uint64_t* sorts, uint64_t* merges, uint64_t* skips, uint32_t* last_movers,
                   uint64_t* movers_total);
 int sph_sort_forms(const sph_ctx* c, uint64_t out[3]);
 int sph_set_sort_mode(sph_ctx* c, int merge);
 int sph_set_direct_hull(sph_ctx* c, uint32_t slots);
 int sph_set_pair_small_launch(sph_ctx* c, uint32_t slots);
 int sph_set_block_order(sph_ctx* c, int xcd, int ztile, uint32_t strip_blocks_log2);
 int sph_last_sort_skipped(const sph_ctx* c);

#define SPH_HALO_RECORD_FLOATS 8
int sph_migrants_count(sph_ctx* c, uint32_t count[2]);
int sph_slab_counts(sph_ctx* c, uint32_t count[4]);
int sph_migrants_pack(sph_ctx* c, void* buf_dev[2], uint32_t capacity);
int sph_migrants_append(sph_ctx* c, const void* buf_dev, uint32_t n);
int sph_halo_count(sph_ctx* c, uint32_t count[2]);
int sph_halo_pack(sph_ctx* c, void* buf_dev[2], uint32_t capacity);
int sph_halo_pack_counts(sph_ctx* c, void* buf_dev[2], uint32_t capacity, const uint32_t count[2]);
int sph_halo_unpack(sph_ctx* c, const void* lo_dev, uint32_t n_lo, const void* hi_dev, uint32_t n_hi);
int sph_halo_pack_density(sph_ctx* c, void* buf_dev[2], uint32_t capacity);
int sph_halo_unpack_density(sph_ctx* c, const void* lo_dev, const void* hi_dev);
int sph_layer_histogram(sph_ctx* c, uint32_t* hist, uint32_t n_layers);

enum { SPH_TAG_MIGRANTS = 1, SPH_TAG_HALO_A = 2, SPH_TAG_HALO_B = 3, SPH_TAG_MIGRANTS_REST = 4, SPH_TAG_PING = 5,
       SPH_TAG_RECUT_COUNTS = 6, SPH_TAG_RECUT = 7,
       SPH_TAG_ONE = 8,
       SPH_TAG_ONE_REST = 9 };
typedef struct sph_transport {
    void* self;
    int (*exchange)(void* self, int tag, const void* send_lo, size_t send_lo_bytes, void* recv_lo, size_t recv_lo_bytes,
                    const void* send_hi, size_t send_hi_bytes, void* recv_hi, size_t recv_hi_bytes, void* hip_stream);
    int host_buffers;
    void (*abort)(void* self);
} sph_transport;

int sph_rccl_unique_id(uint8_t id[128]);
int sph_rccl_transport_create(sph_transport** out, const uint8_t id[128], int rank, int world, int device);
void sph_rccl_transport_destroy(sph_transport* t);
 int sph_rccl_transport_selftest(sph_transport* t, size_t bytes);
 int sph_rccl_transport_info(const sph_transport* t, int out[4]);

typedef struct sph_local_hub sph_local_hub;
int sph_local_hub_create(sph_local_hub** out, int world, int device);
void sph_local_hub_destroy(sph_local_hub* hub);
int sph_local_hub_set_timeout(sph_local_hub* hub, double seconds);
int sph_local_transport_create(sph_transport** out, sph_local_hub* hub, int rank);
void sph_local_transport_destroy(sph_transport* t);

 int sph_loop_transport_create(sph_transport** out, float z_shift, double link_gbs, double latency_us);
 void sph_loop_transport_destroy(sph_transport* t);

typedef struct sph_slab sph_slab;
int sph_slab_create(sph_slab** out, sph_ctx* ctx, int rank, int world, const sph_transport* transport,
                    uint32_t migrant_capacity);
void sph_slab_destroy(sph_slab* s);
int sph_slab_step(sph_slab* s, float dt, uint32_t n_steps);
int sph_slab_sync(sph_slab* s);
int sph_slab_set_wait_timeout(sph_slab* s, double seconds);
 int sph_slab_stats(const sph_slab* s, uint64_t out[5]);
 int sph_slab_counters(const sph_slab* s, uint64_t out[8]);
 uint64_t sph_slab_in_place_merges(const sph_slab* s);
 uint64_t sph_slab_exchanges(const sph_slab* s);
int sph_slab_recut(sph_slab* s, uint32_t new_z_lo, uint32_t new_z_hi);
 int sph_slab_recut_stats(const sph_slab* s, uint64_t out[2]);
int sph_slab_ping(sph_slab* s, size_t bytes, uint32_t reps, double out[3]);
enum {
    SPH_SLAB_T_STEPS = 0, SPH_SLAB_T_WAITS_READY = 1,
    SPH_SLAB_T_WAIT = 2,
    SPH_SLAB_T_PRE = 4, SPH_SLAB_T_POST = 6, SPH_SLAB_T_HOST = 8,
    SPH_SLAB_T_GROUPS = 10,
    SPH_SLAB_T_GROUPS_ONE = 22,
    SPH_SLAB_T_WORDS = 28
};
int sph_slab_timing_enable(sph_slab* s, int on);
int sph_slab_timing_reset(sph_slab* s);
int sph_slab_timing_get(sph_slab* s, double out[SPH_SLAB_T_WORDS]);
 int sph_slab_set_early_force(sph_slab* s, int on);
int sph_slab_set_protocol(sph_slab* s, int groups);
 int sph_slab_protocol(const sph_slab* s, uint64_t out[3]);
 int sph_slab_early_force_stats(const sph_slab* s, uint64_t out[2]);
 int sph_test_trust_mover_hint(sph_ctx* c);
 int sph_slab_test_raise_flag(sph_slab* s, int flag);
int sph_slab_failed(const sph_slab* s);

#ifdef __cplusplus
}
#endif
#endif
```

Before: 4.291 billion particle-steps/s.

## Hand off packed neighbour-row ranges from density kernel to force kernel

The density kernel now writes each lane's nine neighbour-row ranges, packed as 16-bit offsets relative to per-wave hulls, plus the wave hulls into new device buffers. The force kernel reads these back instead of recomputing lane_rows and wave_hulls from the cell table. A generation counter, bumped on every state change such as sort, cell rebuild or integrate, decides whether the cached rows are still valid. The change removes the repeated cell-table lookups and hull reductions in force, at the cost of 9 extra 32-bit stores and loads per particle, about 600 MB of extra memory, and a fallback to the direct path when a hull does not fit in 16 bits.

```diff
diff --git a/gpufluidsimulator_amd/capi.py b/gpufluidsimulator_amd/capi.py
--- a/gpufluidsimulator_amd/capi.py
+++ b/gpufluidsimulator_amd/capi.py
@@ -103,6 +103,8 @@
     "sph_set_block_order": (C.c_int, [_P, C.c_int, C.c_int, C.c_uint32]),
     "sph_sort_forms": (C.c_int, [_P, C.POINTER(C.c_uint64)]),
     "sph_test_trust_mover_hint": (C.c_int, [_P]),
+    "sph_test_set_row_handoff": (C.c_int, [_P, C.c_int]),
+    "sph_test_row_handoff_launches": (C.c_uint64, [_P]),
     "sph_set_precision": (C.c_int, [_P, C.c_int]),
     "sph_get_precision": (C.c_int, [_P]),
     "sph_migrants_count": (C.c_int, [_P, C.POINTER(_U32)]),
@@ -422,6 +424,12 @@
     def trust_mover_hint(self):
         _check(self.L.sph_test_trust_mover_hint(self.h))
 
+    def set_row_handoff(self, on=True):
+        _check(self.L.sph_test_set_row_handoff(self.h, 1 if on else 0))
+
+    def row_handoff_launches(self):
+        return int(self.L.sph_test_row_handoff_launches(self.h))
+
     def sort_forms(self):
         out = (C.c_uint64 * 3)()
         _check(self.L.sph_sort_forms(self.h, out))
diff --git a/gpufluidsimulator_amd/csrc/sph_capi.hip b/gpufluidsimulator_amd/csrc/sph_capi.hip
--- a/gpufluidsimulator_amd/csrc/sph_capi.hip
+++ b/gpufluidsimulator_amd/csrc/sph_capi.hip
@@ -105,6 +105,7 @@
 static void free_all(sph_ctx* c) {
     hipFree(c->posi); hipFree(c->velr); hipFree(c->posi2); hipFree(c->velr2); hipFree(c->keyS); hipFree(c->dp); hipFree(c->cw);
     hipFree(c->fpress); hipFree(c->fvisc); hipFree(c->dvel); hipFree(c->pos_out); hipFree(c->cells_base);
+    hipFree(c->rows); hipFree(c->row_hulls);
     hipFree(c->k0); hipFree(c->v0); hipFree(c->k1); hipFree(c->v1); hipFree(c->os_hist); hipFree(c->os_base); hipFree(c->os_tickets); hipFree(c->os_tot); hipFree(c->os_status); hipFree(c->os_status32); hipFree(c->keyS2); hipFree(c->mm_tileL); hipFree(c->mm_tileA);
     if (c->os_err_host) hipHostFree(c->os_err_host);
     hipFree(c->d_scratch);
@@ -157,6 +158,11 @@
     if (!rc) rc = dev_alloc(&c->fvisc, tot);
     if (!rc) rc = dev_alloc(&c->dvel, tot);
     if (!rc) rc = dev_alloc(&c->pos_out, (size_t)c->pos_out_cap);
+    if (!slab) {
+        c->row_stride = (uint32_t)tot;
+        if (!rc) rc = dev_alloc(&c->rows, 9 * tot);
+        if (!rc) rc = dev_alloc(&c->row_hulls, (tot / 64 + 2) * 18);
+    }
     if (!rc) rc = dev_alloc(&c->cells_base, (size_t)c->grid.ncells + 2);
     if (!rc) { c->cells = c->cells_base + 1; c->cells_alloc = c->grid.ncells; }
     if (!rc) rc = dev_alloc(&c->k0, (size_t)capacity);
@@ -349,6 +355,7 @@
         c->cells_base = base; c->cells = base + 1; c->cells_alloc = tmp.grid.ncells;
     }
     c->grid = tmp.grid; c->z_lo = z_lo; c->z_hi = z_hi; c->key_bits = tmp.key_bits;
+    state_changed(c);
     c->cells_valid = false; c->cells_clear_deferred = false;
     c->keys_fresh = false; c->order_valid = false;
     c->stage = sph_ctx::ST_LOADED;
@@ -488,6 +495,7 @@
     int rc = derive(&tmp, p, c->z_lo, c->z_hi, c->slab);
     if (rc) return rc;
     c->params = tmp.params; c->grid = tmp.grid; c->phys = tmp.phys;
+    state_changed(c);
     c->keys_fresh = false;
     c->order_valid = false;
     c->sort_form_both_until = c->sort_calls + 5;
@@ -526,6 +534,7 @@
         hv[i] = vel ? make_float4(vel[3 * i], vel[3 * i + 1], vel[3 * i + 2], 0.f) : make_float4(0.f, 0.f, 0.f, 0.f);
     }
     SPH_HIP(hipStreamSynchronize(c->stream));
+    state_changed(c);
     int rc = launch_cells_clear(c);
     if (rc) return rc;
     c->own_off = c->gcap;
@@ -560,6 +569,7 @@
                 "creation indices [%u, +%u) exceed the capacity %u", first_index, count, c->pos_out_cap);
     if (count == 0 || (!pos_xyz && !vel_xyz)) return SPH_OK;
     SPH_HIP(hipSetDevice(c->device));
+    state_changed(c);
     float* d_pos = nullptr; float* d_vel = nullptr;
     const size_t bytes = (size_t)count * 3 * sizeof(float);
     int rc = SPH_OK;
@@ -600,6 +610,7 @@
                 c->pos_out_cap);
     SPH_REQUIRE(total <= 0xFFFFFFFFull, SPH_E_INVALID, "creation indices are 32-bit");
     SPH_HIP(hipSetDevice(c->device));
+    state_changed(c);
     int rc = launch_cells_clear(c);
     if (rc) return rc;
     c->own_off = c->gcap;
@@ -1022,6 +1033,14 @@
     return SPH_OK;
 }
 
+int sph_test_set_row_handoff(sph_ctx* c, int on) {
+    SPH_REQUIRE(c, SPH_E_INVALID, "null context");
+    c->row_handoff = on != 0;
+    return SPH_OK;
+}
+
+uint64_t sph_test_row_handoff_launches(const sph_ctx* c) { return c ? c->row_handoff_launches : 0; }
+
 int sph_test_trust_mover_hint(sph_ctx* c) {
     SPH_REQUIRE(c, SPH_E_INVALID, "null context");
     c->sort_form_both_until = 0;
diff --git a/gpufluidsimulator_amd/csrc/sph_common.hpp b/gpufluidsimulator_amd/csrc/sph_common.hpp
--- a/gpufluidsimulator_amd/csrc/sph_common.hpp
+++ b/gpufluidsimulator_amd/csrc/sph_common.hpp
@@ -90,6 +90,14 @@
     float4* dvel = nullptr;
     float4* pos_out = nullptr;
     uint32_t pos_out_cap = 0;
+
+    uint32_t* rows = nullptr;
+    uint32_t* row_hulls = nullptr;
+    uint32_t row_stride = 0;
+    uint64_t state_gen = 1, rows_gen = 0;
+    uint32_t rows_lo = 0, rows_hi = 0;
+    bool row_handoff = true;
+    uint64_t row_handoff_launches = 0;
 
     uint32_t n_colliders = 0;
     sph_collider colliders[SPH_MAX_COLLIDERS] = {};
@@ -167,6 +175,7 @@
 namespace sph {
 
 void set_error(const char* fmt, ...);
+inline void state_changed(sph_ctx* c) { c->state_gen++; }
 void mm_drop_marks(sph_ctx* c);
 void mm_scan_marks(sph_ctx* c);
 int hip_fail(hipError_t e, const char* what, const char* file, int line);
diff --git a/gpufluidsimulator_amd/csrc/sph_pairs.hip b/gpufluidsimulator_amd/csrc/sph_pairs.hip
--- a/gpufluidsimulator_amd/csrc/sph_pairs.hip
+++ b/gpufluidsimulator_amd/csrc/sph_pairs.hip
@@ -54,6 +54,7 @@
 }
 
 int launch_cells_clear_2ranges(sph_ctx* c, uint32_t lo0, uint32_t hi0, uint32_t lo1, uint32_t hi1) {
+    state_changed(c);
     if (hi0 < lo0) hi0 = lo0;
     if (hi1 < lo1) hi1 = lo1;
     const uint32_t tot = (hi0 - lo0) + (hi1 - lo1);
@@ -64,6 +65,7 @@
 }
 
 int launch_cells_build_2ranges(sph_ctx* c, uint32_t lo0, uint32_t hi0, uint32_t lo1, uint32_t hi1) {
+    state_changed(c);
     if (hi0 < lo0) hi0 = lo0;
     if (hi1 < lo1) hi1 = lo1;
     const uint32_t tot = (hi0 - lo0) + (hi1 - lo1);
@@ -74,6 +76,7 @@
 }
 
 int launch_cells_clear(sph_ctx* c) {
+    state_changed(c);
     if (!c->cells_valid || c->cells_hi <= c->cells_lo) { c->cells_valid = false; return SPH_OK; }
     hipLaunchKernelGGL(k_cells_clear, dim3(ceil_div(c->cells_hi - c->cells_lo, 256)), dim3(256), 0, c->stream, c->keyS,
                        c->cells_lo, c->cells_hi, c->cells);
@@ -83,6 +86,7 @@
 }
 
 int launch_cells_clear_range(sph_ctx* c, uint32_t lo, uint32_t hi) {
+    state_changed(c);
     if (hi <= lo) return SPH_OK;
     hipLaunchKernelGGL(k_cells_clear, dim3(ceil_div(hi - lo, 256)), dim3(256), 0, c->stream, c->keyS, lo, hi, c->cells);
     SPH_HIP(hipGetLastError());
@@ -90,6 +94,7 @@
 }
 
 int launch_cells_build_range(sph_ctx* c, uint32_t lo, uint32_t hi) {
+    state_changed(c);
     if (hi <= lo) return SPH_OK;
     uint32_t* ends = (lo == c->own_off && hi == c->own_off + c->n) ? c->mm_count_host_dev + 1 : (uint32_t*)nullptr;
     const uint32_t seq = ends ? c->cells_seq_next : 0u;
@@ -100,6 +105,7 @@
 }
 
 int launch_cells_build(sph_ctx* c) {
+    state_changed(c);
     const uint32_t lo = c->own_off - c->n_glo, hi = c->own_off + c->n + c->n_ghi;
     int rc;
     if (c->cells_valid && c->cells_lo == c->own_off && c->cells_hi == c->own_off + c->n) {
@@ -221,6 +227,72 @@
         const int first = __builtin_ctzll(m), last = 63 - __builtin_clzll(m);
         H.A[r] = (uint32_t)__builtin_amdgcn_readlane((int)R.lo[r], first);
         H.B[r] = (uint32_t)__builtin_amdgcn_readlane((int)R.hi[r], last);
+    }
+}
+
+struct PRows {
+    uint32_t w[9];
+};
+
+__device__ __forceinline__ bool hulls_fit16(const Hulls& H) {
+    uint32_t m = 0u;
+#pragma unroll
+    for (int r = 0; r < 9; r++) m = max(m, H.B[r] - H.A[r]);
+    return m <= 0xFFFFu;
+}
+
+__device__ __forceinline__ void pack_rows(const Rows& R, const Hulls& H, PRows& P) {
+#pragma unroll
+    for (int r = 0; r < 9; r++) {
+        const uint32_t len = R.hi[r] - R.lo[r];
+        P.w[r] = len ? (R.lo[r] - H.A[r]) | (len << 16) : 0u;
+    }
+}
+
+__device__ __forceinline__ void piece_range(uint32_t w, uint32_t hullA, uint32_t a, uint32_t b, uint32_t& rel, uint32_t& len) {
+    const uint32_t pa = a - hullA, pb = b - hullA;
+    const uint32_t r0 = w & 0xFFFFu, r1 = r0 + (w >> 16);
+    const uint32_t l0 = max(r0, pa), l1 = min(r1, pb);
+    len = l1 > l0 ? l1 - l0 : 0u;
+    rel = len ? l0 - pa : 0u;
+}
+
+#ifndef SPH_ROW_HANDOFF
+#define SPH_ROW_HANDOFF 1
+#endif
+struct RowStore {
+    uint32_t* rows;
+    uint32_t* hulls;
+    uint32_t stride;
+};
+
+__device__ __forceinline__ void store_rows(const RowStore& rs, const PRows& P, const Hulls& H, bool fits, uint32_t chunk,
+                                           uint32_t lane, uint32_t i, bool active) {
+    int hv = 0;
+#pragma unroll
+    for (int r = 0; r < 9; r++) {
+        asm("v_writelane_b32 %0, %1, %2" : "+v"(hv) : "s"(H.A[r]), "n"(r));
+        asm("v_writelane_b32 %0, %1, %2" : "+v"(hv) : "s"(H.B[r]), "n"(9 + r));
+    }
+    if (lane < 18u) rs.hulls[(size_t)chunk * 18u + lane] = (uint32_t)hv;
+    if (active && fits) {
+#pragma unroll
+        for (int r = 0; r < 9; r++) rs.rows[(size_t)r * rs.stride + i] = P.w[r];
+    }
+}
+
+__device__ __forceinline__ void load_rows(const uint32_t* __restrict__ rows, const uint32_t* __restrict__ hulls, uint32_t stride,
+                                          uint32_t chunk, uint32_t ii, bool active, PRows& P, Hulls& H) {
+    const uint32_t* hp = hulls + (size_t)chunk * 18u;
+#pragma unroll
+    for (int r = 0; r < 9; r++) {
+        H.A[r] = (uint32_t)__builtin_amdgcn_readfirstlane((int)hp[r]);
+        H.B[r] = (uint32_t)__builtin_amdgcn_readfirstlane((int)hp[9 + r]);
+    }
+#pragma unroll
+    for (int r = 0; r < 9; r++) {
+        const uint32_t w = rows[(size_t)r * stride + ii];
+        P.w[r] = active ? w : 0u;
     }
 }
 
@@ -292,12 +364,12 @@
     return first < hi;
 }
 
-template <int THREADS>
+template <int THREADS, bool WRITE>
 __global__ __launch_bounds__(THREADS, SPH_DENS_OCC) void k_density(const float4* __restrict__ posi,
                                                                    const uint32_t* __restrict__ keyS,
                                                                    const uint2* __restrict__ cells,
                                                                    float2* __restrict__ dp, float2* __restrict__ cw,
-                                                                   Targets tg, GridDesc g, Phys ph) {
+                                                                   Targets tg, GridDesc g, Phys ph, RowStore rs) {
     static_assert(UNROLL % 2 == 0, "the z-pair walk reads candidates two at a time");
     constexpr int DENS_ENT = lds_ent(THREADS);
     __shared__ float2 s_xy[DENS_ENT];
@@ -319,11 +391,18 @@
     const bool active = i < tgt_hi;
     const uint32_t ii = active ? i : tgt_hi - 1;
     const float4 pi = posi[ii];
-    Rows R;
     const uint32_t my_key = keyS[ii];
-    lane_rows(cells, g, my_key, active, R);
+    PRows P;
     Hulls H;
-    wave_hulls(R, H);
+    bool fits;
+    {
+        Rows R;
+        lane_rows(cells, g, my_key, active, R);
+        wave_hulls(R, H);
+        fits = hulls_fit16(H);
+        pack_rows(R, H, P);
+    }
+    if (WRITE) store_rows(rs, P, H, fits, (uint32_t)__builtin_amdgcn_readfirstlane((int)((wave_first - tg.lo) >> 6)), lane, i, active);
     float4 q0, q1;
     float acc = 0.f;
     const float h2_v = in_vgpr(ph.h2);
@@ -341,7 +420,7 @@
             cw[i] = neighbour_terms(ph, rho, p);
         }
     };
-    if (wave_has_long_hull(H, my_key, tg.direct_hull)) {
+    if (!fits || wave_has_long_hull(H, my_key, tg.direct_hull)) {
         const uint32_t me = active ? i : tgt_hi - 1u;
         direct_rows(cells, g, keyS[me], active, [&](uint32_t l0, uint32_t len, uint32_t T) {
             for (uint32_t t = 0; t < T; t += 2u) {
@@ -370,9 +449,8 @@
             s_zo[slice + WAVE + lane - 1u] = q1.z;
         },
         [&](int r, uint32_t a, uint32_t b) {
-            const uint32_t l0 = max(R.lo[r], a), l1 = min(R.hi[r], b);
-            const uint32_t len = l1 > l0 ? l1 - l0 : 0u;
-            const uint32_t rel = len ? l0 - a : 0u;
+            uint32_t rel, len;
+            piece_range(P.w[r], H.A[r], a, b, rel, len);
             uint32_t idx = slice + rel;
             const uint32_t tmin = wave_min_u32_uniform_first(len) & ~(uint32_t)(UNROLL - 1);
             lds_v2f_ptr zp = (lds_v2f_ptr)((rel & 1u) ? (const float*)s_zo : (const float*)s_z) + ((slice + rel) >> 1);
@@ -686,14 +764,15 @@
 #else
 #define PAIR_STAT(k, v) do { } while (0)
 #endif
-template <bool FORCE, bool COLL, bool INTEG, int THREADS, class... Sph>
+template <bool FORCE, bool COLL, bool INTEG, int THREADS, bool HANDOFF, class... Sph>
 __global__ __launch_bounds__(THREADS, SPH_FORCE_OCC) void k_force(
     const float4* __restrict__ posi, const float4* __restrict__ velr, const float2* __restrict__ dp,
     const float2* __restrict__ cw, const uint32_t* __restrict__ keyS, const uint2* __restrict__ cells, float4* __restrict__ fpress,
     float4* __restrict__ fvisc, float4* __restrict__ dvel, float4* __restrict__ posi_out,
     float4* __restrict__ velr_out, float4* __restrict__ pos_by_index, uint32_t* __restrict__ keys_out,
     uint64_t* __restrict__ mm_mask, uint32_t* __restrict__ mm_tile_cnt, Targets tg,
-    uint32_t slot0, float dt, GridDesc g, Phys ph, Sph... sp) {
+    uint32_t slot0, float dt, GridDesc g, Phys ph, const uint32_t* __restrict__ rows, const uint32_t* __restrict__ row_hulls,
+    uint32_t row_stride, Sph... sp) {
     constexpr int E2 = 5;
     constexpr int ENT = lds_ent(THREADS);
     __shared__ float2 s_e[ENT * 5];
@@ -710,11 +789,18 @@
     float4 pi = posi[ii];
     float4 vi = velr[ii];
     const float2 dpi = dp[ii];
-    Rows R;
     const uint32_t my_key = keyS[ii];
-    lane_rows(cells, g, my_key, active, R);
+    PRows P;
     Hulls H;
-    wave_hulls(R, H);
+    if constexpr (HANDOFF) {
+        load_rows(rows, row_hulls, row_stride, (uint32_t)__builtin_amdgcn_readfirstlane((int)((wave_first - tg.lo) >> 6)), ii, active, P, H);
+    } else {
+        Rows R;
+        lane_rows(cells, g, my_key, active, R);
+        wave_hulls(R, H);
+        pack_rows(R, H, P);
+    }
+    const bool fits = hulls_fit16(H);
     PAIR_STAT(0, 1);
 #ifdef SPH_PAIR_STATS
     {
@@ -813,7 +899,7 @@
             }
         }
     };
-    if (wave_has_long_hull(H, my_key, tg.direct_hull)) {
+    if (!fits || wave_has_long_hull(H, my_key, tg.direct_hull)) {
         const uint32_t me = active ? i : tgt_hi - 1u;
         direct_rows(cells, g, keyS[me], active, [&](uint32_t l0, uint32_t len, uint32_t T) {
             for (uint32_t t = 0; t < T; t++) {
@@ -853,11 +939,11 @@
             }
         },
         [&](int r, uint32_t a, uint32_t b) {
-            const uint32_t l0 = max(R.lo[r], a), l1 = min(R.hi[r], b);
-            const uint32_t len = l1 > l0 ? l1 - l0 : 0u;
+            uint32_t rel, len;
+            piece_range(P.w[r], H.A[r], a, b, rel, len);
             uint32_t T, tmin_raw;
             wave_min_max_u32(len, tmin_raw, T);
-            uint32_t idx = slice + (len ? l0 - a : 0u);
+            uint32_t idx = slice + rel;
             const uint32_t tmin = tmin_raw & ~(uint32_t)(SPH_FORCE_UNROLL - 1);
             uint32_t near = 0u;
             PAIR_STAT(1, 1); PAIR_STAT(2, T);
@@ -952,14 +1038,26 @@
     return t;
 }
 
+static bool rows_launch_ok(const sph_ctx* c, const Targets& tg) {
+    return SPH_ROW_HANDOFF && c->row_handoff && c->rows && !c->slab && !tg.dev && tg.gap_len == 0u && tg.hi > tg.lo;
+}
+static bool rows_handoff_ok(const sph_ctx* c, const Targets& tg) {
+    return rows_launch_ok(c, tg) && c->rows_gen == c->state_gen && c->rows_lo == tg.lo && c->rows_hi == tg.hi;
+}
+
 template <bool F, bool C, bool I, class... Sph>
 static void force_kernel(sph_ctx* c, bool small, const Targets& tg, uint32_t threads, float dt, bool mark, Sph... sp) {
-#define SPH_LAUNCH_FORCE_T(T)                                                                                                   \
-    hipLaunchKernelGGL((k_force<F, C, I, T, Sph...>), dim3(ceil_div(threads, (uint32_t)T)), dim3(T), 0, c->stream, c->posi,       \
+#define SPH_LAUNCH_FORCE_T(T, H)                                                                                                \
+    hipLaunchKernelGGL((k_force<F, C, I, T, H, Sph...>), dim3(ceil_div(threads, (uint32_t)T)), dim3(T), 0, c->stream, c->posi,    \
                        c->velr, c->dp, c->cw, c->keyS, c->cells, c->fpress, c->fvisc, c->dvel, c->posi2, c->velr2,                \
                        c->slab ? nullptr : c->pos_out, c->k0, mark ? c->mm_mask : nullptr, c->mm_tile_cnt, tg, c->own_off, dt, \
-                       c->grid, c->phys, sp...)
-    if (small) SPH_LAUNCH_FORCE_T(SMALL_THREADS_PAIR); else SPH_LAUNCH_FORCE_T(PAIR_THREADS);
+                       c->grid, c->phys, c->rows, c->row_hulls, c->row_stride, sp...)
+    if (rows_handoff_ok(c, tg)) {
+        c->row_handoff_launches++;
+        if (small) SPH_LAUNCH_FORCE_T(SMALL_THREADS_PAIR, true); else SPH_LAUNCH_FORCE_T(PAIR_THREADS, true);
+    } else {
+        if (small) SPH_LAUNCH_FORCE_T(SMALL_THREADS_PAIR, false); else SPH_LAUNCH_FORCE_T(PAIR_THREADS, false);
+    }
 #undef SPH_LAUNCH_FORCE_T
 }
 
@@ -999,10 +1097,10 @@
     if (max_count == 0) return SPH_OK;
     const Targets tg{0u, 0u, 0xFFFFFFFFu, 0u, range_dev, c->direct_hull, BlockOrder{0u, 0u, 0u, 0u, 0u}};
 #define SPH_LAUNCH_EARLY(T, ...)                                                                                                    \
-    hipLaunchKernelGGL((k_force<true, true, true, T __VA_OPT__(, ) __VA_ARGS__>), dim3(ceil_div(max_count, (uint32_t)T)), dim3(T), 0,   \
+    hipLaunchKernelGGL((k_force<true, true, true, T, false __VA_OPT__(, ) __VA_ARGS__>), dim3(ceil_div(max_count, (uint32_t)T)), dim3(T), 0,   \
                        c->stream, c->posi, c->velr, c->dp, c->cw, c->keyS, c->cells, c->fpress, c->fvisc, c->dvel, c->posi2, c->velr2,  \
-                       c->slab ? nullptr : c->pos_out, c->keyS2, (uint64_t*)nullptr, c->mm_tile_cnt, tg, 0u, dt, c->grid, c->phys      \
-                       __VA_OPT__(, sphere_table(c)))
+                       c->slab ? nullptr : c->pos_out, c->keyS2, (uint64_t*)nullptr, c->mm_tile_cnt, tg, 0u, dt, c->grid, c->phys,     \
+                       (const uint32_t*)nullptr, (const uint32_t*)nullptr, 0u __VA_OPT__(, sphere_table(c)))
     if (c->n_colliders) {
         if (small_blocks(c)) SPH_LAUNCH_EARLY(SMALL_THREADS_PAIR, Spheres); else SPH_LAUNCH_EARLY(PAIR_THREADS, Spheres);
     } else {
@@ -1024,6 +1122,7 @@
 
 void force_finish(sph_ctx* c, bool integrate, bool mark, float dt) {
     if (!integrate) return;
+    state_changed(c);
     advance_colliders(c, dt);
     float4* t;
     t = c->posi; c->posi = c->posi2; c->posi2 = t;
@@ -1052,12 +1151,17 @@
     if (c->precision == SPH_PRECISION_MIXED_F16)
         hipLaunchKernelGGL(k_density_h, dim3(ceil_div(threads, PAIR_THREADS)), dim3(PAIR_THREADS), 0, c->stream, c->posi,
                            c->keyS, c->cells, c->dp, c->cw, tg, c->grid, c->phys);
-    else if (small_blocks(c))
-        hipLaunchKernelGGL(k_density<SMALL_THREADS_PAIR>, dim3(ceil_div(threads, (uint32_t)SMALL_THREADS_PAIR)), dim3(SMALL_THREADS_PAIR), 0, c->stream,
-                           c->posi, c->keyS, c->cells, c->dp, c->cw, tg, c->grid, c->phys);
-    else
-        hipLaunchKernelGGL(k_density<DENS_THREADS>, dim3(ceil_div(threads, (uint32_t)DENS_THREADS)), dim3(DENS_THREADS), 0, c->stream, c->posi,
-                           c->keyS, c->cells, c->dp, c->cw, tg, c->grid, c->phys);
+    else {
+        const bool write = rows_launch_ok(c, tg);
+        const RowStore rs{c->rows, c->row_hulls, c->row_stride};
+#define SPH_LAUNCH_DENS_T(T, W)                                                                                              \
+    hipLaunchKernelGGL((k_density<T, W>), dim3(ceil_div(threads, (uint32_t)T)), dim3(T), 0, c->stream, c->posi, c->keyS, c->cells, \
+                       c->dp, c->cw, tg, c->grid, c->phys, rs)
+        if (small_blocks(c)) { if (write) SPH_LAUNCH_DENS_T(SMALL_THREADS_PAIR, true); else SPH_LAUNCH_DENS_T(SMALL_THREADS_PAIR, false); }
+        else { if (write) SPH_LAUNCH_DENS_T(DENS_THREADS, true); else SPH_LAUNCH_DENS_T(DENS_THREADS, false); }
+#undef SPH_LAUNCH_DENS_T
+        if (write) { c->rows_gen = c->state_gen; c->rows_lo = tg.lo; c->rows_hi = tg.hi; }
+    }
     SPH_HIP(hipGetLastError());
     return SPH_OK;
 }
@@ -1101,6 +1205,7 @@
         return SPH_OK;
     }
     float4* const pos_out = c->slab ? nullptr : c->pos_out;
+    state_changed(c);
     if (c->n_colliders)
         hipLaunchKernelGGL(k_integrate<Spheres>, dim3(ceil_div(c->n, 256)), dim3(256), 0, c->stream, c->posi, c->velr, c->dp,
                            c->fpress, c->fvisc, c->dvel, pos_out, c->own_off, c->own_off + c->n, dt, c->phys, sphere_table(c));
diff --git a/gpufluidsimulator_amd/csrc/sph_sort.hip b/gpufluidsimulator_amd/csrc/sph_sort.hip
--- a/gpufluidsimulator_amd/csrc/sph_sort.hip
+++ b/gpufluidsimulator_amd/csrc/sph_sort.hip
@@ -1147,6 +1147,7 @@
 }
 
 int launch_sort(sph_ctx* c) {
+    state_changed(c);
     const uint32_t n = c->n;
     if (n == 0) return SPH_OK;
     const uint32_t nblocks = ceil_div(n, SORT_TILE);
@@ -1232,6 +1233,7 @@
 }
 
 int launch_merge_arrivals(sph_ctx* c, uint32_t n_in, uint32_t n_front) {
+    state_changed(c);
     const uint32_t n = c->n, n_tot = n + n_in;
     SPH_REQUIRE(c->order_valid && c->cells_valid && c->cells_lo == c->own_off && c->cells_hi == c->own_off + n, SPH_E_STATE,
                 "launch_merge_arrivals needs the sorted owned range and its cell table");
diff --git a/include/sph_hip.h b/include/sph_hip.h
--- a/include/sph_hip.h
+++ b/include/sph_hip.h
@@ -204,6 +204,8 @@
  int sph_slab_protocol(const sph_slab* s, uint64_t out[3]);
  int sph_slab_early_force_stats(const sph_slab* s, uint64_t out[2]);
  int sph_test_trust_mover_hint(sph_ctx* c);
+ int sph_test_set_row_handoff(sph_ctx* c, int on);
+ uint64_t sph_test_row_handoff_launches(const sph_ctx* c);
  int sph_slab_test_raise_flag(sph_slab* s, int flag);
 int sph_slab_failed(const sph_slab* s);
 
```

New measurement: 4.212 billion particle-steps/s. -1.8%, worse.
